# JasonHopeSpace/panda

Measured on AMD Instinct MI355X. Metric: MSM points/s (BN254, 2^24), higher is better.
Workload: dtype u32; 1 GPU; BN254 MSM 2^24 points per GPU, Jacobian output, bases and scalars resident in HBM; curve=bn254, log_points_per_gpu=24, exchange=none

## Files before the change

panda_amd/csrc/curve29.h:

```cpp
#pragma once
#include "fe29.h"

namespace panda29 {

template <class F>
struct Xyzz {
    Fe<F> X, Y, ZZ, ZZZ;
};

template <class F>
struct Bounds {
    static constexpr int M = SubMargin<F>::value;
    static constexpr int XB = 8 + M;
    static constexpr int YB = SubGrowth<F, 2>::value;
    static constexpr int PB = 2 + SubGrowth<F, XB>::value;
    static constexpr int RB = 2 + SubGrowth<F, YB>::value;
    static constexpr int VB = 2 + SubGrowth<F, XB>::value;
    static constexpr long long LIM = F::HEADROOM * 9 / 10;
    static_assert((long long)PB * PB < LIM, "P^2 exceeds the lazy-reduction headroom");
    static constexpr int NB = SubGrowth<F, 2>::value;
    static_assert((long long)RB * VB + (long long)YB * NB < LIM, "R*(Q-X3) - Y1*PPP exceeds the lazy-reduction headroom");
    static_assert(6LL * VB + 2LL * NB < LIM, "3x^2*(S-X3) - W*Y exceeds the lazy-reduction headroom");
    static_assert((long long)(2 * YB) * (2 * YB) < LIM, "(2Y)^2 exceeds the lazy-reduction headroom");
    static_assert(2 + SubGrowth<F, 6>::value <= XB, "X3 bound");
};

template <class F>
PANDA_HD void xyzz_set_identity(Xyzz<F> &p)
{
    fe_zero(p.X);
    fe_zero(p.Y);
    fe_zero(p.ZZ);
    fe_zero(p.ZZZ);
}

template <class F>
PANDA_HD bool xyzz_is_identity(const Xyzz<F> &p)
{
    return fe_all_zero(p.ZZ);
}

template <class F>
PANDA_HD void xyzz_from_affine(Xyzz<F> &p, const Fe<F> &x, const Fe<F> &y)
{
    p.X = x;
    p.Y = y;
    fe_one(p.ZZ);
    fe_one(p.ZZZ);
}

template <class F>
PANDA_HD void xyzz_finish(Fe<F> &X3, Fe<F> &Y3, const Fe<F> &R, const Fe<F> &Q, const Fe<F> &PPP, const Fe<F> &S1)
{
    typedef Bounds<F> B;
    Fe<F> t, rr, v, nppp;
    fe_add_nr(t, Q, Q);
    fe_add_nr(t, t, PPP);
    fe_sqr(rr, R);
    fe_sub<F, 6>(X3, rr, t);
    fe_sub<F, B::XB>(v, Q, X3);
    if constexpr (RawOperandOk<F>::value)
        fe_neg_raw<F, 2>(nppp, PPP);
    else
        fe_neg<F, 2>(nppp, PPP);
    fe_mul_add(Y3, R, v, S1, nppp);
}

template <class F>
PANDA_HD void xyzz_dbl_affine(Xyzz<F> &r, const Fe<F> &x, const Fe<F> &y)
{
    typedef Bounds<F> B;
    Fe<F> U, V, W, S, A, M3, t, v, t1, t2;
    fe_add(U, y, y);
    fe_sqr(V, U);
    if (fe_is_zero_2p(V)) {
        xyzz_set_identity(r);
        return;
    }
    fe_mul(W, U, V);
    fe_mul(S, x, V);
    fe_sqr(A, x);
    fe_add_nr(t, A, A);
    fe_add_nr(t, t, A);
    fe_norm(M3, t);
    fe_sqr(t1, M3);
    fe_add_nr(t, S, S);
    fe_sub<F, 4>(r.X, t1, t);
    fe_sub<F, B::XB>(v, S, r.X);
    fe_neg<F, 2>(t2, W);
    fe_mul_add(r.Y, M3, v, t2, y);
    r.ZZ = V;
    r.ZZZ = W;
}

template <class F>
PANDA_HD void xyzz_dbl(Xyzz<F> &r, const Xyzz<F> &p)
{
    typedef Bounds<F> B;
    if (xyzz_is_identity(p)) {
        xyzz_set_identity(r);
        return;
    }
    Fe<F> U, V, W, S, A, M3, t, v, t1, t2, X3, Y3;
    fe_add(U, p.Y, p.Y);
    fe_sqr(V, U);
    if (fe_is_zero_2p(V)) {
        xyzz_set_identity(r);
        return;
    }
    fe_mul(W, U, V);
    fe_mul(S, p.X, V);
    fe_sqr(A, p.X);
    fe_add_nr(t, A, A);
    fe_add_nr(t, t, A);
    fe_norm(M3, t);
    fe_sqr(t1, M3);
    fe_add_nr(t, S, S);
    fe_sub<F, 4>(X3, t1, t);
    fe_sub<F, B::XB>(v, S, X3);
    fe_neg<F, 2>(t2, W);
    fe_mul_add(Y3, M3, v, t2, p.Y);
    fe_mul(t, V, p.ZZ);
    fe_mul(t2, W, p.ZZZ);
    r.X = X3;
    r.Y = Y3;
    r.ZZ = t;
    r.ZZZ = t2;
}

template <class F>
PANDA_HD int xyzz_madd_core(Xyzz<F> &acc, const Fe<F> &bx, const Fe<F> &by)
{
    typedef Bounds<F> B;
    Fe<F> U2, S2, P, R, PP, PPP, Q, X3, Y3;
    fe_mul(U2, bx, acc.ZZ);
    fe_sub<F, B::XB>(P, U2, acc.X);
    fe_mul(S2, by, acc.ZZZ);
    fe_sub<F, B::YB>(R, S2, acc.Y);
    fe_sqr(PP, P);
    if (fe_is_zero_2p(PP))
        return fe_is_zero_mod_p(R) ? 1 : 2;
    fe_mul(PPP, P, PP);
    fe_mul(Q, acc.X, PP);
    fe_mul(acc.ZZ, acc.ZZ, PP);
    fe_mul(acc.ZZZ, acc.ZZZ, PPP);
    xyzz_finish(X3, Y3, R, Q, PPP, acc.Y);
    acc.X = X3;
    acc.Y = Y3;
    return 0;
}

template <class F>
PANDA_HD void xyzz_madd(Xyzz<F> &acc, const Fe<F> &bx, const Fe<F> &by, bool base_identity)
{
    if (base_identity) return;
    if (xyzz_is_identity(acc)) {
        xyzz_from_affine(acc, bx, by);
        return;
    }
    const int rare = xyzz_madd_core(acc, bx, by);
    if (rare == 1)
        xyzz_dbl_affine(acc, bx, by);
    else if (rare == 2)
        xyzz_set_identity(acc);
}

template <class F>
struct OutlineRareDoubling {
    static constexpr bool value = IsExt2<F>::value && F::N > 18;
};
template <class F>
#if defined(__HIPCC__)
__host__ __device__
#endif
__attribute__((noinline)) void xyzz_dbl_noinline(Xyzz<F> &r, const Xyzz<F> &p)
{
    xyzz_dbl(r, p);
}

template <class F>
PANDA_HD void xyzz_add(Xyzz<F> &acc, const Xyzz<F> &q)
{
    if (xyzz_is_identity(q)) return;
    if (xyzz_is_identity(acc)) {
        acc = q;
        return;
    }
    Fe<F> U1, U2, S1, S2, P, R, PP, PPP, Q, X3, Y3, t;
    fe_mul(U1, acc.X, q.ZZ);
    fe_mul(U2, q.X, acc.ZZ);
    fe_mul(S1, acc.Y, q.ZZZ);
    fe_mul(S2, q.Y, acc.ZZZ);
    fe_sub<F, 2>(P, U2, U1);
    fe_sub<F, 2>(R, S2, S1);
    fe_sqr(PP, P);
    if (fe_is_zero_2p(PP)) {
        if (fe_is_zero_mod_p(R)) {
            Xyzz<F> d;
            if constexpr (OutlineRareDoubling<F>::value)
                xyzz_dbl_noinline(d, acc);
            else
                xyzz_dbl(d, acc);
            acc = d;
        } else
            xyzz_set_identity(acc);
        return;
    }
    fe_mul(PPP, P, PP);
    fe_mul(Q, U1, PP);
    xyzz_finish(X3, Y3, R, Q, PPP, S1);
    fe_mul(t, acc.ZZ, q.ZZ);
    fe_mul(acc.ZZ, t, PP);
    fe_mul(t, acc.ZZZ, q.ZZZ);
    fe_mul(acc.ZZZ, t, PPP);
    acc.X = X3;
    acc.Y = Y3;
}

template <class F>
PANDA_HD void fe_neg_tight2p(Fe<F> &r, const Fe<F> &a)
{
    fe_neg<F, 2>(r, a);
}

template <class F>
PANDA_HD void xyzz_to_jacobian_wire(u32 *out, const Xyzz<F> &p)
{
    constexpr int L = F::L;
    if (xyzz_is_identity(p)) {
#pragma unroll
        for (int i = 0; i < 3 * L; i++) out[i] = 0;
        return;
    }
    Fe<F> x, y;
    fe_mul(x, p.X, p.ZZ);
    fe_mul(y, p.Y, p.ZZZ);
    fe_to_wire(out, x);
    fe_to_wire(out + L, y);
    fe_to_wire(out + 2 * L, p.ZZ);
}

template <class F>
PANDA_HD void xyzz_to_homogeneous_wire(u32 *out, const Xyzz<F> &p)
{
    constexpr int L = F::L;
    if (xyzz_is_identity(p)) {
#pragma unroll
        for (int i = 0; i < 3 * L; i++) out[i] = 0;
        return;
    }
    Fe<F> x, y, z;
    fe_mul(x, p.X, p.ZZZ);
    fe_mul(y, p.Y, p.ZZ);
    fe_mul(z, p.ZZ, p.ZZZ);
    fe_to_wire(out, x);
    fe_to_wire(out + L, y);
    fe_to_wire(out + 2 * L, z);
}

template <class F>
PANDA_HD void xyzz_to_affine_internal(Fe<F> &x, Fe<F> &y, const Xyzz<F> &p)
{
    Fe<F> zi3, t, zi2;
    fe_inv(zi3, p.ZZZ);
    fe_mul(t, p.ZZ, zi3);
    fe_sqr(zi2, t);
    fe_mul(x, p.X, zi2);
    fe_mul(y, p.Y, zi3);
}

template <class F>
PANDA_HD void xyzz_from_jacobian_wire(Xyzz<F> &p, const u32 *in)
{
    constexpr int L = F::L;
    Fe<F> z;
    fe_from_wire(z, in + 2 * L);
    if (fe_is_zero_2p(z)) {
        xyzz_set_identity(p);
        return;
    }
    fe_from_wire(p.X, in);
    fe_from_wire(p.Y, in + L);
    fe_sqr(p.ZZ, z);
    fe_mul(p.ZZZ, p.ZZ, z);
}

template <class F>
PANDA_HD bool affine_from_wire(Fe<F> &x, Fe<F> &y, const u32 *in)
{
    constexpr int L = F::L;
    u32 nz = 0;
#pragma unroll
    for (int i = 0; i < L; i++) nz |= in[i];
    fe_from_wire(x, in);
    fe_from_wire(y, in + L);
    return nz == 0;
}

}
```

panda_amd/csrc/fe29.h:

```cpp
#pragma once
#include <stdint.h>

#include "fe29_params.h"

#if defined(__HIPCC__)
#define PANDA_HD __host__ __device__ inline __attribute__((always_inline))
#else
#define PANDA_HD inline __attribute__((always_inline))
#endif

#if defined(FE29_CHECK)
#include <assert.h>
#define FE29_SHADOW_DECL unsigned __int128 shadow = 0;
#define FE29_SHADOW_MAC(x, y) shadow += (unsigned __int128)(x) * (y);
#define FE29_SHADOW_SHIFT()                                      \
    assert(shadow < ((unsigned __int128)1 << 64) && "fe29 column accumulator overflow"); \
    shadow >>= 29;
#else
#define FE29_SHADOW_DECL
#define FE29_SHADOW_MAC(x, y)
#define FE29_SHADOW_SHIFT()
#endif

#if defined(__HIP_DEVICE_COMPILE__) && !defined(FE29_NO_ASM)
#define FE29_MAC(acc, x, y) asm("v_mad_u64_u32 %0, vcc, %1, %2, %0" : "+v"(acc) : "v"(x), "v"(y) : "vcc")
#define FE29_MAC_CONST(acc, x, c) asm("v_mad_u64_u32 %0, vcc, %1, %2, %0" : "+v"(acc) : "v"(x), "s"(c) : "vcc")
#else
#define FE29_MAC(acc, x, y) acc += (u64)(x) * (y)
#define FE29_MAC_CONST(acc, x, c) acc += (u64)(x) * (c)
#endif

#if defined(__HIP_DEVICE_COMPILE__) && !defined(FE29_NO_ASM)
#define FE29_DEVICE_CHAINS 1
#include <utility>

#include "fe29_chain.h"
#endif

namespace panda29 {

typedef uint32_t u32;
typedef uint64_t u64;
constexpr u32 LIMB_BITS = 29;
constexpr u32 LIMB_MASK = (1u << 29) - 1;

template <class F>
struct Fe {
    u32 l[F::N];
};

template <class B>
struct Ext2;
template <class F>
struct IsExt2 {
    static constexpr bool value = false;
};
template <class B>
struct IsExt2<Ext2<B>> {
    static constexpr bool value = true;
};
template <class B>
PANDA_HD Fe<B> &ext_c0(Fe<Ext2<B>> &a) { return *reinterpret_cast<Fe<B> *>(&a.l[0]); }
template <class B>
PANDA_HD Fe<B> &ext_c1(Fe<Ext2<B>> &a) { return *reinterpret_cast<Fe<B> *>(&a.l[B::N]); }
template <class B>
PANDA_HD const Fe<B> &ext_c0(const Fe<Ext2<B>> &a) { return *reinterpret_cast<const Fe<B> *>(&a.l[0]); }
template <class B>
PANDA_HD const Fe<B> &ext_c1(const Fe<Ext2<B>> &a) { return *reinterpret_cast<const Fe<B> *>(&a.l[B::N]); }

template <class F>
PANDA_HD void fe_zero(Fe<F> &r)
{
#pragma unroll
    for (int i = 0; i < F::N; i++) r.l[i] = 0;
}

template <class F>
PANDA_HD void fe_one(Fe<F> &r)
{
#pragma unroll
    for (int i = 0; i < F::N; i++) r.l[i] = F::ONE[i];
}

template <class F>
PANDA_HD void fe_const(Fe<F> &r, const u32 (&c)[F::N])
{
#pragma unroll
    for (int i = 0; i < F::N; i++) r.l[i] = c[i];
}

template <class F>
PANDA_HD bool fe_all_zero(const Fe<F> &a)
{
    u32 acc = 0;
#pragma unroll
    for (int i = 0; i < F::N; i++) acc |= a.l[i];
    return acc == 0;
}

#if defined(FE29_DEVICE_CHAINS)
template <class F, int K>
__device__ inline __attribute__((always_inline)) void fe29_reduce_col(uint64_t &acc, uint32_t *m, uint32_t *out)
{
    constexpr int N = F::N;
    constexpr bool TOP0 = F::P[N - 1] == 0;
    if constexpr (K < N) {
        if constexpr (TOP0 && K == N - 1)
            MacChain<K - 1>::vs(acc, m + 1, &F::P[K - 1]);
        else
            MacChain<K>::vs(acc, m, &F::P[K]);
        m[K] = ((uint32_t)acc * F::INV) & ((1u << 29) - 1);
        MacChain<1>::vs(acc, m + K, &F::P[0]);
    } else {
        if constexpr (TOP0)
            MacChain<2 * N - 2 - K>::vs(acc, m + (K - N + 2), &F::P[N - 2]);
        else
            MacChain<2 * N - 1 - K>::vs(acc, m + (K - N + 1), &F::P[N - 1]);
        out[K - N] = (uint32_t)acc & ((1u << 29) - 1);
    }
    acc >>= 29;
}
template <class F, int K>
__device__ inline __attribute__((always_inline)) void fe29_mul_col(uint64_t &acc, const uint32_t *a, const uint32_t *b, uint32_t *m, uint32_t *out)
{
    constexpr int N = F::N;
    if constexpr (K == 0)
        MacChain<1>::vv0(acc, a, b);
    else if constexpr (K < N)
        MacChain<K + 1>::vv(acc, a, b + K);
    else
        MacChain<2 * N - 1 - K>::vv(acc, a + (K - N + 1), b + (N - 1));
    fe29_reduce_col<F, K>(acc, m, out);
}
template <class F, int K>
__device__ inline __attribute__((always_inline)) void fe29_sqr_col(uint64_t &acc, const uint32_t *a, const uint32_t *a2, uint32_t *m, uint32_t *out)
{
    constexpr int N = F::N;
    constexpr int I0 = K < N ? 0 : K - N + 1;
    constexpr int CNT = (K + 1) / 2 - I0;
    MacChain<CNT>::vv(acc, a2 + I0, a + (K - I0));
    if constexpr (K == 0)
        MacChain<1>::vv0(acc, a, a);
    else if constexpr ((K & 1) == 0)
        MacChain<1>::vv(acc, a + K / 2, a + K / 2);
    fe29_reduce_col<F, K>(acc, m, out);
}
template <class F, int... K>
__device__ inline __attribute__((always_inline)) void fe29_mul_cols(uint64_t &acc, const uint32_t *a, const uint32_t *b, uint32_t *m, uint32_t *out, std::integer_sequence<int, K...>)
{
    (fe29_mul_col<F, K>(acc, a, b, m, out), ...);
}
template <class F, int K>
__device__ inline __attribute__((always_inline)) void fe29_mul_add_col(uint64_t &acc, const uint32_t *a, const uint32_t *b, const uint32_t *c, const uint32_t *d, uint32_t *m,
                                                                       uint32_t *out)
{
    constexpr int N = F::N;
    if constexpr (K == 0) {
        MacChain<1>::vv0(acc, a, b);
        MacChain<1>::vv(acc, c, d);
    } else if constexpr (K < N) {
        MacChain<K + 1>::vv(acc, a, b + K);
        MacChain<K + 1>::vv(acc, c, d + K);
    } else {
        MacChain<2 * N - 1 - K>::vv(acc, a + (K - N + 1), b + (N - 1));
        MacChain<2 * N - 1 - K>::vv(acc, c + (K - N + 1), d + (N - 1));
    }
    fe29_reduce_col<F, K>(acc, m, out);
}
template <class F, int... K>
__device__ inline __attribute__((always_inline)) void fe29_mul_add_cols(uint64_t &acc, const uint32_t *a, const uint32_t *b, const uint32_t *c, const uint32_t *d,
                                                                        uint32_t *m, uint32_t *out, std::integer_sequence<int, K...>)
{
    (fe29_mul_add_col<F, K>(acc, a, b, c, d, m, out), ...);
}
template <class F, int... K>
__device__ inline __attribute__((always_inline)) void fe29_sqr_cols(uint64_t &acc, const uint32_t *a, const uint32_t *a2, uint32_t *m, uint32_t *out, std::integer_sequence<int, K...>)
{
    (fe29_sqr_col<F, K>(acc, a, a2, m, out), ...);
}
#endif

template <class F>
PANDA_HD void fe_mul(Fe<F> &r, const Fe<F> &a, const Fe<F> &b)
{
    constexpr int N = F::N;
    u32 m[N];
    u32 out[N];
    u64 acc = 0;
#if defined(FE29_DEVICE_CHAINS)
    fe29_mul_cols<F>(acc, a.l, b.l, m, out, std::make_integer_sequence<int, 2 * N - 1>());
    out[N - 1] = (u32)acc;
#pragma unroll
    for (int i = 0; i < N; i++) r.l[i] = out[i];
    return;
#endif
    FE29_SHADOW_DECL
#pragma unroll
    for (int k = 0; k < N; k++) {
#pragma unroll
        for (int i = 0; i <= k; i++) {
            FE29_MAC(acc, a.l[i], b.l[k - i]);
            FE29_SHADOW_MAC(a.l[i], b.l[k - i])
        }
#pragma unroll
        for (int i = 0; i < k; i++) {
            FE29_MAC_CONST(acc, m[i], F::P[k - i]);
            FE29_SHADOW_MAC(m[i], F::P[k - i])
        }
        m[k] = ((u32)acc * F::INV) & LIMB_MASK;
        FE29_MAC_CONST(acc, m[k], F::P[0]);
        FE29_SHADOW_MAC(m[k], F::P[0])
        acc >>= LIMB_BITS;
        FE29_SHADOW_SHIFT()
    }
#pragma unroll
    for (int k = N; k < 2 * N - 1; k++) {
#pragma unroll
        for (int i = k - N + 1; i < N; i++) {
            FE29_MAC(acc, a.l[i], b.l[k - i]);
            FE29_SHADOW_MAC(a.l[i], b.l[k - i])
        }
#pragma unroll
        for (int i = k - N + 1; i < N; i++) {
            FE29_MAC_CONST(acc, m[i], F::P[k - i]);
            FE29_SHADOW_MAC(m[i], F::P[k - i])
        }
        out[k - N] = (u32)acc & LIMB_MASK;
        acc >>= LIMB_BITS;
        FE29_SHADOW_SHIFT()
    }
    out[N - 1] = (u32)acc;
#pragma unroll
    for (int i = 0; i < N; i++) r.l[i] = out[i];
}

template <class F>
PANDA_HD void fe_mul_add(Fe<F> &r, const Fe<F> &a, const Fe<F> &b, const Fe<F> &c, const Fe<F> &d)
{
    constexpr int N = F::N;
    static_assert(3 * N * (1ull << 58) + (3ull * N << 38) < (1ull << 63) * 2 - 1, "column accumulator too narrow");
    u32 m[N];
    u32 out[N];
    u64 acc = 0;
#if defined(FE29_DEVICE_CHAINS)
    fe29_mul_add_cols<F>(acc, a.l, b.l, c.l, d.l, m, out, std::make_integer_sequence<int, 2 * N - 1>());
    out[N - 1] = (u32)acc;
#pragma unroll
    for (int i = 0; i < N; i++) r.l[i] = out[i];
    return;
#endif
    FE29_SHADOW_DECL
#pragma unroll
    for (int k = 0; k < N; k++) {
#pragma unroll
        for (int i = 0; i <= k; i++) {
            FE29_MAC(acc, a.l[i], b.l[k - i]);
            FE29_SHADOW_MAC(a.l[i], b.l[k - i])
            FE29_MAC(acc, c.l[i], d.l[k - i]);
            FE29_SHADOW_MAC(c.l[i], d.l[k - i])
        }
#pragma unroll
        for (int i = 0; i < k; i++) {
            FE29_MAC_CONST(acc, m[i], F::P[k - i]);
            FE29_SHADOW_MAC(m[i], F::P[k - i])
        }
        m[k] = ((u32)acc * F::INV) & LIMB_MASK;
        FE29_MAC_CONST(acc, m[k], F::P[0]);
        FE29_SHADOW_MAC(m[k], F::P[0])
        acc >>= LIMB_BITS;
        FE29_SHADOW_SHIFT()
    }
#pragma unroll
    for (int k = N; k < 2 * N - 1; k++) {
#pragma unroll
        for (int i = k - N + 1; i < N; i++) {
            FE29_MAC(acc, a.l[i], b.l[k - i]);
            FE29_SHADOW_MAC(a.l[i], b.l[k - i])
            FE29_MAC(acc, c.l[i], d.l[k - i]);
            FE29_SHADOW_MAC(c.l[i], d.l[k - i])
        }
#pragma unroll
        for (int i = k - N + 1; i < N; i++) {
            FE29_MAC_CONST(acc, m[i], F::P[k - i]);
            FE29_SHADOW_MAC(m[i], F::P[k - i])
        }
        out[k - N] = (u32)acc & LIMB_MASK;
        acc >>= LIMB_BITS;
        FE29_SHADOW_SHIFT()
    }
    out[N - 1] = (u32)acc;
#pragma unroll
    for (int i = 0; i < N; i++) r.l[i] = out[i];
}

template <class F>
PANDA_HD void fe_sqr(Fe<F> &r, const Fe<F> &a)
{
    constexpr int N = F::N;
    u32 m[N], out[N], a2[N];
#pragma unroll
    for (int i = 0; i < N; i++) a2[i] = a.l[i] << 1;
    u64 acc = 0;
#if defined(FE29_DEVICE_CHAINS)
    fe29_sqr_cols<F>(acc, a.l, a2, m, out, std::make_integer_sequence<int, 2 * N - 1>());
    out[N - 1] = (u32)acc;
#pragma unroll
    for (int i = 0; i < N; i++) r.l[i] = out[i];
    return;
#endif
    FE29_SHADOW_DECL
#pragma unroll
    for (int k = 0; k < N; k++) {
#pragma unroll
        for (int i = 0; 2 * i < k; i++) {
            FE29_MAC(acc, a2[i], a.l[k - i]);
            FE29_SHADOW_MAC(a2[i], a.l[k - i])
        }
        if ((k & 1) == 0) {
            FE29_MAC(acc, a.l[k / 2], a.l[k / 2]);
            FE29_SHADOW_MAC(a.l[k / 2], a.l[k / 2])
        }
#pragma unroll
        for (int i = 0; i < k; i++) {
            FE29_MAC_CONST(acc, m[i], F::P[k - i]);
            FE29_SHADOW_MAC(m[i], F::P[k - i])
        }
        m[k] = ((u32)acc * F::INV) & LIMB_MASK;
        FE29_MAC_CONST(acc, m[k], F::P[0]);
        FE29_SHADOW_MAC(m[k], F::P[0])
        acc >>= LIMB_BITS;
        FE29_SHADOW_SHIFT()
    }
// ... 21 lines not shown
#pragma unroll
    for (int i = 0; i < N; i++) r.l[i] = out[i];
}

template <class F>
PANDA_HD void fe_norm(Fe<F> &r, const Fe<F> &t)
{
    constexpr int N = F::N;
    u32 c[N];
#pragma unroll
    for (int i = 0; i < N - 1; i++) c[i] = t.l[i] >> LIMB_BITS;
    u32 o[N];
    o[0] = t.l[0] & LIMB_MASK;
#pragma unroll
    for (int i = 1; i < N - 1; i++) o[i] = (t.l[i] & LIMB_MASK) + c[i - 1];
    o[N - 1] = t.l[N - 1] + c[N - 2];
#pragma unroll
    for (int i = 0; i < N; i++) r.l[i] = o[i];
}

template <class F>
PANDA_HD void fe_add_nr(Fe<F> &r, const Fe<F> &a, const Fe<F> &b)
{
#pragma unroll
    for (int i = 0; i < F::N; i++) r.l[i] = a.l[i] + b.l[i];
}

template <class F>
PANDA_HD void fe_add(Fe<F> &r, const Fe<F> &a, const Fe<F> &b)
{
    Fe<F> t;
    fe_add_nr(t, a, b);
    fe_norm(r, t);
}

template <class F>
struct SubMargin {
    static constexpr int value = (F::P[F::N - 1] >= 16) ? 1 : 6;
};

template <class F, int KB>
PANDA_HD void fe_sub(Fe<F> &r, const Fe<F> &a, const Fe<F> &b)
{
    if constexpr (IsExt2<F>::value) {
        fe_sub<typename F::Base, KB>(ext_c0(r), ext_c0(a), ext_c0(b));
        fe_sub<typename F::Base, KB>(ext_c1(r), ext_c1(a), ext_c1(b));
        return;
    } else {
    constexpr int K = KB + SubMargin<F>::value;
    static_assert(K <= 200, "subtraction constant table too small");
    Fe<F> t;
#pragma unroll
    for (int i = 0; i < F::N; i++) {
#if defined(FE29_CHECK)
        assert((u64)a.l[i] + F::KP[K][i] >= b.l[i] && (u64)a.l[i] + F::KP[K][i] - b.l[i] < (1ull << 32) && "fe_sub limb range");
#endif
        t.l[i] = a.l[i] + F::KP[K][i] - b.l[i];
    }
    fe_norm(r, t);
    }
}

template <class F, int K>
PANDA_HD constexpr u32 fe_kp30(int i)
{
    return i == 0 ? F::KP[K][0] - (2u << LIMB_BITS) : (i < F::N - 1 ? F::KP[K][i] - (2u << LIMB_BITS) + 2u : F::KP[K][i] + 2u);
}

template <class F>
struct RawOperandOk {
    static constexpr bool value = F::N <= 9;
};

template <class F, int KB>
PANDA_HD void fe_sub_raw(Fe<F> &r, const Fe<F> &a, const Fe<F> &b)
{
    static_assert(RawOperandOk<F>::value, "no column headroom for a raw operand in this field");
    constexpr int K = KB + SubMargin<F>::value;
    static_assert(K <= 200, "subtraction constant table too small");
#pragma unroll
    for (int i = 0; i < F::N; i++) {
        const u32 kp = fe_kp30<F, K>(i);
#if defined(FE29_CHECK)
        assert((u64)a.l[i] + kp >= b.l[i] && (u64)a.l[i] + kp - b.l[i] < (1ull << 31) + (1ull << 24) && "fe_sub_raw limb range");
#endif
        r.l[i] = a.l[i] + kp - b.l[i];
    }
}

template <class F, int K, int U>
PANDA_HD constexpr u32 fe_kp_bias(int i)
{
    static_assert(U >= 2 && U <= 4, "bias in units of 2^29");
    return i == 0 ? F::KP[K][0] - ((u32)(4 - U) << LIMB_BITS) : (i < F::N - 1 ? F::KP[K][i] - ((u32)(4 - U) << LIMB_BITS) + (u32)(4 - U) : F::KP[K][i] + (u32)(4 - U));
}
template <class F, int KB, int U>
PANDA_HD void fe_sub_raw_bias(Fe<F> &r, const Fe<F> &a, const Fe<F> &b)
{
    static_assert(RawOperandOk<F>::value, "no column headroom for a raw operand in this field");
    constexpr int K = KB + SubMargin<F>::value;
    static_assert(K <= 200, "subtraction constant table too small");
#pragma unroll
    for (int i = 0; i < F::N; i++) {
        const u32 kp = fe_kp_bias<F, K, U>(i);
#if defined(FE29_CHECK)
        assert((u64)a.l[i] + kp >= b.l[i] && (u64)a.l[i] + kp - b.l[i] < 3 * (1ull << 30) + 64 && "fe_sub_raw_bias limb range");
#endif
        r.l[i] = a.l[i] + kp - b.l[i];
    }
}

template <class F, int KB>
PANDA_HD void fe_neg_raw(Fe<F> &r, const Fe<F> &a)
{
    static_assert(RawOperandOk<F>::value, "no column headroom for a raw operand in this field");
    constexpr int K = KB + SubMargin<F>::value;
#pragma unroll
    for (int i = 0; i < F::N; i++) {
        const u32 kp = fe_kp30<F, K>(i);
#if defined(FE29_CHECK)
        assert(kp >= a.l[i] && "fe_neg_raw limb range");
#endif
        r.l[i] = kp - a.l[i];
    }
}

template <class F, int KB>
struct SubGrowth {
    static constexpr int value = F::KEFF[KB + SubMargin<F>::value];
};

template <class F, int KB>
PANDA_HD void fe_neg(Fe<F> &r, const Fe<F> &a)
{
    if constexpr (IsExt2<F>::value) {
        fe_neg<typename F::Base, KB>(ext_c0(r), ext_c0(a));
        fe_neg<typename F::Base, KB>(ext_c1(r), ext_c1(a));
        return;
    } else {
    constexpr int K = KB + SubMargin<F>::value;
    Fe<F> t;
#pragma unroll
    for (int i = 0; i < F::N; i++) {
#if defined(FE29_CHECK)
        assert(F::KP[K][i] >= a.l[i] && "fe_neg limb range");
#endif
        t.l[i] = F::KP[K][i] - a.l[i];
    }
    fe_norm(r, t);
    }
}

template <class F>
PANDA_HD void fe_unpack(Fe<F> &r, const u32 *w)
{
    constexpr int N = F::N, L = F::L;
#pragma unroll
    for (int k = 0; k < N; k++) {
        const int bit = 29 * k, wi = bit >> 5, sh = bit & 31;
        u32 v = 0;
        if (wi < L) {
            v = w[wi] >> sh;
            if (sh > 3 && wi + 1 < L) v |= w[wi + 1] << (32 - sh);
        }
        r.l[k] = (k < N - 1) ? (v & LIMB_MASK) : v;
    }
}

template <class F>
PANDA_HD void fe_pack(u32 *w, const Fe<F> &a)
{
    constexpr int N = F::N, L = F::L;
#pragma unroll
    for (int i = 0; i < L; i++) {
        const int bit = 32 * i, j = bit / 29, s = bit - 29 * j;
        u32 v = a.l[j] >> s;
        if (j + 1 < N) v |= a.l[j + 1] << (29 - s);
        if (29 - s + 29 < 32 && j + 2 < N) v |= a.l[j + 2] << (58 - s);
        w[i] = v;
    }
}

template <class F>
PANDA_HD void fe_words_neg(u32 *r, const u32 *w)
{
    static_assert(!IsExt2<F>::value, "prime fields only");
#if defined(__clang__)
    unsigned borrow = 0;
#pragma unroll
    for (int i = 0; i < F::L; i++) r[i] = __builtin_subc(F::PW[i], w[i], borrow, &borrow);
#else
    u32 borrow = 0;
#pragma unroll
    for (int i = 0; i < F::L; i++) {
        const u32 d = F::PW[i] - w[i];
        const u32 out = (u32)(F::PW[i] < w[i]) | (u32)(d < borrow);
        r[i] = d - borrow;
        borrow = out;
    }
#endif
}

template <class F>
PANDA_HD void fe_carry(Fe<F> &a)
{
#pragma unroll
    for (int i = 0; i < F::N - 1; i++) {
#if defined(FE29_CHECK)
        assert((u64)a.l[i + 1] + (a.l[i] >> LIMB_BITS) < (1ull << 32) && "fe_carry limb range");
#endif
        a.l[i + 1] += a.l[i] >> LIMB_BITS;
        a.l[i] &= LIMB_MASK;
    }
}

template <class F>
PANDA_HD void fe_reduce_once(Fe<F> &a)
{
    constexpr int N = F::N;
    u32 d[N];
    u32 borrow = 0;
#pragma unroll
    for (int i = 0; i < N; i++) {
        u32 t = a.l[i] - F::P[i] - borrow;
        borrow = t >> 31;
        d[i] = (i < N - 1) ? (t & LIMB_MASK) : t;
    }
#pragma unroll
    for (int i = 0; i < N; i++) a.l[i] = borrow ? a.l[i] : d[i];
}

template <class F>
PANDA_HD void fe_reduce_small_2p(Fe<F> &a)
{
    constexpr int N = F::N;
    fe_carry(a);
    u32 m;
    if constexpr (F::P[N - 1] >= (1u << 16)) {
        constexpr u64 C = (1ull << 52) / ((u64)F::P[N - 1] + 1);
        m = (u32)(((u64)a.l[N - 1] * C) >> 52);
    } else {
        constexpr u64 D = ((u64)F::P[N - 1] << LIMB_BITS) + F::P[N - 2] + 1;
        static_assert(F::P[N - 1] < (1u << 12) && D >= (1u << 16), "fe_reduce_small: two-limb quotient estimate needs 2^16 <= D, top limb of p < 2^12");
        constexpr u64 C = (1ull << 52) / D;
        const u64 T = ((u64)a.l[N - 1] << LIMB_BITS) | a.l[N - 2];
        m = (u32)((T * C) >> 52);
    }
    int64_t carry = 0;
#pragma unroll
    for (int i = 0; i < N; i++) {
        int64_t t = (int64_t)a.l[i] - (int64_t)((u64)m * F::P[i]) + carry;
        a.l[i] = (i < N - 1) ? ((u32)t & LIMB_MASK) : (u32)t;
        carry = t >> LIMB_BITS;
    }
}

template <class F>
PANDA_HD void fe_reduce_small(Fe<F> &a)
{
    fe_reduce_small_2p(a);
    fe_reduce_once(a);
}

template <class F>
struct FeTw {
    u32 w[F::N];
    u32 q[F::N];
};

#if defined(FE29_DEVICE_CHAINS)
template <class F, bool UNIFORM, int C>
__device__ inline __attribute__((always_inline)) void fe29_shoup_hi_col(uint64_t &acc, const uint32_t *x, const uint32_t *wq, uint32_t *q)
{
    constexpr int N = F::N;
    constexpr int I0 = C < N ? 0 : C - N + 1;
    constexpr int CNT = (C < N ? C : N - 1) - I0 + 1;
    if constexpr (C == N - 2) {
        if constexpr (UNIFORM)
            MacChain<CNT>::vs0(acc, x + I0, wq + (C - I0));
        else
            MacChain<CNT>::vv0(acc, x + I0, wq + (C - I0));
    } else if constexpr (UNIFORM)
        MacChain<CNT>::vs(acc, x + I0, wq + (C - I0));
    else
        MacChain<CNT>::vv(acc, x + I0, wq + (C - I0));
    if constexpr (C >= N) q[C - N] = (uint32_t)acc & ((1u << 29) - 1);
    acc >>= 29;
}
template <class F, bool UNIFORM, int... C>
__device__ inline __attribute__((always_inline)) void fe29_shoup_hi_cols(uint64_t &acc, const uint32_t *x, const uint32_t *wq, uint32_t *q, std::integer_sequence<int, C...>)
{
    (fe29_shoup_hi_col<F, UNIFORM, F::N - 2 + C>(acc, x, wq, q), ...);
}
template <class F, bool UNIFORM, int C>
__device__ inline __attribute__((always_inline)) void fe29_shoup_lo_col(uint64_t &acc, const uint32_t *x, const uint32_t *w, const uint32_t *q, uint32_t *out)
{
    if constexpr (C == 0) {
        if constexpr (UNIFORM)
            MacChain<1>::vs0(acc, x, w);
        else
            MacChain<1>::vv0(acc, x, w);
    } else if constexpr (UNIFORM)
        MacChain<C + 1>::vs(acc, x, w + C);
    else
        MacChain<C + 1>::vv(acc, x, w + C);
    MacChain<C + 1>::vs(acc, q, &F::PNEG[C]);
    out[C] = (uint32_t)acc & ((1u << 29) - 1);
    if constexpr (C + 1 < F::N) acc >>= 29;
}
template <class F, bool UNIFORM, int... C>
__device__ inline __attribute__((always_inline)) void fe29_shoup_lo_cols(uint64_t &acc, const uint32_t *x, const uint32_t *w, const uint32_t *q, uint32_t *out,
                                                                         std::integer_sequence<int, C...>)
{
    (fe29_shoup_lo_col<F, UNIFORM, C>(acc, x, w, q, out), ...);
}
template <class F, bool UNIFORM, int... C>
__device__ inline __attribute__((always_inline)) void fe29_shoup_hi_cols_x2(uint64_t &a0, uint64_t &a1, const uint32_t *x0, const uint32_t *x1, const uint32_t *wq0,
                                                                            const uint32_t *wq1, uint32_t *q0, uint32_t *q1, std::integer_sequence<int, C...>)
{
    ((fe29_shoup_hi_col<F, UNIFORM, F::N - 2 + C>(a0, x0, wq0, q0), fe29_shoup_hi_col<F, UNIFORM, F::N - 2 + C>(a1, x1, wq1, q1)), ...);
}
template <class F, bool UNIFORM, int... C>
__device__ inline __attribute__((always_inline)) void fe29_shoup_lo_cols_x2(uint64_t &a0, uint64_t &a1, const uint32_t *x0, const uint32_t *x1, const uint32_t *w0,
                                                                            const uint32_t *w1, const uint32_t *q0, const uint32_t *q1, uint32_t *o0, uint32_t *o1,
                                                                            std::integer_sequence<int, C...>)
{
    ((fe29_shoup_lo_col<F, UNIFORM, C>(a0, x0, w0, q0, o0), fe29_shoup_lo_col<F, UNIFORM, C>(a1, x1, w1, q1, o1)), ...);
}
#endif

template <class F, bool UNIFORM = false>
PANDA_HD void fe_mul_shoup(Fe<F> &r, const Fe<F> &x, const u32 *w, const u32 *wq)
{
    constexpr int N = F::N;
    static_assert(RawOperandOk<F>::value, "no column headroom for a raw operand in this field");
    u32 q[N], out[N];
    u64 acc = 0;
#if defined(FE29_DEVICE_CHAINS)
    fe29_shoup_hi_cols<F, UNIFORM>(acc, x.l, wq, q, std::make_integer_sequence<int, N + 1>());
    q[N - 1] = (u32)acc & LIMB_MASK;
    acc = 0;
    fe29_shoup_lo_cols<F, UNIFORM>(acc, x.l, w, q, out, std::make_integer_sequence<int, N>());
#pragma unroll
// ... 231 lines not shown
```

panda_amd/csrc/fe29_chain.h:

```cpp
#pragma once
#include <stdint.h>

namespace panda29 {

template <int CNT>
struct MacChain;

template <>
struct MacChain<1> {
    static __device__ inline __attribute__((always_inline)) void vv(uint64_t &acc, const uint32_t *x, const uint32_t *y)
    {
        asm("v_mad_u64_u32 %0, vcc, %1, %2, %0" : "+v"(acc) : "v"(x[0]), "v"(y[0]) : "vcc");
    }
    static __device__ inline __attribute__((always_inline)) void vs(uint64_t &acc, const uint32_t *x, const uint32_t *y)
    {
        asm("v_mad_u64_u32 %0, vcc, %1, %2, %0" : "+v"(acc) : "v"(x[0]), "s"(y[0]) : "vcc");
    }
    static __device__ inline __attribute__((always_inline)) void vv0(uint64_t &acc, const uint32_t *x, const uint32_t *y)
    {
        asm("v_mad_u64_u32 %0, vcc, %1, %2, 0" : "=&v"(acc) : "v"(x[0]), "v"(y[0]) : "vcc");
    }
    static __device__ inline __attribute__((always_inline)) void vs0(uint64_t &acc, const uint32_t *x, const uint32_t *y)
    {
        asm("v_mad_u64_u32 %0, vcc, %1, %2, 0" : "=&v"(acc) : "v"(x[0]), "s"(y[0]) : "vcc");
    }
};
template <>
struct MacChain<2> {
    static __device__ inline __attribute__((always_inline)) void vv(uint64_t &acc, const uint32_t *x, const uint32_t *y)
    {
        asm("v_mad_u64_u32 %0, vcc, %1, %2, %0\n\tv_mad_u64_u32 %0, vcc, %3, %4, %0" : "+v"(acc) : "v"(x[0]), "v"(y[0]), "v"(x[1]), "v"(y[-1]) : "vcc");
    }
    static __device__ inline __attribute__((always_inline)) void vs(uint64_t &acc, const uint32_t *x, const uint32_t *y)
    {
        asm("v_mad_u64_u32 %0, vcc, %1, %2, %0\n\tv_mad_u64_u32 %0, vcc, %3, %4, %0" : "+v"(acc) : "v"(x[0]), "s"(y[0]), "v"(x[1]), "s"(y[-1]) : "vcc");
    }
    static __device__ inline __attribute__((always_inline)) void vv0(uint64_t &acc, const uint32_t *x, const uint32_t *y)
    {
        asm("v_mad_u64_u32 %0, vcc, %1, %2, 0\n\tv_mad_u64_u32 %0, vcc, %3, %4, %0" : "=&v"(acc) : "v"(x[0]), "v"(y[0]), "v"(x[1]), "v"(y[-1]) : "vcc");
    }
    static __device__ inline __attribute__((always_inline)) void vs0(uint64_t &acc, const uint32_t *x, const uint32_t *y)
    {
        asm("v_mad_u64_u32 %0, vcc, %1, %2, 0\n\tv_mad_u64_u32 %0, vcc, %3, %4, %0" : "=&v"(acc) : "v"(x[0]), "s"(y[0]), "v"(x[1]), "s"(y[-1]) : "vcc");
    }
};
template <>
struct MacChain<3> {
    static __device__ inline __attribute__((always_inline)) void vv(uint64_t &acc, const uint32_t *x, const uint32_t *y)
    {
        asm("v_mad_u64_u32 %0, vcc, %1, %2, %0\n\tv_mad_u64_u32 %0, vcc, %3, %4, %0\n\tv_mad_u64_u32 %0, vcc, %5, %6, %0" : "+v"(acc) : "v"(x[0]), "v"(y[0]), "v"(x[1]), "v"(y[-1]), "v"(x[2]), "v"(y[-2]) : "vcc");
    }
    static __device__ inline __attribute__((always_inline)) void vs(uint64_t &acc, const uint32_t *x, const uint32_t *y)
    {
        asm("v_mad_u64_u32 %0, vcc, %1, %2, %0\n\tv_mad_u64_u32 %0, vcc, %3, %4, %0\n\tv_mad_u64_u32 %0, vcc, %5, %6, %0" : "+v"(acc) : "v"(x[0]), "s"(y[0]), "v"(x[1]), "s"(y[-1]), "v"(x[2]), "s"(y[-2]) : "vcc");
    }
    static __device__ inline __attribute__((always_inline)) void vv0(uint64_t &acc, const uint32_t *x, const uint32_t *y)
    {
        asm("v_mad_u64_u32 %0, vcc, %1, %2, 0\n\tv_mad_u64_u32 %0, vcc, %3, %4, %0\n\tv_mad_u64_u32 %0, vcc, %5, %6, %0" : "=&v"(acc) : "v"(x[0]), "v"(y[0]), "v"(x[1]), "v"(y[-1]), "v"(x[2]), "v"(y[-2]) : "vcc");
    }
    static __device__ inline __attribute__((always_inline)) void vs0(uint64_t &acc, const uint32_t *x, const uint32_t *y)
    {
        asm("v_mad_u64_u32 %0, vcc, %1, %2, 0\n\tv_mad_u64_u32 %0, vcc, %3, %4, %0\n\tv_mad_u64_u32 %0, vcc, %5, %6, %0" : "=&v"(acc) : "v"(x[0]), "s"(y[0]), "v"(x[1]), "s"(y[-1]), "v"(x[2]), "s"(y[-2]) : "vcc");
    }
};
template <>
struct MacChain<4> {
    static __device__ inline __attribute__((always_inline)) void vv(uint64_t &acc, const uint32_t *x, const uint32_t *y)
    {
        asm("v_mad_u64_u32 %0, vcc, %1, %2, %0\n\tv_mad_u64_u32 %0, vcc, %3, %4, %0\n\tv_mad_u64_u32 %0, vcc, %5, %6, %0\n\tv_mad_u64_u32 %0, vcc, %7, %8, %0" : "+v"(acc) : "v"(x[0]), "v"(y[0]), "v"(x[1]), "v"(y[-1]), "v"(x[2]), "v"(y[-2]), "v"(x[3]), "v"(y[-3]) : "vcc");
    }
    static __device__ inline __attribute__((always_inline)) void vs(uint64_t &acc, const uint32_t *x, const uint32_t *y)
    {
        asm("v_mad_u64_u32 %0, vcc, %1, %2, %0\n\tv_mad_u64_u32 %0, vcc, %3, %4, %0\n\tv_mad_u64_u32 %0, vcc, %5, %6, %0\n\tv_mad_u64_u32 %0, vcc, %7, %8, %0" : "+v"(acc) : "v"(x[0]), "s"(y[0]), "v"(x[1]), "s"(y[-1]), "v"(x[2]), "s"(y[-2]), "v"(x[3]), "s"(y[-3]) : "vcc");
    }
    static __device__ inline __attribute__((always_inline)) void vv0(uint64_t &acc, const uint32_t *x, const uint32_t *y)
    {
        asm("v_mad_u64_u32 %0, vcc, %1, %2, 0\n\tv_mad_u64_u32 %0, vcc, %3, %4, %0\n\tv_mad_u64_u32 %0, vcc, %5, %6, %0\n\tv_mad_u64_u32 %0, vcc, %7, %8, %0" : "=&v"(acc) : "v"(x[0]), "v"(y[0]), "v"(x[1]), "v"(y[-1]), "v"(x[2]), "v"(y[-2]), "v"(x[3]), "v"(y[-3]) : "vcc");
    }
    static __device__ inline __attribute__((always_inline)) void vs0(uint64_t &acc, const uint32_t *x, const uint32_t *y)
    {
        asm("v_mad_u64_u32 %0, vcc, %1, %2, 0\n\tv_mad_u64_u32 %0, vcc, %3, %4, %0\n\tv_mad_u64_u32 %0, vcc, %5, %6, %0\n\tv_mad_u64_u32 %0, vcc, %7, %8, %0" : "=&v"(acc) : "v"(x[0]), "s"(y[0]), "v"(x[1]), "s"(y[-1]), "v"(x[2]), "s"(y[-2]), "v"(x[3]), "s"(y[-3]) : "vcc");
    }
};
template <>
struct MacChain<5> {
    static __device__ inline __attribute__((always_inline)) void vv(uint64_t &acc, const uint32_t *x, const uint32_t *y)
    {
        asm("v_mad_u64_u32 %0, vcc, %1, %2, %0\n\tv_mad_u64_u32 %0, vcc, %3, %4, %0\n\tv_mad_u64_u32 %0, vcc, %5, %6, %0\n\tv_mad_u64_u32 %0, vcc, %7, %8, %0\n\tv_mad_u64_u32 %0, vcc, %9, %10, %0" : "+v"(acc) : "v"(x[0]), "v"(y[0]), "v"(x[1]), "v"(y[-1]), "v"(x[2]), "v"(y[-2]), "v"(x[3]), "v"(y[-3]), "v"(x[4]), "v"(y[-4]) : "vcc");
    }
    static __device__ inline __attribute__((always_inline)) void vs(uint64_t &acc, const uint32_t *x, const uint32_t *y)
    {
        asm("v_mad_u64_u32 %0, vcc, %1, %2, %0\n\tv_mad_u64_u32 %0, vcc, %3, %4, %0\n\tv_mad_u64_u32 %0, vcc, %5, %6, %0\n\tv_mad_u64_u32 %0, vcc, %7, %8, %0\n\tv_mad_u64_u32 %0, vcc, %9, %10, %0" : "+v"(acc) : "v"(x[0]), "s"(y[0]), "v"(x[1]), "s"(y[-1]), "v"(x[2]), "s"(y[-2]), "v"(x[3]), "s"(y[-3]), "v"(x[4]), "s"(y[-4]) : "vcc");
    }
    static __device__ inline __attribute__((always_inline)) void vv0(uint64_t &acc, const uint32_t *x, const uint32_t *y)
    {
        asm("v_mad_u64_u32 %0, vcc, %1, %2, 0\n\tv_mad_u64_u32 %0, vcc, %3, %4, %0\n\tv_mad_u64_u32 %0, vcc, %5, %6, %0\n\tv_mad_u64_u32 %0, vcc, %7, %8, %0\n\tv_mad_u64_u32 %0, vcc, %9, %10, %0" : "=&v"(acc) : "v"(x[0]), "v"(y[0]), "v"(x[1]), "v"(y[-1]), "v"(x[2]), "v"(y[-2]), "v"(x[3]), "v"(y[-3]), "v"(x[4]), "v"(y[-4]) : "vcc");
    }
    static __device__ inline __attribute__((always_inline)) void vs0(uint64_t &acc, const uint32_t *x, const uint32_t *y)
    {
        asm("v_mad_u64_u32 %0, vcc, %1, %2, 0\n\tv_mad_u64_u32 %0, vcc, %3, %4, %0\n\tv_mad_u64_u32 %0, vcc, %5, %6, %0\n\tv_mad_u64_u32 %0, vcc, %7, %8, %0\n\tv_mad_u64_u32 %0, vcc, %9, %10, %0" : "=&v"(acc) : "v"(x[0]), "s"(y[0]), "v"(x[1]), "s"(y[-1]), "v"(x[2]), "s"(y[-2]), "v"(x[3]), "s"(y[-3]), "v"(x[4]), "s"(y[-4]) : "vcc");
    }
};
template <>
struct MacChain<6> {
    static __device__ inline __attribute__((always_inline)) void vv(uint64_t &acc, const uint32_t *x, const uint32_t *y)
    {
        asm("v_mad_u64_u32 %0, vcc, %1, %2, %0\n\tv_mad_u64_u32 %0, vcc, %3, %4, %0\n\tv_mad_u64_u32 %0, vcc, %5, %6, %0\n\tv_mad_u64_u32 %0, vcc, %7, %8, %0\n\tv_mad_u64_u32 %0, vcc, %9, %10, %0\n\tv_mad_u64_u32 %0, vcc, %11, %12, %0" : "+v"(acc) : "v"(x[0]), "v"(y[0]), "v"(x[1]), "v"(y[-1]), "v"(x[2]), "v"(y[-2]), "v"(x[3]), "v"(y[-3]), "v"(x[4]), "v"(y[-4]), "v"(x[5]), "v"(y[-5]) : "vcc");
    }
    static __device__ inline __attribute__((always_inline)) void vs(uint64_t &acc, const uint32_t *x, const uint32_t *y)
    {
        asm("v_mad_u64_u32 %0, vcc, %1, %2, %0\n\tv_mad_u64_u32 %0, vcc, %3, %4, %0\n\tv_mad_u64_u32 %0, vcc, %5, %6, %0\n\tv_mad_u64_u32 %0, vcc, %7, %8, %0\n\tv_mad_u64_u32 %0, vcc, %9, %10, %0\n\tv_mad_u64_u32 %0, vcc, %11, %12, %0" : "+v"(acc) : "v"(x[0]), "s"(y[0]), "v"(x[1]), "s"(y[-1]), "v"(x[2]), "s"(y[-2]), "v"(x[3]), "s"(y[-3]), "v"(x[4]), "s"(y[-4]), "v"(x[5]), "s"(y[-5]) : "vcc");
    }
    static __device__ inline __attribute__((always_inline)) void vv0(uint64_t &acc, const uint32_t *x, const uint32_t *y)
    {
        asm("v_mad_u64_u32 %0, vcc, %1, %2, 0\n\tv_mad_u64_u32 %0, vcc, %3, %4, %0\n\tv_mad_u64_u32 %0, vcc, %5, %6, %0\n\tv_mad_u64_u32 %0, vcc, %7, %8, %0\n\tv_mad_u64_u32 %0, vcc, %9, %10, %0\n\tv_mad_u64_u32 %0, vcc, %11, %12, %0" : "=&v"(acc) : "v"(x[0]), "v"(y[0]), "v"(x[1]), "v"(y[-1]), "v"(x[2]), "v"(y[-2]), "v"(x[3]), "v"(y[-3]), "v"(x[4]), "v"(y[-4]), "v"(x[5]), "v"(y[-5]) : "vcc");
    }
    static __device__ inline __attribute__((always_inline)) void vs0(uint64_t &acc, const uint32_t *x, const uint32_t *y)
    {
        asm("v_mad_u64_u32 %0, vcc, %1, %2, 0\n\tv_mad_u64_u32 %0, vcc, %3, %4, %0\n\tv_mad_u64_u32 %0, vcc, %5, %6, %0\n\tv_mad_u64_u32 %0, vcc, %7, %8, %0\n\tv_mad_u64_u32 %0, vcc, %9, %10, %0\n\tv_mad_u64_u32 %0, vcc, %11, %12, %0" : "=&v"(acc) : "v"(x[0]), "s"(y[0]), "v"(x[1]), "s"(y[-1]), "v"(x[2]), "s"(y[-2]), "v"(x[3]), "s"(y[-3]), "v"(x[4]), "s"(y[-4]), "v"(x[5]), "s"(y[-5]) : "vcc");
    }
};
template <>
struct MacChain<7> {
    static __device__ inline __attribute__((always_inline)) void vv(uint64_t &acc, const uint32_t *x, const uint32_t *y)
    {
        asm("v_mad_u64_u32 %0, vcc, %1, %2, %0\n\tv_mad_u64_u32 %0, vcc, %3, %4, %0\n\tv_mad_u64_u32 %0, vcc, %5, %6, %0\n\tv_mad_u64_u32 %0, vcc, %7, %8, %0\n\tv_mad_u64_u32 %0, vcc, %9, %10, %0\n\tv_mad_u64_u32 %0, vcc, %11, %12, %0\n\tv_mad_u64_u32 %0, vcc, %13, %14, %0" : "+v"(acc) : "v"(x[0]), "v"(y[0]), "v"(x[1]), "v"(y[-1]), "v"(x[2]), "v"(y[-2]), "v"(x[3]), "v"(y[-3]), "v"(x[4]), "v"(y[-4]), "v"(x[5]), "v"(y[-5]), "v"(x[6]), "v"(y[-6]) : "vcc");
    }
    static __device__ inline __attribute__((always_inline)) void vs(uint64_t &acc, const uint32_t *x, const uint32_t *y)
    {
        asm("v_mad_u64_u32 %0, vcc, %1, %2, %0\n\tv_mad_u64_u32 %0, vcc, %3, %4, %0\n\tv_mad_u64_u32 %0, vcc, %5, %6, %0\n\tv_mad_u64_u32 %0, vcc, %7, %8, %0\n\tv_mad_u64_u32 %0, vcc, %9, %10, %0\n\tv_mad_u64_u32 %0, vcc, %11, %12, %0\n\tv_mad_u64_u32 %0, vcc, %13, %14, %0" : "+v"(acc) : "v"(x[0]), "s"(y[0]), "v"(x[1]), "s"(y[-1]), "v"(x[2]), "s"(y[-2]), "v"(x[3]), "s"(y[-3]), "v"(x[4]), "s"(y[-4]), "v"(x[5]), "s"(y[-5]), "v"(x[6]), "s"(y[-6]) : "vcc");
    }
    static __device__ inline __attribute__((always_inline)) void vv0(uint64_t &acc, const uint32_t *x, const uint32_t *y)
    {
        asm("v_mad_u64_u32 %0, vcc, %1, %2, 0\n\tv_mad_u64_u32 %0, vcc, %3, %4, %0\n\tv_mad_u64_u32 %0, vcc, %5, %6, %0\n\tv_mad_u64_u32 %0, vcc, %7, %8, %0\n\tv_mad_u64_u32 %0, vcc, %9, %10, %0\n\tv_mad_u64_u32 %0, vcc, %11, %12, %0\n\tv_mad_u64_u32 %0, vcc, %13, %14, %0" : "=&v"(acc) : "v"(x[0]), "v"(y[0]), "v"(x[1]), "v"(y[-1]), "v"(x[2]), "v"(y[-2]), "v"(x[3]), "v"(y[-3]), "v"(x[4]), "v"(y[-4]), "v"(x[5]), "v"(y[-5]), "v"(x[6]), "v"(y[-6]) : "vcc");
    }
    static __device__ inline __attribute__((always_inline)) void vs0(uint64_t &acc, const uint32_t *x, const uint32_t *y)
    {
        asm("v_mad_u64_u32 %0, vcc, %1, %2, 0\n\tv_mad_u64_u32 %0, vcc, %3, %4, %0\n\tv_mad_u64_u32 %0, vcc, %5, %6, %0\n\tv_mad_u64_u32 %0, vcc, %7, %8, %0\n\tv_mad_u64_u32 %0, vcc, %9, %10, %0\n\tv_mad_u64_u32 %0, vcc, %11, %12, %0\n\tv_mad_u64_u32 %0, vcc, %13, %14, %0" : "=&v"(acc) : "v"(x[0]), "s"(y[0]), "v"(x[1]), "s"(y[-1]), "v"(x[2]), "s"(y[-2]), "v"(x[3]), "s"(y[-3]), "v"(x[4]), "s"(y[-4]), "v"(x[5]), "s"(y[-5]), "v"(x[6]), "s"(y[-6]) : "vcc");
    }
};
template <>
struct MacChain<8> {
    static __device__ inline __attribute__((always_inline)) void vv(uint64_t &acc, const uint32_t *x, const uint32_t *y)
    {
        asm("v_mad_u64_u32 %0, vcc, %1, %2, %0\n\tv_mad_u64_u32 %0, vcc, %3, %4, %0\n\tv_mad_u64_u32 %0, vcc, %5, %6, %0\n\tv_mad_u64_u32 %0, vcc, %7, %8, %0\n\tv_mad_u64_u32 %0, vcc, %9, %10, %0\n\tv_mad_u64_u32 %0, vcc, %11, %12, %0\n\tv_mad_u64_u32 %0, vcc, %13, %14, %0\n\tv_mad_u64_u32 %0, vcc, %15, %16, %0" : "+v"(acc) : "v"(x[0]), "v"(y[0]), "v"(x[1]), "v"(y[-1]), "v"(x[2]), "v"(y[-2]), "v"(x[3]), "v"(y[-3]), "v"(x[4]), "v"(y[-4]), "v"(x[5]), "v"(y[-5]), "v"(x[6]), "v"(y[-6]), "v"(x[7]), "v"(y[-7]) : "vcc");
    }
    static __device__ inline __attribute__((always_inline)) void vs(uint64_t &acc, const uint32_t *x, const uint32_t *y)
    {
        asm("v_mad_u64_u32 %0, vcc, %1, %2, %0\n\tv_mad_u64_u32 %0, vcc, %3, %4, %0\n\tv_mad_u64_u32 %0, vcc, %5, %6, %0\n\tv_mad_u64_u32 %0, vcc, %7, %8, %0\n\tv_mad_u64_u32 %0, vcc, %9, %10, %0\n\tv_mad_u64_u32 %0, vcc, %11, %12, %0\n\tv_mad_u64_u32 %0, vcc, %13, %14, %0\n\tv_mad_u64_u32 %0, vcc, %15, %16, %0" : "+v"(acc) : "v"(x[0]), "s"(y[0]), "v"(x[1]), "s"(y[-1]), "v"(x[2]), "s"(y[-2]), "v"(x[3]), "s"(y[-3]), "v"(x[4]), "s"(y[-4]), "v"(x[5]), "s"(y[-5]), "v"(x[6]), "s"(y[-6]), "v"(x[7]), "s"(y[-7]) : "vcc");
    }
    static __device__ inline __attribute__((always_inline)) void vv0(uint64_t &acc, const uint32_t *x, const uint32_t *y)
    {
        asm("v_mad_u64_u32 %0, vcc, %1, %2, 0\n\tv_mad_u64_u32 %0, vcc, %3, %4, %0\n\tv_mad_u64_u32 %0, vcc, %5, %6, %0\n\tv_mad_u64_u32 %0, vcc, %7, %8, %0\n\tv_mad_u64_u32 %0, vcc, %9, %10, %0\n\tv_mad_u64_u32 %0, vcc, %11, %12, %0\n\tv_mad_u64_u32 %0, vcc, %13, %14, %0\n\tv_mad_u64_u32 %0, vcc, %15, %16, %0" : "=&v"(acc) : "v"(x[0]), "v"(y[0]), "v"(x[1]), "v"(y[-1]), "v"(x[2]), "v"(y[-2]), "v"(x[3]), "v"(y[-3]), "v"(x[4]), "v"(y[-4]), "v"(x[5]), "v"(y[-5]), "v"(x[6]), "v"(y[-6]), "v"(x[7]), "v"(y[-7]) : "vcc");
    }
    static __device__ inline __attribute__((always_inline)) void vs0(uint64_t &acc, const uint32_t *x, const uint32_t *y)
    {
        asm("v_mad_u64_u32 %0, vcc, %1, %2, 0\n\tv_mad_u64_u32 %0, vcc, %3, %4, %0\n\tv_mad_u64_u32 %0, vcc, %5, %6, %0\n\tv_mad_u64_u32 %0, vcc, %7, %8, %0\n\tv_mad_u64_u32 %0, vcc, %9, %10, %0\n\tv_mad_u64_u32 %0, vcc, %11, %12, %0\n\tv_mad_u64_u32 %0, vcc, %13, %14, %0\n\tv_mad_u64_u32 %0, vcc, %15, %16, %0" : "=&v"(acc) : "v"(x[0]), "s"(y[0]), "v"(x[1]), "s"(y[-1]), "v"(x[2]), "s"(y[-2]), "v"(x[3]), "s"(y[-3]), "v"(x[4]), "s"(y[-4]), "v"(x[5]), "s"(y[-5]), "v"(x[6]), "s"(y[-6]), "v"(x[7]), "s"(y[-7]) : "vcc");
    }
};
template <>
struct MacChain<9> {
    static __device__ inline __attribute__((always_inline)) void vv(uint64_t &acc, const uint32_t *x, const uint32_t *y)
    {
        asm("v_mad_u64_u32 %0, vcc, %1, %2, %0\n\tv_mad_u64_u32 %0, vcc, %3, %4, %0\n\tv_mad_u64_u32 %0, vcc, %5, %6, %0\n\tv_mad_u64_u32 %0, vcc, %7, %8, %0\n\tv_mad_u64_u32 %0, vcc, %9, %10, %0\n\tv_mad_u64_u32 %0, vcc, %11, %12, %0\n\tv_mad_u64_u32 %0, vcc, %13, %14, %0\n\tv_mad_u64_u32 %0, vcc, %15, %16, %0\n\tv_mad_u64_u32 %0, vcc, %17, %18, %0" : "+v"(acc) : "v"(x[0]), "v"(y[0]), "v"(x[1]), "v"(y[-1]), "v"(x[2]), "v"(y[-2]), "v"(x[3]), "v"(y[-3]), "v"(x[4]), "v"(y[-4]), "v"(x[5]), "v"(y[-5]), "v"(x[6]), "v"(y[-6]), "v"(x[7]), "v"(y[-7]), "v"(x[8]), "v"(y[-8]) : "vcc");
    }
    static __device__ inline __attribute__((always_inline)) void vs(uint64_t &acc, const uint32_t *x, const uint32_t *y)
    {
        asm("v_mad_u64_u32 %0, vcc, %1, %2, %0\n\tv_mad_u64_u32 %0, vcc, %3, %4, %0\n\tv_mad_u64_u32 %0, vcc, %5, %6, %0\n\tv_mad_u64_u32 %0, vcc, %7, %8, %0\n\tv_mad_u64_u32 %0, vcc, %9, %10, %0\n\tv_mad_u64_u32 %0, vcc, %11, %12, %0\n\tv_mad_u64_u32 %0, vcc, %13, %14, %0\n\tv_mad_u64_u32 %0, vcc, %15, %16, %0\n\tv_mad_u64_u32 %0, vcc, %17, %18, %0" : "+v"(acc) : "v"(x[0]), "s"(y[0]), "v"(x[1]), "s"(y[-1]), "v"(x[2]), "s"(y[-2]), "v"(x[3]), "s"(y[-3]), "v"(x[4]), "s"(y[-4]), "v"(x[5]), "s"(y[-5]), "v"(x[6]), "s"(y[-6]), "v"(x[7]), "s"(y[-7]), "v"(x[8]), "s"(y[-8]) : "vcc");
    }
    static __device__ inline __attribute__((always_inline)) void vv0(uint64_t &acc, const uint32_t *x, const uint32_t *y)
    {
        asm("v_mad_u64_u32 %0, vcc, %1, %2, 0\n\tv_mad_u64_u32 %0, vcc, %3, %4, %0\n\tv_mad_u64_u32 %0, vcc, %5, %6, %0\n\tv_mad_u64_u32 %0, vcc, %7, %8, %0\n\tv_mad_u64_u32 %0, vcc, %9, %10, %0\n\tv_mad_u64_u32 %0, vcc, %11, %12, %0\n\tv_mad_u64_u32 %0, vcc, %13, %14, %0\n\tv_mad_u64_u32 %0, vcc, %15, %16, %0\n\tv_mad_u64_u32 %0, vcc, %17, %18, %0" : "=&v"(acc) : "v"(x[0]), "v"(y[0]), "v"(x[1]), "v"(y[-1]), "v"(x[2]), "v"(y[-2]), "v"(x[3]), "v"(y[-3]), "v"(x[4]), "v"(y[-4]), "v"(x[5]), "v"(y[-5]), "v"(x[6]), "v"(y[-6]), "v"(x[7]), "v"(y[-7]), "v"(x[8]), "v"(y[-8]) : "vcc");
    }
    static __device__ inline __attribute__((always_inline)) void vs0(uint64_t &acc, const uint32_t *x, const uint32_t *y)
    {
        asm("v_mad_u64_u32 %0, vcc, %1, %2, 0\n\tv_mad_u64_u32 %0, vcc, %3, %4, %0\n\tv_mad_u64_u32 %0, vcc, %5, %6, %0\n\tv_mad_u64_u32 %0, vcc, %7, %8, %0\n\tv_mad_u64_u32 %0, vcc, %9, %10, %0\n\tv_mad_u64_u32 %0, vcc, %11, %12, %0\n\tv_mad_u64_u32 %0, vcc, %13, %14, %0\n\tv_mad_u64_u32 %0, vcc, %15, %16, %0\n\tv_mad_u64_u32 %0, vcc, %17, %18, %0" : "=&v"(acc) : "v"(x[0]), "s"(y[0]), "v"(x[1]), "s"(y[-1]), "v"(x[2]), "s"(y[-2]), "v"(x[3]), "s"(y[-3]), "v"(x[4]), "s"(y[-4]), "v"(x[5]), "s"(y[-5]), "v"(x[6]), "s"(y[-6]), "v"(x[7]), "s"(y[-7]), "v"(x[8]), "s"(y[-8]) : "vcc");
    }
};
template <>
struct MacChain<10> {
    static __device__ inline __attribute__((always_inline)) void vv(uint64_t &acc, const uint32_t *x, const uint32_t *y)
    {
        asm("v_mad_u64_u32 %0, vcc, %1, %2, %0\n\tv_mad_u64_u32 %0, vcc, %3, %4, %0\n\tv_mad_u64_u32 %0, vcc, %5, %6, %0\n\tv_mad_u64_u32 %0, vcc, %7, %8, %0\n\tv_mad_u64_u32 %0, vcc, %9, %10, %0\n\tv_mad_u64_u32 %0, vcc, %11, %12, %0\n\tv_mad_u64_u32 %0, vcc, %13, %14, %0\n\tv_mad_u64_u32 %0, vcc, %15, %16, %0\n\tv_mad_u64_u32 %0, vcc, %17, %18, %0\n\tv_mad_u64_u32 %0, vcc, %19, %20, %0" : "+v"(acc) : "v"(x[0]), "v"(y[0]), "v"(x[1]), "v"(y[-1]), "v"(x[2]), "v"(y[-2]), "v"(x[3]), "v"(y[-3]), "v"(x[4]), "v"(y[-4]), "v"(x[5]), "v"(y[-5]), "v"(x[6]), "v"(y[-6]), "v"(x[7]), "v"(y[-7]), "v"(x[8]), "v"(y[-8]), "v"(x[9]), "v"(y[-9]) : "vcc");
    }
    static __device__ inline __attribute__((always_inline)) void vs(uint64_t &acc, const uint32_t *x, const uint32_t *y)
    {
        asm("v_mad_u64_u32 %0, vcc, %1, %2, %0\n\tv_mad_u64_u32 %0, vcc, %3, %4, %0\n\tv_mad_u64_u32 %0, vcc, %5, %6, %0\n\tv_mad_u64_u32 %0, vcc, %7, %8, %0\n\tv_mad_u64_u32 %0, vcc, %9, %10, %0\n\tv_mad_u64_u32 %0, vcc, %11, %12, %0\n\tv_mad_u64_u32 %0, vcc, %13, %14, %0\n\tv_mad_u64_u32 %0, vcc, %15, %16, %0\n\tv_mad_u64_u32 %0, vcc, %17, %18, %0\n\tv_mad_u64_u32 %0, vcc, %19, %20, %0" : "+v"(acc) : "v"(x[0]), "s"(y[0]), "v"(x[1]), "s"(y[-1]), "v"(x[2]), "s"(y[-2]), "v"(x[3]), "s"(y[-3]), "v"(x[4]), "s"(y[-4]), "v"(x[5]), "s"(y[-5]), "v"(x[6]), "s"(y[-6]), "v"(x[7]), "s"(y[-7]), "v"(x[8]), "s"(y[-8]), "v"(x[9]), "s"(y[-9]) : "vcc");
    }
    static __device__ inline __attribute__((always_inline)) void vv0(uint64_t &acc, const uint32_t *x, const uint32_t *y)
    {
        asm("v_mad_u64_u32 %0, vcc, %1, %2, 0\n\tv_mad_u64_u32 %0, vcc, %3, %4, %0\n\tv_mad_u64_u32 %0, vcc, %5, %6, %0\n\tv_mad_u64_u32 %0, vcc, %7, %8, %0\n\tv_mad_u64_u32 %0, vcc, %9, %10, %0\n\tv_mad_u64_u32 %0, vcc, %11, %12, %0\n\tv_mad_u64_u32 %0, vcc, %13, %14, %0\n\tv_mad_u64_u32 %0, vcc, %15, %16, %0\n\tv_mad_u64_u32 %0, vcc, %17, %18, %0\n\tv_mad_u64_u32 %0, vcc, %19, %20, %0" : "=&v"(acc) : "v"(x[0]), "v"(y[0]), "v"(x[1]), "v"(y[-1]), "v"(x[2]), "v"(y[-2]), "v"(x[3]), "v"(y[-3]), "v"(x[4]), "v"(y[-4]), "v"(x[5]), "v"(y[-5]), "v"(x[6]), "v"(y[-6]), "v"(x[7]), "v"(y[-7]), "v"(x[8]), "v"(y[-8]), "v"(x[9]), "v"(y[-9]) : "vcc");
    }
    static __device__ inline __attribute__((always_inline)) void vs0(uint64_t &acc, const uint32_t *x, const uint32_t *y)
    {
        asm("v_mad_u64_u32 %0, vcc, %1, %2, 0\n\tv_mad_u64_u32 %0, vcc, %3, %4, %0\n\tv_mad_u64_u32 %0, vcc, %5, %6, %0\n\tv_mad_u64_u32 %0, vcc, %7, %8, %0\n\tv_mad_u64_u32 %0, vcc, %9, %10, %0\n\tv_mad_u64_u32 %0, vcc, %11, %12, %0\n\tv_mad_u64_u32 %0, vcc, %13, %14, %0\n\tv_mad_u64_u32 %0, vcc, %15, %16, %0\n\tv_mad_u64_u32 %0, vcc, %17, %18, %0\n\tv_mad_u64_u32 %0, vcc, %19, %20, %0" : "=&v"(acc) : "v"(x[0]), "s"(y[0]), "v"(x[1]), "s"(y[-1]), "v"(x[2]), "s"(y[-2]), "v"(x[3]), "s"(y[-3]), "v"(x[4]), "s"(y[-4]), "v"(x[5]), "s"(y[-5]), "v"(x[6]), "s"(y[-6]), "v"(x[7]), "s"(y[-7]), "v"(x[8]), "s"(y[-8]), "v"(x[9]), "s"(y[-9]) : "vcc");
    }
};
template <>
struct MacChain<11> {
    static __device__ inline __attribute__((always_inline)) void vv(uint64_t &acc, const uint32_t *x, const uint32_t *y)
    {
        asm("v_mad_u64_u32 %0, vcc, %1, %2, %0\n\tv_mad_u64_u32 %0, vcc, %3, %4, %0\n\tv_mad_u64_u32 %0, vcc, %5, %6, %0\n\tv_mad_u64_u32 %0, vcc, %7, %8, %0\n\tv_mad_u64_u32 %0, vcc, %9, %10, %0\n\tv_mad_u64_u32 %0, vcc, %11, %12, %0\n\tv_mad_u64_u32 %0, vcc, %13, %14, %0\n\tv_mad_u64_u32 %0, vcc, %15, %16, %0\n\tv_mad_u64_u32 %0, vcc, %17, %18, %0\n\tv_mad_u64_u32 %0, vcc, %19, %20, %0\n\tv_mad_u64_u32 %0, vcc, %21, %22, %0" : "+v"(acc) : "v"(x[0]), "v"(y[0]), "v"(x[1]), "v"(y[-1]), "v"(x[2]), "v"(y[-2]), "v"(x[3]), "v"(y[-3]), "v"(x[4]), "v"(y[-4]), "v"(x[5]), "v"(y[-5]), "v"(x[6]), "v"(y[-6]), "v"(x[7]), "v"(y[-7]), "v"(x[8]), "v"(y[-8]), "v"(x[9]), "v"(y[-9]), "v"(x[10]), "v"(y[-10]) : "vcc");
    }
    static __device__ inline __attribute__((always_inline)) void vs(uint64_t &acc, const uint32_t *x, const uint32_t *y)
    {
        asm("v_mad_u64_u32 %0, vcc, %1, %2, %0\n\tv_mad_u64_u32 %0, vcc, %3, %4, %0\n\tv_mad_u64_u32 %0, vcc, %5, %6, %0\n\tv_mad_u64_u32 %0, vcc, %7, %8, %0\n\tv_mad_u64_u32 %0, vcc, %9, %10, %0\n\tv_mad_u64_u32 %0, vcc, %11, %12, %0\n\tv_mad_u64_u32 %0, vcc, %13, %14, %0\n\tv_mad_u64_u32 %0, vcc, %15, %16, %0\n\tv_mad_u64_u32 %0, vcc, %17, %18, %0\n\tv_mad_u64_u32 %0, vcc, %19, %20, %0\n\tv_mad_u64_u32 %0, vcc, %21, %22, %0" : "+v"(acc) : "v"(x[0]), "s"(y[0]), "v"(x[1]), "s"(y[-1]), "v"(x[2]), "s"(y[-2]), "v"(x[3]), "s"(y[-3]), "v"(x[4]), "s"(y[-4]), "v"(x[5]), "s"(y[-5]), "v"(x[6]), "s"(y[-6]), "v"(x[7]), "s"(y[-7]), "v"(x[8]), "s"(y[-8]), "v"(x[9]), "s"(y[-9]), "v"(x[10]), "s"(y[-10]) : "vcc");
    }
    static __device__ inline __attribute__((always_inline)) void vv0(uint64_t &acc, const uint32_t *x, const uint32_t *y)
    {
        asm("v_mad_u64_u32 %0, vcc, %1, %2, 0\n\tv_mad_u64_u32 %0, vcc, %3, %4, %0\n\tv_mad_u64_u32 %0, vcc, %5, %6, %0\n\tv_mad_u64_u32 %0, vcc, %7, %8, %0\n\tv_mad_u64_u32 %0, vcc, %9, %10, %0\n\tv_mad_u64_u32 %0, vcc, %11, %12, %0\n\tv_mad_u64_u32 %0, vcc, %13, %14, %0\n\tv_mad_u64_u32 %0, vcc, %15, %16, %0\n\tv_mad_u64_u32 %0, vcc, %17, %18, %0\n\tv_mad_u64_u32 %0, vcc, %19, %20, %0\n\tv_mad_u64_u32 %0, vcc, %21, %22, %0" : "=&v"(acc) : "v"(x[0]), "v"(y[0]), "v"(x[1]), "v"(y[-1]), "v"(x[2]), "v"(y[-2]), "v"(x[3]), "v"(y[-3]), "v"(x[4]), "v"(y[-4]), "v"(x[5]), "v"(y[-5]), "v"(x[6]), "v"(y[-6]), "v"(x[7]), "v"(y[-7]), "v"(x[8]), "v"(y[-8]), "v"(x[9]), "v"(y[-9]), "v"(x[10]), "v"(y[-10]) : "vcc");
    }
    static __device__ inline __attribute__((always_inline)) void vs0(uint64_t &acc, const uint32_t *x, const uint32_t *y)
    {
        asm("v_mad_u64_u32 %0, vcc, %1, %2, 0\n\tv_mad_u64_u32 %0, vcc, %3, %4, %0\n\tv_mad_u64_u32 %0, vcc, %5, %6, %0\n\tv_mad_u64_u32 %0, vcc, %7, %8, %0\n\tv_mad_u64_u32 %0, vcc, %9, %10, %0\n\tv_mad_u64_u32 %0, vcc, %11, %12, %0\n\tv_mad_u64_u32 %0, vcc, %13, %14, %0\n\tv_mad_u64_u32 %0, vcc, %15, %16, %0\n\tv_mad_u64_u32 %0, vcc, %17, %18, %0\n\tv_mad_u64_u32 %0, vcc, %19, %20, %0\n\tv_mad_u64_u32 %0, vcc, %21, %22, %0" : "=&v"(acc) : "v"(x[0]), "s"(y[0]), "v"(x[1]), "s"(y[-1]), "v"(x[2]), "s"(y[-2]), "v"(x[3]), "s"(y[-3]), "v"(x[4]), "s"(y[-4]), "v"(x[5]), "s"(y[-5]), "v"(x[6]), "s"(y[-6]), "v"(x[7]), "s"(y[-7]), "v"(x[8]), "s"(y[-8]), "v"(x[9]), "s"(y[-9]), "v"(x[10]), "s"(y[-10]) : "vcc");
    }
};
template <>
struct MacChain<12> {
    static __device__ inline __attribute__((always_inline)) void vv(uint64_t &acc, const uint32_t *x, const uint32_t *y)
    {
        asm("v_mad_u64_u32 %0, vcc, %1, %2, %0\n\tv_mad_u64_u32 %0, vcc, %3, %4, %0\n\tv_mad_u64_u32 %0, vcc, %5, %6, %0\n\tv_mad_u64_u32 %0, vcc, %7, %8, %0\n\tv_mad_u64_u32 %0, vcc, %9, %10, %0\n\tv_mad_u64_u32 %0, vcc, %11, %12, %0\n\tv_mad_u64_u32 %0, vcc, %13, %14, %0\n\tv_mad_u64_u32 %0, vcc, %15, %16, %0\n\tv_mad_u64_u32 %0, vcc, %17, %18, %0\n\tv_mad_u64_u32 %0, vcc, %19, %20, %0\n\tv_mad_u64_u32 %0, vcc, %21, %22, %0\n\tv_mad_u64_u32 %0, vcc, %23, %24, %0" : "+v"(acc) : "v"(x[0]), "v"(y[0]), "v"(x[1]), "v"(y[-1]), "v"(x[2]), "v"(y[-2]), "v"(x[3]), "v"(y[-3]), "v"(x[4]), "v"(y[-4]), "v"(x[5]), "v"(y[-5]), "v"(x[6]), "v"(y[-6]), "v"(x[7]), "v"(y[-7]), "v"(x[8]), "v"(y[-8]), "v"(x[9]), "v"(y[-9]), "v"(x[10]), "v"(y[-10]), "v"(x[11]), "v"(y[-11]) : "vcc");
    }
    static __device__ inline __attribute__((always_inline)) void vs(uint64_t &acc, const uint32_t *x, const uint32_t *y)
    {
        asm("v_mad_u64_u32 %0, vcc, %1, %2, %0\n\tv_mad_u64_u32 %0, vcc, %3, %4, %0\n\tv_mad_u64_u32 %0, vcc, %5, %6, %0\n\tv_mad_u64_u32 %0, vcc, %7, %8, %0\n\tv_mad_u64_u32 %0, vcc, %9, %10, %0\n\tv_mad_u64_u32 %0, vcc, %11, %12, %0\n\tv_mad_u64_u32 %0, vcc, %13, %14, %0\n\tv_mad_u64_u32 %0, vcc, %15, %16, %0\n\tv_mad_u64_u32 %0, vcc, %17, %18, %0\n\tv_mad_u64_u32 %0, vcc, %19, %20, %0\n\tv_mad_u64_u32 %0, vcc, %21, %22, %0\n\tv_mad_u64_u32 %0, vcc, %23, %24, %0" : "+v"(acc) : "v"(x[0]), "s"(y[0]), "v"(x[1]), "s"(y[-1]), "v"(x[2]), "s"(y[-2]), "v"(x[3]), "s"(y[-3]), "v"(x[4]), "s"(y[-4]), "v"(x[5]), "s"(y[-5]), "v"(x[6]), "s"(y[-6]), "v"(x[7]), "s"(y[-7]), "v"(x[8]), "s"(y[-8]), "v"(x[9]), "s"(y[-9]), "v"(x[10]), "s"(y[-10]), "v"(x[11]), "s"(y[-11]) : "vcc");
    }
    static __device__ inline __attribute__((always_inline)) void vv0(uint64_t &acc, const uint32_t *x, const uint32_t *y)
    {
        asm("v_mad_u64_u32 %0, vcc, %1, %2, 0\n\tv_mad_u64_u32 %0, vcc, %3, %4, %0\n\tv_mad_u64_u32 %0, vcc, %5, %6, %0\n\tv_mad_u64_u32 %0, vcc, %7, %8, %0\n\tv_mad_u64_u32 %0, vcc, %9, %10, %0\n\tv_mad_u64_u32 %0, vcc, %11, %12, %0\n\tv_mad_u64_u32 %0, vcc, %13, %14, %0\n\tv_mad_u64_u32 %0, vcc, %15, %16, %0\n\tv_mad_u64_u32 %0, vcc, %17, %18, %0\n\tv_mad_u64_u32 %0, vcc, %19, %20, %0\n\tv_mad_u64_u32 %0, vcc, %21, %22, %0\n\tv_mad_u64_u32 %0, vcc, %23, %24, %0" : "=&v"(acc) : "v"(x[0]), "v"(y[0]), "v"(x[1]), "v"(y[-1]), "v"(x[2]), "v"(y[-2]), "v"(x[3]), "v"(y[-3]), "v"(x[4]), "v"(y[-4]), "v"(x[5]), "v"(y[-5]), "v"(x[6]), "v"(y[-6]), "v"(x[7]), "v"(y[-7]), "v"(x[8]), "v"(y[-8]), "v"(x[9]), "v"(y[-9]), "v"(x[10]), "v"(y[-10]), "v"(x[11]), "v"(y[-11]) : "vcc");
    }
    static __device__ inline __attribute__((always_inline)) void vs0(uint64_t &acc, const uint32_t *x, const uint32_t *y)
    {
        asm("v_mad_u64_u32 %0, vcc, %1, %2, 0\n\tv_mad_u64_u32 %0, vcc, %3, %4, %0\n\tv_mad_u64_u32 %0, vcc, %5, %6, %0\n\tv_mad_u64_u32 %0, vcc, %7, %8, %0\n\tv_mad_u64_u32 %0, vcc, %9, %10, %0\n\tv_mad_u64_u32 %0, vcc, %11, %12, %0\n\tv_mad_u64_u32 %0, vcc, %13, %14, %0\n\tv_mad_u64_u32 %0, vcc, %15, %16, %0\n\tv_mad_u64_u32 %0, vcc, %17, %18, %0\n\tv_mad_u64_u32 %0, vcc, %19, %20, %0\n\tv_mad_u64_u32 %0, vcc, %21, %22, %0\n\tv_mad_u64_u32 %0, vcc, %23, %24, %0" : "=&v"(acc) : "v"(x[0]), "s"(y[0]), "v"(x[1]), "s"(y[-1]), "v"(x[2]), "s"(y[-2]), "v"(x[3]), "s"(y[-3]), "v"(x[4]), "s"(y[-4]), "v"(x[5]), "s"(y[-5]), "v"(x[6]), "s"(y[-6]), "v"(x[7]), "s"(y[-7]), "v"(x[8]), "s"(y[-8]), "v"(x[9]), "s"(y[-9]), "v"(x[10]), "s"(y[-10]), "v"(x[11]), "s"(y[-11]) : "vcc");
    }
};
template <>
struct MacChain<13> {
    static __device__ inline __attribute__((always_inline)) void vv(uint64_t &acc, const uint32_t *x, const uint32_t *y)
    {
        asm("v_mad_u64_u32 %0, vcc, %1, %2, %0\n\tv_mad_u64_u32 %0, vcc, %3, %4, %0\n\tv_mad_u64_u32 %0, vcc, %5, %6, %0\n\tv_mad_u64_u32 %0, vcc, %7, %8, %0\n\tv_mad_u64_u32 %0, vcc, %9, %10, %0\n\tv_mad_u64_u32 %0, vcc, %11, %12, %0\n\tv_mad_u64_u32 %0, vcc, %13, %14, %0\n\tv_mad_u64_u32 %0, vcc, %15, %16, %0\n\tv_mad_u64_u32 %0, vcc, %17, %18, %0\n\tv_mad_u64_u32 %0, vcc, %19, %20, %0\n\tv_mad_u64_u32 %0, vcc, %21, %22, %0\n\tv_mad_u64_u32 %0, vcc, %23, %24, %0\n\tv_mad_u64_u32 %0, vcc, %25, %26, %0" : "+v"(acc) : "v"(x[0]), "v"(y[0]), "v"(x[1]), "v"(y[-1]), "v"(x[2]), "v"(y[-2]), "v"(x[3]), "v"(y[-3]), "v"(x[4]), "v"(y[-4]), "v"(x[5]), "v"(y[-5]), "v"(x[6]), "v"(y[-6]), "v"(x[7]), "v"(y[-7]), "v"(x[8]), "v"(y[-8]), "v"(x[9]), "v"(y[-9]), "v"(x[10]), "v"(y[-10]), "v"(x[11]), "v"(y[-11]), "v"(x[12]), "v"(y[-12]) : "vcc");
    }
    static __device__ inline __attribute__((always_inline)) void vs(uint64_t &acc, const uint32_t *x, const uint32_t *y)
    {
        asm("v_mad_u64_u32 %0, vcc, %1, %2, %0\n\tv_mad_u64_u32 %0, vcc, %3, %4, %0\n\tv_mad_u64_u32 %0, vcc, %5, %6, %0\n\tv_mad_u64_u32 %0, vcc, %7, %8, %0\n\tv_mad_u64_u32 %0, vcc, %9, %10, %0\n\tv_mad_u64_u32 %0, vcc, %11, %12, %0\n\tv_mad_u64_u32 %0, vcc, %13, %14, %0\n\tv_mad_u64_u32 %0, vcc, %15, %16, %0\n\tv_mad_u64_u32 %0, vcc, %17, %18, %0\n\tv_mad_u64_u32 %0, vcc, %19, %20, %0\n\tv_mad_u64_u32 %0, vcc, %21, %22, %0\n\tv_mad_u64_u32 %0, vcc, %23, %24, %0\n\tv_mad_u64_u32 %0, vcc, %25, %26, %0" : "+v"(acc) : "v"(x[0]), "s"(y[0]), "v"(x[1]), "s"(y[-1]), "v"(x[2]), "s"(y[-2]), "v"(x[3]), "s"(y[-3]), "v"(x[4]), "s"(y[-4]), "v"(x[5]), "s"(y[-5]), "v"(x[6]), "s"(y[-6]), "v"(x[7]), "s"(y[-7]), "v"(x[8]), "s"(y[-8]), "v"(x[9]), "s"(y[-9]), "v"(x[10]), "s"(y[-10]), "v"(x[11]), "s"(y[-11]), "v"(x[12]), "s"(y[-12]) : "vcc");
    }
    static __device__ inline __attribute__((always_inline)) void vv0(uint64_t &acc, const uint32_t *x, const uint32_t *y)
    {
        asm("v_mad_u64_u32 %0, vcc, %1, %2, 0\n\tv_mad_u64_u32 %0, vcc, %3, %4, %0\n\tv_mad_u64_u32 %0, vcc, %5, %6, %0\n\tv_mad_u64_u32 %0, vcc, %7, %8, %0\n\tv_mad_u64_u32 %0, vcc, %9, %10, %0\n\tv_mad_u64_u32 %0, vcc, %11, %12, %0\n\tv_mad_u64_u32 %0, vcc, %13, %14, %0\n\tv_mad_u64_u32 %0, vcc, %15, %16, %0\n\tv_mad_u64_u32 %0, vcc, %17, %18, %0\n\tv_mad_u64_u32 %0, vcc, %19, %20, %0\n\tv_mad_u64_u32 %0, vcc, %21, %22, %0\n\tv_mad_u64_u32 %0, vcc, %23, %24, %0\n\tv_mad_u64_u32 %0, vcc, %25, %26, %0" : "=&v"(acc) : "v"(x[0]), "v"(y[0]), "v"(x[1]), "v"(y[-1]), "v"(x[2]), "v"(y[-2]), "v"(x[3]), "v"(y[-3]), "v"(x[4]), "v"(y[-4]), "v"(x[5]), "v"(y[-5]), "v"(x[6]), "v"(y[-6]), "v"(x[7]), "v"(y[-7]), "v"(x[8]), "v"(y[-8]), "v"(x[9]), "v"(y[-9]), "v"(x[10]), "v"(y[-10]), "v"(x[11]), "v"(y[-11]), "v"(x[12]), "v"(y[-12]) : "vcc");
    }
    static __device__ inline __attribute__((always_inline)) void vs0(uint64_t &acc, const uint32_t *x, const uint32_t *y)
    {
        asm("v_mad_u64_u32 %0, vcc, %1, %2, 0\n\tv_mad_u64_u32 %0, vcc, %3, %4, %0\n\tv_mad_u64_u32 %0, vcc, %5, %6, %0\n\tv_mad_u64_u32 %0, vcc, %7, %8, %0\n\tv_mad_u64_u32 %0, vcc, %9, %10, %0\n\tv_mad_u64_u32 %0, vcc, %11, %12, %0\n\tv_mad_u64_u32 %0, vcc, %13, %14, %0\n\tv_mad_u64_u32 %0, vcc, %15, %16, %0\n\tv_mad_u64_u32 %0, vcc, %17, %18, %0\n\tv_mad_u64_u32 %0, vcc, %19, %20, %0\n\tv_mad_u64_u32 %0, vcc, %21, %22, %0\n\tv_mad_u64_u32 %0, vcc, %23, %24, %0\n\tv_mad_u64_u32 %0, vcc, %25, %26, %0" : "=&v"(acc) : "v"(x[0]), "s"(y[0]), "v"(x[1]), "s"(y[-1]), "v"(x[2]), "s"(y[-2]), "v"(x[3]), "s"(y[-3]), "v"(x[4]), "s"(y[-4]), "v"(x[5]), "s"(y[-5]), "v"(x[6]), "s"(y[-6]), "v"(x[7]), "s"(y[-7]), "v"(x[8]), "s"(y[-8]), "v"(x[9]), "s"(y[-9]), "v"(x[10]), "s"(y[-10]), "v"(x[11]), "s"(y[-11]), "v"(x[12]), "s"(y[-12]) : "vcc");
    }
};
template <>
struct MacChain<14> {
    static __device__ inline __attribute__((always_inline)) void vv(uint64_t &acc, const uint32_t *x, const uint32_t *y)
    {
        asm("v_mad_u64_u32 %0, vcc, %1, %2, %0\n\tv_mad_u64_u32 %0, vcc, %3, %4, %0\n\tv_mad_u64_u32 %0, vcc, %5, %6, %0\n\tv_mad_u64_u32 %0, vcc, %7, %8, %0\n\tv_mad_u64_u32 %0, vcc, %9, %10, %0\n\tv_mad_u64_u32 %0, vcc, %11, %12, %0\n\tv_mad_u64_u32 %0, vcc, %13, %14, %0\n\tv_mad_u64_u32 %0, vcc, %15, %16, %0\n\tv_mad_u64_u32 %0, vcc, %17, %18, %0\n\tv_mad_u64_u32 %0, vcc, %19, %20, %0\n\tv_mad_u64_u32 %0, vcc, %21, %22, %0\n\tv_mad_u64_u32 %0, vcc, %23, %24, %0\n\tv_mad_u64_u32 %0, vcc, %25, %26, %0\n\tv_mad_u64_u32 %0, vcc, %27, %28, %0" : "+v"(acc) : "v"(x[0]), "v"(y[0]), "v"(x[1]), "v"(y[-1]), "v"(x[2]), "v"(y[-2]), "v"(x[3]), "v"(y[-3]), "v"(x[4]), "v"(y[-4]), "v"(x[5]), "v"(y[-5]), "v"(x[6]), "v"(y[-6]), "v"(x[7]), "v"(y[-7]), "v"(x[8]), "v"(y[-8]), "v"(x[9]), "v"(y[-9]), "v"(x[10]), "v"(y[-10]), "v"(x[11]), "v"(y[-11]), "v"(x[12]), "v"(y[-12]), "v"(x[13]), "v"(y[-13]) : "vcc");
    }
    static __device__ inline __attribute__((always_inline)) void vs(uint64_t &acc, const uint32_t *x, const uint32_t *y)
    {
        asm("v_mad_u64_u32 %0, vcc, %1, %2, %0\n\tv_mad_u64_u32 %0, vcc, %3, %4, %0\n\tv_mad_u64_u32 %0, vcc, %5, %6, %0\n\tv_mad_u64_u32 %0, vcc, %7, %8, %0\n\tv_mad_u64_u32 %0, vcc, %9, %10, %0\n\tv_mad_u64_u32 %0, vcc, %11, %12, %0\n\tv_mad_u64_u32 %0, vcc, %13, %14, %0\n\tv_mad_u64_u32 %0, vcc, %15, %16, %0\n\tv_mad_u64_u32 %0, vcc, %17, %18, %0\n\tv_mad_u64_u32 %0, vcc, %19, %20, %0\n\tv_mad_u64_u32 %0, vcc, %21, %22, %0\n\tv_mad_u64_u32 %0, vcc, %23, %24, %0\n\tv_mad_u64_u32 %0, vcc, %25, %26, %0\n\tv_mad_u64_u32 %0, vcc, %27, %28, %0" : "+v"(acc) : "v"(x[0]), "s"(y[0]), "v"(x[1]), "s"(y[-1]), "v"(x[2]), "s"(y[-2]), "v"(x[3]), "s"(y[-3]), "v"(x[4]), "s"(y[-4]), "v"(x[5]), "s"(y[-5]), "v"(x[6]), "s"(y[-6]), "v"(x[7]), "s"(y[-7]), "v"(x[8]), "s"(y[-8]), "v"(x[9]), "s"(y[-9]), "v"(x[10]), "s"(y[-10]), "v"(x[11]), "s"(y[-11]), "v"(x[12]), "s"(y[-12]), "v"(x[13]), "s"(y[-13]) : "vcc");
    }
    static __device__ inline __attribute__((always_inline)) void vv0(uint64_t &acc, const uint32_t *x, const uint32_t *y)
    {
        asm("v_mad_u64_u32 %0, vcc, %1, %2, 0\n\tv_mad_u64_u32 %0, vcc, %3, %4, %0\n\tv_mad_u64_u32 %0, vcc, %5, %6, %0\n\tv_mad_u64_u32 %0, vcc, %7, %8, %0\n\tv_mad_u64_u32 %0, vcc, %9, %10, %0\n\tv_mad_u64_u32 %0, vcc, %11, %12, %0\n\tv_mad_u64_u32 %0, vcc, %13, %14, %0\n\tv_mad_u64_u32 %0, vcc, %15, %16, %0\n\tv_mad_u64_u32 %0, vcc, %17, %18, %0\n\tv_mad_u64_u32 %0, vcc, %19, %20, %0\n\tv_mad_u64_u32 %0, vcc, %21, %22, %0\n\tv_mad_u64_u32 %0, vcc, %23, %24, %0\n\tv_mad_u64_u32 %0, vcc, %25, %26, %0\n\tv_mad_u64_u32 %0, vcc, %27, %28, %0" : "=&v"(acc) : "v"(x[0]), "v"(y[0]), "v"(x[1]), "v"(y[-1]), "v"(x[2]), "v"(y[-2]), "v"(x[3]), "v"(y[-3]), "v"(x[4]), "v"(y[-4]), "v"(x[5]), "v"(y[-5]), "v"(x[6]), "v"(y[-6]), "v"(x[7]), "v"(y[-7]), "v"(x[8]), "v"(y[-8]), "v"(x[9]), "v"(y[-9]), "v"(x[10]), "v"(y[-10]), "v"(x[11]), "v"(y[-11]), "v"(x[12]), "v"(y[-12]), "v"(x[13]), "v"(y[-13]) : "vcc");
    }
    static __device__ inline __attribute__((always_inline)) void vs0(uint64_t &acc, const uint32_t *x, const uint32_t *y)
    {
        asm("v_mad_u64_u32 %0, vcc, %1, %2, 0\n\tv_mad_u64_u32 %0, vcc, %3, %4, %0\n\tv_mad_u64_u32 %0, vcc, %5, %6, %0\n\tv_mad_u64_u32 %0, vcc, %7, %8, %0\n\tv_mad_u64_u32 %0, vcc, %9, %10, %0\n\tv_mad_u64_u32 %0, vcc, %11, %12, %0\n\tv_mad_u64_u32 %0, vcc, %13, %14, %0\n\tv_mad_u64_u32 %0, vcc, %15, %16, %0\n\tv_mad_u64_u32 %0, vcc, %17, %18, %0\n\tv_mad_u64_u32 %0, vcc, %19, %20, %0\n\tv_mad_u64_u32 %0, vcc, %21, %22, %0\n\tv_mad_u64_u32 %0, vcc, %23, %24, %0\n\tv_mad_u64_u32 %0, vcc, %25, %26, %0\n\tv_mad_u64_u32 %0, vcc, %27, %28, %0" : "=&v"(acc) : "v"(x[0]), "s"(y[0]), "v"(x[1]), "s"(y[-1]), "v"(x[2]), "s"(y[-2]), "v"(x[3]), "s"(y[-3]), "v"(x[4]), "s"(y[-4]), "v"(x[5]), "s"(y[-5]), "v"(x[6]), "s"(y[-6]), "v"(x[7]), "s"(y[-7]), "v"(x[8]), "s"(y[-8]), "v"(x[9]), "s"(y[-9]), "v"(x[10]), "s"(y[-10]), "v"(x[11]), "s"(y[-11]), "v"(x[12]), "s"(y[-12]), "v"(x[13]), "s"(y[-13]) : "vcc");
    }
};
template <>
struct MacChain<0> {
    static __device__ inline __attribute__((always_inline)) void vv(uint64_t &, const uint32_t *, const uint32_t *) {}
    static __device__ inline __attribute__((always_inline)) void vs(uint64_t &, const uint32_t *, const uint32_t *) {}
    static __device__ inline __attribute__((always_inline)) void vv0(uint64_t &acc, const uint32_t *, const uint32_t *) { acc = 0; }
    static __device__ inline __attribute__((always_inline)) void vs0(uint64_t &acc, const uint32_t *, const uint32_t *) { acc = 0; }
};

}
```

panda_amd/csrc/msm_impl.h:

```cpp
#pragma once
#include <algorithm>
#include <vector>

#include "curve29_quad.h"
#include "msm_sort.h"
#include "panda_internal.h"

namespace panda {

struct MsmRegistration {
    const void *wire;
    void *converted;
    unsigned log_n, curve;
    int device;
    bool tabled;
    WindowPlan plan;
    size_t bytes;
    const uint32_t *samples;
    uint64_t hash;
};
hipError_t msm_hash_wire(const void *d_buf, size_t bytes, hipStream_t s, uint64_t *hash);

struct MsmTuning {
    unsigned window_bits;
// ... 153 lines not shown
        dst[4 * i] = v.x;
        dst[4 * i + 1] = v.y;
        dst[4 * i + 2] = v.z;
        dst[4 * i + 3] = v.w;
    }
}

template <int WORDS>
__device__ __forceinline__ void load_words_stream(u32 *dst, const u32 *src)
{
    static_assert(WORDS % 4 == 0, "vector loads");
    typedef u32 v4u __attribute__((ext_vector_type(4)));
    const v4u *s4 = reinterpret_cast<const v4u *>(src);
#pragma unroll
    for (int i = 0; i < WORDS / 4; i++) {
        const v4u v = __builtin_nontemporal_load(&s4[i]);
        dst[4 * i] = v.x;
        dst[4 * i + 1] = v.y;
        dst[4 * i + 2] = v.z;
        dst[4 * i + 3] = v.w;
    }
}

template <int WORDS>
__device__ __forceinline__ void store_words(u32 *dst, const u32 *src)
{
    uint4 *d4 = reinterpret_cast<uint4 *>(dst);
#pragma unroll
    for (int i = 0; i < WORDS / 4; i++) d4[i] = make_uint4(src[4 * i], src[4 * i + 1], src[4 * i + 2], src[4 * i + 3]);
}


template <class F>
__global__ void __launch_bounds__(256) k_convert_bases(const u32 *__restrict__ wire, u32 *__restrict__ out, u64 n)
{
    constexpr int L = F::L;
    u64 i = (u64)blockIdx.x * blockDim.x + threadIdx.x;
    if (i >= n) return;
    u32 w[2 * L], o[2 * L];
    load_words<2 * L>(w, wire + i * 2 * L);
    Fe<F> x, y;
    bool inf = affine_from_wire(x, y, w);
    fe_reduce_once(x);
    fe_reduce_once(y);
    fe_pack(o, x);
    fe_pack(o + L, y);
    if (inf) {
#pragma unroll
        for (int k = 0; k < 2 * L; k++) o[k] = 0;
    }
    store_words<2 * L>(out + i * 2 * L, o);
}

template <class F>
__device__ __noinline__ void xyzz_add_outlined(Xyzz<F> &acc, const Xyzz<F> &q)
{
    xyzz_add(acc, q);
}
template <class F>
__device__ __noinline__ void xyzz_dbl_outlined(Xyzz<F> &r, const Xyzz<F> &p)
{
    xyzz_dbl(r, p);
}
template <class F>
__device__ __forceinline__ void xyzz_add_k(Xyzz<F> &acc, const Xyzz<F> &q)
{
    if constexpr (IsExt2<F>::value)
        xyzz_add_outlined(acc, q);
    else
        xyzz_add(acc, q);
}
template <class F>
__device__ __forceinline__ void xyzz_dbl_k(Xyzz<F> &r, const Xyzz<F> &p)
{
    if constexpr (IsExt2<F>::value)
        xyzz_dbl_outlined(r, p);
    else
        xyzz_dbl(r, p);
}

template <class F>
__device__ __noinline__ void xyzz_add_quad_outlined(Xyzz<F> &acc, const Xyzz<F> &q, unsigned role)
{
    xyzz_add_quad(acc, q, role);
}
template <class F>
__device__ __noinline__ void xyzz_dbl_quad_outlined(Xyzz<F> &r, const Xyzz<F> &p, unsigned role)
{
    xyzz_dbl_quad(r, p, role);
}
template <class F>
__device__ __forceinline__ void xyzz_add_q(Xyzz<F> &acc, const Xyzz<F> &q, unsigned role)
{
    if constexpr (IsExt2<F>::value)
        xyzz_add_quad_outlined(acc, q, role);
    else
        xyzz_add_quad(acc, q, role);
}
template <class F>
__device__ __forceinline__ void xyzz_dbl_q(Xyzz<F> &r, const Xyzz<F> &p, unsigned role)
{
    if constexpr (IsExt2<F>::value)
        xyzz_dbl_quad_outlined(r, p, role);
    else
        xyzz_dbl_quad(r, p, role);
}

__global__ void __launch_bounds__(panda::REG_SAMPLES * 16) k_take_samples(const u32 *__restrict__ wire, u32 *__restrict__ samples, u64 n, unsigned row_words)
{
    const unsigned t = threadIdx.x >> 4, l = threadIdx.x & 15;
    const u64 row = panda::sample_row(t, n);
    for (unsigned k = l; k < row_words; k += 16) samples[t * row_words + k] = wire[row * row_words + k];
}

__device__ __forceinline__ u32 owner_bucket(const u32 *off, u32 NB, u32 pos)
{
    u32 lo = 0, hi = NB;
    while (hi - lo > 1) {
        u32 mid = (lo + hi) >> 1;
        if (off[mid] <= pos) lo = mid;
        else hi = mid;
    }
    return lo;
}

__global__ void __launch_bounds__(256) k_chunk_first(const u32 *__restrict__ off, u32 *__restrict__ first, unsigned NB, unsigned K, unsigned chunks)
{
    const unsigned w = blockIdx.y;
    const u32 *ow = off + (u64)w * (NB + 1);
    u32 *fw = first + (u64)w * chunks;
    const unsigned b = blockIdx.x * blockDim.x + threadIdx.x;
    u32 t0 = 0, t1 = 0;
    if (b < NB) {
        const u32 lo = ow[b], hi = ow[b + 1];
        t0 = (lo + K - 1) / K;
        t1 = min((u32)((hi + K - 1) / K), (u32)chunks);
    }
    const unsigned lane = threadIdx.x & 63u;
    u64 wide = __ballot(t1 > t0 + 4);
    while (wide) {
        const int src = __ffsll((long long)wide) - 1;
        wide &= wide - 1;
        const u32 a = (u32)__shfl((int)t0, src), e = (u32)__shfl((int)t1, src), owner = (u32)__shfl((int)b, src);
        for (u32 t = a + lane; t < e; t += 64) fw[t] = owner;
    }
    if (t1 <= t0 + 4)
        for (u32 t = t0; t < t1; t++) fw[t] = b;
}

#ifndef PANDA_ROW_MASK
#define PANDA_ROW_MASK 0x7fffffffu
#endif
#ifndef PANDA_ACC_ITEMS
#define PANDA_ACC_ITEMS 0x3fu
#endif
constexpr unsigned ACC_ITEM_ROW_TUPLES = 32u;
constexpr unsigned ACC_ITEM_WORDS_NEG = 1u;
constexpr unsigned ACC_ITEM_Y_IDENTITY = 2u;
constexpr unsigned ACC_ITEM_QUAD_SHIFT = 4u;
constexpr unsigned ACC_ITEM_ID_FLAG = 8u;
constexpr unsigned ACC_ITEM_BOUNDARY = 16u;
template <class F>
struct AccSlim {
    static constexpr bool value = !IsExt2<F>::value && F::N <= 9;
};
template <class F>
__host__ __device__ constexpr bool acc_item(unsigned item)
{
    return AccSlim<F>::value && (PANDA_ACC_ITEMS & item) != 0;
}
template <class F>
struct PackedBase {
    u32 w[2 * F::L];
};

template <class F>
__device__ __forceinline__ void fetch_base(PackedBase<F> &b, const u32 *bases, u32 entry)
{
#if defined(PANDA_ROWS_NT)
    load_words_stream<2 * F::L>(b.w, bases + (u64)(entry & PANDA_ROW_MASK) * 2 * F::L);
#else
    load_words<2 * F::L>(b.w, bases + (u64)(entry & PANDA_ROW_MASK) * 2 * F::L);
#endif
}

template <class F>
struct PackedRow {
    typedef u32 v4u __attribute__((ext_vector_type(4)));
    v4u q[2 * F::L / 4];
};
template <class F>
__device__ __forceinline__ void fetch_row(PackedRow<F> &r, const u32 *bases, u32 entry)
{
    typedef typename PackedRow<F>::v4u v4u;
    const v4u *s4 = reinterpret_cast<const v4u *>(bases + (u64)(entry & PANDA_ROW_MASK) * 2 * F::L);
#pragma unroll
    for (int j = 0; j < 2 * F::L / 4; j++) {
#if defined(PANDA_ROWS_NT)
        r.q[j] = __builtin_nontemporal_load(&s4[j]);
#else
        r.q[j] = s4[j];
#endif
    }
}
template <class F>
__device__ __forceinline__ void row_words(PackedBase<F> &b, const PackedRow<F> &r)
{
#pragma unroll
    for (int j = 0; j < 2 * F::L / 4; j++) {
        b.w[4 * j] = r.q[j].x;
        b.w[4 * j + 1] = r.q[j].y;
        b.w[4 * j + 2] = r.q[j].z;
        b.w[4 * j + 3] = r.q[j].w;
    }
}

template <class F, bool RAW = false, bool SLIM = false>
__device__ __forceinline__ void unpack_base(Fe<F> &x, Fe<F> &y, bool &inf, const PackedBase<F> &b, u32 entry)
{
    constexpr int L = F::L;
    constexpr bool WORDS_NEG = SLIM && acc_item<F>(ACC_ITEM_WORDS_NEG);
    constexpr int NZ_FROM = SLIM && acc_item<F>(ACC_ITEM_Y_IDENTITY) ? L : 0;
    u32 nz = 0;
#pragma unroll
    for (int k = NZ_FROM; k < 2 * L; k++) nz |= b.w[k];
    if constexpr (WORDS_NEG) asm volatile("" : "+v"(nz));
    inf = (nz == 0);
    fe_unpack(x, b.w);
    if constexpr (WORDS_NEG) {
        u32 yw[L];
#pragma unroll
        for (int k = 0; k < L; k++) yw[k] = b.w[L + k];
        if (entry >> 31) fe_words_neg<F>(yw, b.w + L);
        fe_unpack(y, yw);
    } else {
        fe_unpack(y, b.w + L);
        if (entry >> 31) {
            Fe<F> ny;
            if constexpr (RAW)
                fe_neg_raw<F, 1>(ny, y);
            else
                fe_neg<F, 1>(ny, y);
            y = ny;
        }
    }
}

#ifndef ACC_RAW_Y
#define ACC_RAW_Y false
#endif
struct AccPart {
    const u32 *pos;
    unsigned lo, hi, last, hi_bucket;
    u32 *queue;
};

template <class F>
__device__ __forceinline__ void fetch_base_lds(uint4 *lds_wave, const u32 *bases, u32 entry)
{
    const u32 *src = bases + (u64)(entry & PANDA_ROW_MASK) * 2 * F::L;
#pragma unroll
    for (int j = 0; j < 2 * F::L / 4; j++)
        __builtin_amdgcn_global_load_lds((const __attribute__((address_space(1))) void *)(src + 4 * j), (__attribute__((address_space(3))) void *)(lds_wave + j * 64), 16, 0, 0);
}
template <class F>
__device__ __forceinline__ void read_base_lds(PackedBase<F> &b, const uint4 *lds_wave, unsigned lane)
{
    asm volatile("s_waitcnt vmcnt(0)" ::: "memory");
#pragma unroll
    for (int j = 0; j < 2 * F::L / 4; j++) {
        const uint4 v = lds_wave[j * 64 + lane];
        b.w[4 * j] = v.x;
        b.w[4 * j + 1] = v.y;
        b.w[4 * j + 2] = v.z;
        b.w[4 * j + 3] = v.w;
    }
}

template <class F, bool LDSROW, bool SWLDS = false>
__device__ __forceinline__ void accumulate_chunk(const u32 *__restrict__ bases, const u32 *__restrict__ sw, const u32 *__restrict__ ow, u32 *__restrict__ bw, u32 *__restrict__ pw,
                                                 u32 b, u32 start, u32 end, uint4 *lds_wave, unsigned lane, uint4 *lds_words = nullptr)
{
    constexpr int PW = 4 * F::N;
    u32 next = ow[b + 1];
    bool run_starts_inside = ow[b] >= start;
    Xyzz<F> acc;
    xyzz_set_identity(acc);

    PackedBase<F> next_base;
    const bool quads = ((reinterpret_cast<uintptr_t>(sw + start) & 15) == 0);
    const bool sectors = SWLDS && ((reinterpret_cast<uintptr_t>(sw + start) & 63) == 0);
    auto sector_to_lds = [&](u32 sector, const u32 *src) {
        const u32 buffer = (u32)__builtin_amdgcn_readfirstlane((int)(sector & 1u));
#pragma unroll
        for (int q = 0; q < 4; q++)
            __builtin_amdgcn_global_load_lds((const __attribute__((address_space(1))) void *)(src + 4 * q),
                                             (__attribute__((address_space(3))) void *)(lds_words + buffer * 256 + q * 64), 16, 0, 0);
    };
    uint4 quad = make_uint4(0, 0, 0, 0);
    if constexpr (SWLDS) {
        if (sectors) {
            sector_to_lds(0, sw + start);
            if (start + 16 < end) sector_to_lds(1, sw + start + 16);
            asm volatile("s_waitcnt vmcnt(0)" ::: "memory");
            quad = lds_words[lane];
        } else if (quads)
            quad = *reinterpret_cast<const uint4 *>(sw + start);
    } else if (quads)
        quad = *reinterpret_cast<const uint4 *>(sw + start);
    u32 cur_entry = quads ? quad.x : sw[start];
    u32 ahead_entry = quads ? quad.y : (start + 1 < end ? sw[start + 1] : 0u);
    constexpr bool ROW_TUPLES = !LDSROW && acc_item<F>(ACC_ITEM_ROW_TUPLES);
    constexpr int ROW_LOADS = 2 * F::L / 4;
    PackedRow<F> next_row;
    if constexpr (LDSROW)
        fetch_base_lds<F>(lds_wave, bases, cur_entry);
    else if constexpr (ROW_TUPLES)
        fetch_row<F>(next_row, bases, cur_entry);
    else
        fetch_base<F>(next_base, bases, cur_entry);
    constexpr bool QUAD_SHIFT = acc_item<F>(ACC_ITEM_QUAD_SHIFT);
    constexpr bool ID_FLAG = acc_item<F>(ACC_ITEM_ID_FLAG);
    constexpr bool SLIM_BOUNDARY = ID_FLAG && acc_item<F>(ACC_ITEM_BOUNDARY);
    constexpr bool Y_STORABLE = acc_item<F>(ACC_ITEM_WORDS_NEG) || !(ACC_RAW_Y && RawOperandOk<F>::value);
    bool acc_id = true;
    u32 *brun = bw + (u64)b * PW;
    if constexpr (QUAD_SHIFT) {
        quad.x = quad.y;
        quad.y = quad.z;
        quad.z = quad.w;
    }
    u32 trip = 0;
    for (u32 pos = start; pos < end; pos++, trip++) {
        Fe<F> cx, cy;
        bool cinf;
        const u32 entry = cur_entry;
        if constexpr (LDSROW) read_base_lds<F>(next_base, lds_wave, lane);
        if constexpr (ROW_TUPLES) row_words<F>(next_base, next_row);
        unpack_base<F, ACC_RAW_Y && RawOperandOk<F>::value, true>(cx, cy, cinf, next_base, entry);
        if constexpr (ROW_TUPLES) {
#pragma unroll
            for (int i = 0; i < F::N; i++) asm volatile("" : "+v"(cx.l[i]), "+v"(cy.l[i]));
        }
        const bool boundary = pos >= next;
        if (boundary) {
            if constexpr (SLIM_BOUNDARY) {
                store_xyzz<F>(run_starts_inside ? brun : pw, acc);
                run_starts_inside = true;
                do {
                    b++;
                    brun += PW;
                    next = ow[b + 1];
                } while (next <= pos);
                if (cinf) xyzz_set_identity(acc);
                acc_id = true;
            } else {
                store_xyzz<F>(run_starts_inside ? bw + (u64)b * PW : pw, acc);
                run_starts_inside = true;
                do {
                    b++;
                    next = ow[b + 1];
                } while (next <= pos);
                acc_id = cinf;
                if (cinf)
                    xyzz_set_identity(acc);
                else {
                    Fe<F> ty;
                    fe_norm(ty, cy);
                    xyzz_from_affine(acc, cx, ty);
                }
            }
        }
        if (pos + 1 < end) {
            cur_entry = ahead_entry;
            if constexpr (LDSROW)
                fetch_base_lds<F>(lds_wave, bases, cur_entry);
            else if constexpr (ROW_TUPLES)
                fetch_row<F>(next_row, bases, cur_entry);
            else
                fetch_base<F>(next_base, bases, cur_entry);
            if (pos + 2 < end) {
                if (quads) {
                    const u32 idx = QUAD_SHIFT ? trip + 2 : pos + 2 - start;
                    if ((idx & 3u) == 0) {
                        if (SWLDS && sectors) {
                            if ((idx & 15u) == 0) {
                                if (pos + 18 < end) {
                                    sector_to_lds((idx >> 4) + 1, sw + pos + 18);
                                    asm volatile("s_waitcnt vmcnt(%0)" ::"n"(ROW_LOADS + 4) : "memory");
                                } else
                                    asm volatile("s_waitcnt vmcnt(%0)" ::"n"(ROW_LOADS) : "memory");
                            }
                            quad = lds_words[((idx >> 4) & 1u) * 256 + ((idx >> 2) & 3u) * 64 + lane];
                        } else {
                            quad = *reinterpret_cast<const uint4 *>(sw + pos + 2);
                            if constexpr (ROW_TUPLES) asm volatile("" : "+v"(quad.x), "+v"(quad.y), "+v"(quad.z), "+v"(quad.w));
                        }
                    } else if constexpr (QUAD_SHIFT) {
                        quad.x = quad.y;
                        quad.y = quad.z;
                        quad.z = quad.w;
                    }
                    if constexpr (QUAD_SHIFT)
                        ahead_entry = quad.x;
                    else
                        ahead_entry = (idx & 2u) ? ((idx & 1u) ? quad.w : quad.z) : ((idx & 1u) ? quad.y : quad.x);
                } else {
                    ahead_entry = sw[pos + 2];
                    if constexpr (ROW_TUPLES) asm volatile("" : "+v"(ahead_entry));
                }
            }
        }
        if constexpr (!SLIM_BOUNDARY)
            if (boundary) continue;
        if (cinf) continue;
        if (ID_FLAG ? acc_id : xyzz_is_identity(acc)) {
            if constexpr (SLIM_BOUNDARY && Y_STORABLE) {
#pragma unroll
                for (int i = 0; i < F::N; i++) {
                    asm("v_mov_b32 %0, %1" : "=v"(acc.X.l[i]) : "v"(cx.l[i]));
                    asm("v_mov_b32 %0, %1" : "=v"(acc.Y.l[i]) : "v"(cy.l[i]));
                }
                fe_one(acc.ZZ);
                fe_one(acc.ZZZ);
            } else {
                Fe<F> ty;
                fe_norm(ty, cy);
                xyzz_from_affine(acc, cx, ty);
            }
            acc_id = false;
            continue;
        }
        const int rare = xyzz_madd_core(acc, cx, cy);
        if (rare) {
            if (rare == 1) {
                PackedBase<F> again;
                const u32 same = acc_item<F>(ACC_ITEM_WORDS_NEG) ? sw[pos] : entry;
                fetch_base<F>(again, bases, same);
                unpack_base<F, false, true>(cx, cy, cinf, again, same);
                xyzz_dbl_affine(acc, cx, cy);
                acc_id = xyzz_is_identity(acc);
            } else {
                xyzz_set_identity(acc);
                acc_id = true;
            }
        }
    }
    const bool starts_inside = run_starts_inside;
    const bool ends_inside = next <= end;
    u32 *dst = (starts_inside && ends_inside) ? (SLIM_BOUNDARY ? brun : bw + (u64)b * PW) : (starts_inside ? pw + PW : pw);
    store_xyzz<F>(dst, acc);
}

template <class F, bool PERSIST, int WAVES = AccWaves<F>::value, bool LDSROW = false, bool SWLDS = false>
__global__ void __launch_bounds__(128, WAVES) k_accumulate(const u32 *__restrict__ bases, const u32 *__restrict__ sorted, const u32 *__restrict__ off,
                                                    u32 *__restrict__ bucket_acc, u32 *__restrict__ parts, u64 stride, unsigned NB, unsigned K,
                                                    unsigned chunks, u32 *__restrict__ long_count, const u32 *__restrict__ stale, AccPart part,
                                                    const u32 *__restrict__ chunk_first)
{
    constexpr int PW = 4 * F::N;
    const unsigned w = blockIdx.y;
    const unsigned t0 = blockIdx.x * blockDim.x + threadIdx.x;
    const u32 *fw = chunk_first ? chunk_first + (u64)w * chunks : nullptr;
    if (t0 == 0) long_count[w] = 0;
    if (stale && *stale) return;
    const u32 *ow = off + (u64)w * (NB + 1);
    const u32 lo_pos = part.pos ? part.pos[part.lo] : 0u;
    const u32 limit = part.pos ? part.pos[part.hi] : ow[NB];
    const unsigned search_hi = part.pos ? part.hi_bucket : NB;
    const bool takes_short_chunk = part.pos ? part.last != 0 : true;
    const u32 *sw = sorted + (u64)w * stride;
    u32 *bw = bucket_acc + (u64)w * NB * PW;
    __shared__ uint4 s_rows[LDSROW ? 2 * (2 * F::L / 4) * 64 : 1];
    uint4 *lds_wave = s_rows + (threadIdx.x >> 6) * (LDSROW ? (2 * F::L / 4) * 64 : 0);
    __shared__ uint4 s_words[SWLDS ? 2 * 512 : 1];
    uint4 *lds_words = s_words + (threadIdx.x >> 6) * (SWLDS ? 512 : 0);
    const unsigned lane = threadIdx.x & 63u;
    if constexpr (PERSIST) {
        const unsigned first = lo_pos / K;
#pragma unroll 1
        for (;;) {
            unsigned base = 0;
            if (lane == 0) base = atomicAdd(part.queue, 64u);
            base = __builtin_amdgcn_readfirstlane(base) + first;
            if (base >= chunks || (u64)base * K >= limit) return;
            const unsigned t = base + lane;
            const u32 start = t * K;
            u32 end = start + K;
            bool mine = t < chunks && start < limit;
            bool clamped = false;
            if (end > limit) {
                mine = mine && takes_short_chunk;
                end = limit;
                clamped = true;
            }
            if (mine && (end > lo_pos || clamped))
                accumulate_chunk<F, LDSROW, SWLDS>(bases, sw, ow, bw, parts + ((u64)w * chunks + t) * 2 * PW, fw ? fw[t] : owner_bucket(ow, search_hi, start), start, end, lds_wave, lane, lds_words);
        }
    } else {
        const unsigned t = t0;
        if (t >= chunks) return;
        const u32 start = t * K;
        if (start >= limit) return;
        u32 end = start + K;
        bool clamped = false;
        if (end > limit) {
            if (!takes_short_chunk) return;
            end = limit;
            clamped = true;
        }
        if (end > lo_pos || clamped)
            accumulate_chunk<F, LDSROW, SWLDS>(bases, sw, ow, bw, parts + ((u64)w * chunks + t) * 2 * PW, fw ? fw[t] : owner_bucket(ow, search_hi, start), start, end, lds_wave, lane, lds_words);
    }
}

template <class F>
__device__ __forceinline__ void fetch_rows_shared(uint4 *lds_wave, const u32 *bases, u32 entry, unsigned lane)
{
    constexpr unsigned P = 2 * F::L / 4;
#pragma unroll
    for (unsigned m = 0; m < P; m++) {
        const unsigned f = m * 64 + lane;
        const u32 e = (u32)__shfl((int)entry, (int)(f / P));
        const u32 *src = bases + (u64)(e & PANDA_ROW_MASK) * 2 * F::L + 4 * (f % P);
        __builtin_amdgcn_global_load_lds((const __attribute__((address_space(1))) void *)src, (__attribute__((address_space(3))) void *)(lds_wave + m * 64), 16, 0, 0);
    }
}
template <class F>
__device__ __forceinline__ void read_row_shared(PackedBase<F> &b, const uint4 *lds_wave, unsigned lane)
{
    constexpr unsigned P = 2 * F::L / 4;
    asm volatile("s_waitcnt vmcnt(0)" ::: "memory");
#pragma unroll
    for (unsigned j = 0; j < P; j++) {
        const uint4 v = lds_wave[lane * P + j];
        b.w[4 * j] = v.x;
        b.w[4 * j + 1] = v.y;
        b.w[4 * j + 2] = v.z;
        b.w[4 * j + 3] = v.w;
    }
}

template <class F, int WAVES = AccWaves<F>::value>
__global__ void __launch_bounds__(128, WAVES) k_accumulate_shared(const u32 *__restrict__ bases, const u32 *__restrict__ sorted, const u32 *__restrict__ off,
                                                           u32 *__restrict__ bucket_acc, u32 *__restrict__ parts, u64 stride, unsigned NB, unsigned K,
                                                           unsigned chunks, u32 *__restrict__ long_count, const u32 *__restrict__ stale)
{
    constexpr int PW = 4 * F::N;
    constexpr unsigned P = 2 * F::L / 4;
    const unsigned w = blockIdx.y;
    const unsigned t = blockIdx.x * blockDim.x + threadIdx.x;
    if (t == 0) long_count[w] = 0;
    if (stale && *stale) return;
    const u32 *ow = off + (u64)w * (NB + 1);
    const u32 *sw = sorted + (u64)w * stride;
    u32 *bw = bucket_acc + (u64)w * NB * PW;
    u32 *pw = parts + ((u64)w * chunks + t) * 2 * PW;
    const u32 limit = ow[NB];
    const bool has = t < chunks && (u64)t * K < limit;
    if (__ballot(has) == 0) return;
    const u32 start = has ? t * K : 0u;
    const u32 end = has ? (u32)min((u64)start + K, (u64)limit) : 0u;
    __shared__ uint4 s_rows[2 * P * 64];
    uint4 *lds_wave = s_rows + (threadIdx.x >> 6) * (P * 64);
    const unsigned lane = threadIdx.x & 63u;

    u32 b = 0, next = 0;
    bool run_starts_inside = false;
    if (has) {
        b = owner_bucket(ow, NB, start);
        next = ow[b + 1];
        run_starts_inside = ow[b] >= start;
    }
    Xyzz<F> acc;
    xyzz_set_identity(acc);
    const bool quads = has && ((reinterpret_cast<uintptr_t>(sw + start) & 15) == 0);
    uint4 quad = make_uint4(0, 0, 0, 0);
    if (quads) quad = *reinterpret_cast<const uint4 *>(sw + start);
    u32 cur_entry = has ? (quads ? quad.x : sw[start]) : 0u;
    u32 ahead_entry = quads ? quad.y : (start + 1 < end ? sw[start + 1] : 0u);
    fetch_rows_shared<F>(lds_wave, bases, cur_entry, lane);
#pragma unroll 1
    for (u32 i = 0; i < K; i++) {
        const u32 pos = start + i;
        const bool live = pos < end;
        const u32 entry = cur_entry;
        PackedBase<F> row;
        read_row_shared<F>(row, lds_wave, lane);
        Fe<F> cx, cy;
        bool cinf;
        unpack_base<F, ACC_RAW_Y && RawOperandOk<F>::value>(cx, cy, cinf, row, entry);
        const bool boundary = live && pos >= next;
        if (boundary) {
            store_xyzz<F>(run_starts_inside ? bw + (u64)b * PW : pw, acc);
            run_starts_inside = true;
            do {
                b++;
                next = ow[b + 1];
            } while (next <= pos);
            if (cinf)
                xyzz_set_identity(acc);
            else {
                Fe<F> ty;
                fe_norm(ty, cy);
                xyzz_from_affine(acc, cx, ty);
            }
        }
        cur_entry = (pos + 1 < end) ? ahead_entry : 0u;
        if (i + 1 < K) fetch_rows_shared<F>(lds_wave, bases, cur_entry, lane);
        if (pos + 2 < end) {
            if (quads) {
                const u32 idx = i + 2;
                if ((idx & 3u) == 0) quad = *reinterpret_cast<const uint4 *>(sw + pos + 2);
                ahead_entry = (idx & 2u) ? ((idx & 1u) ? quad.w : quad.z) : ((idx & 1u) ? quad.y : quad.x);
            } else
                ahead_entry = sw[pos + 2];
        }
        if (!live || boundary || cinf) continue;
        if (xyzz_is_identity(acc)) {
            Fe<F> ty;
            fe_norm(ty, cy);
            xyzz_from_affine(acc, cx, ty);
            continue;
        }
        const int rare = xyzz_madd_core(acc, cx, cy);
        if (rare) {
            if (rare == 1) {
                PackedBase<F> again;
                fetch_base<F>(again, bases, entry);
                unpack_base<F>(cx, cy, cinf, again, entry);
                xyzz_dbl_affine(acc, cx, cy);
            } else
                xyzz_set_identity(acc);
        }
    }
    if (!has) return;
    const bool ends_inside = next <= end;
    u32 *dst = (run_starts_inside && ends_inside) ? bw + (u64)b * PW : (run_starts_inside ? pw + PW : pw);
    store_xyzz<F>(dst, acc);
}

constexpr unsigned LONG_SPAN = 128;
constexpr unsigned LONG_BLOCKS = 256;

template <class F, bool MERGE>
__global__ void __launch_bounds__(256) k_fixup(const u32 *__restrict__ off, const u32 *__restrict__ parts, u32 *__restrict__ bucket_acc, u32 *__restrict__ total,
                                               unsigned NB, unsigned K, unsigned chunks, u32 *__restrict__ long_count, u32 *__restrict__ long_list, unsigned long_cap)
{
    constexpr int PW = 4 * F::N;
    const unsigned w = blockIdx.y;
    const unsigned b = blockIdx.x * blockDim.x + threadIdx.x;
    if (b >= NB) return;
    const u32 *ow = off + (u64)w * (NB + 1);
    const u32 s = ow[b], e = ow[b + 1];
    Xyzz<F> acc, q;
    if (s == e) {
        if (!MERGE) {
            xyzz_set_identity(acc);
            store_xyzz<F>(bucket_acc + ((u64)w * NB + b) * PW, acc);
        }
        return;
    }
    const u32 t0 = s / K, t1 = (e - 1) / K;
    if (t0 == t1) {
        if (!MERGE) return;
        load_xyzz<F>(acc, bucket_acc + ((u64)w * NB + b) * PW);
    } else if (t1 - t0 > LONG_SPAN) {
        u32 slot = atomicAdd(&long_count[w], 1u);
        if (slot < long_cap) {
            u32 *e3 = long_list + ((u64)w * long_cap + slot) * 3;
            e3[0] = b;
            e3[1] = t0;
            e3[2] = t1;
        }
        return;
    } else {
        const u32 *pw = parts + (u64)w * chunks * 2 * PW;
        load_xyzz<F>(acc, pw + ((u64)t0 * 2 + 1) * PW);
        for (u32 t = t0 + 1; t <= t1; t++) {
            load_xyzz<F>(q, pw + (u64)t * 2 * PW);
            xyzz_add_k(acc, q);
        }
    }
    if (MERGE) {
        load_xyzz<F>(q, total + ((u64)w * NB + b) * PW);
        xyzz_add_k(acc, q);
        store_xyzz<F>(total + ((u64)w * NB + b) * PW, acc);
    } else
        store_xyzz<F>(bucket_acc + ((u64)w * NB + b) * PW, acc);
}

template <class F>
__global__ void __launch_bounds__(256) k_fixup_long(const u32 *__restrict__ parts, u32 *__restrict__ dst, unsigned add, unsigned NB, unsigned chunks,
                                                    const u32 *__restrict__ long_count, const u32 *__restrict__ long_list, unsigned long_cap)
{
    constexpr int PW = 4 * F::N;
    __shared__ __attribute__((aligned(16))) u32 lds[256 * PW];
    const unsigned w = blockIdx.y, t = threadIdx.x;
    const u32 count = min(long_count[w], long_cap);
    const u32 *pw = parts + (u64)w * chunks * 2 * PW;
    for (u32 item = blockIdx.x; item < count; item += gridDim.x) {
        const u32 *e3 = long_list + ((u64)w * long_cap + item) * 3;
        const u32 b = e3[0], t0 = e3[1], t1 = e3[2];
        Xyzz<F> acc, q;
        xyzz_set_identity(acc);
        for (u32 c = t0 + t; c <= t1; c += 256) {
            load_xyzz<F>(q, pw + ((u64)c * 2 + (c == t0 ? 1 : 0)) * PW);
            xyzz_add_k(acc, q);
        }
        store_xyzz<F>(lds + t * PW, acc);
        __syncthreads();
        for (unsigned s = 128; s > 0; s >>= 1) {
            if (t < s) {
                load_xyzz<F>(q, lds + (t + s) * PW);
                xyzz_add_k(acc, q);
                store_xyzz<F>(lds + t * PW, acc);
            }
            __syncthreads();
        }
        if (t == 0) {
            if (add) {
                load_xyzz<F>(q, dst + ((u64)w * NB + b) * PW);
                xyzz_add_k(acc, q);
            }
            store_xyzz<F>(dst + ((u64)w * NB + b) * PW, acc);
        }
        __syncthreads();
    }
}

template <class F>
__device__ __forceinline__ void wave_reduce(Xyzz<F> &acc, u32 *lds, unsigned lane)
{
    constexpr int PW = 4 * F::N;
    const unsigned quad = lane >> 2, role = lane & 3u;
    Xyzz<F> q;
    store_xyzz<F>(lds + lane * PW, acc);
    __syncthreads();
    load_xyzz<F>(acc, lds + (4 * quad) * PW);
#pragma unroll 1
    for (unsigned k = 1; k < 4; k++) {
        load_xyzz<F>(q, lds + (4 * quad + k) * PW);
        xyzz_add_q(acc, q, role);
    }
#pragma unroll 1
    for (unsigned s = 8; s > 0; s >>= 1) {
        __syncthreads();
        if (quad >= s && quad < 2 * s && role == 0) store_xyzz<F>(lds + quad * PW, acc);
        __syncthreads();
        if (quad < s) {
            load_xyzz<F>(q, lds + (quad + s) * PW);
            xyzz_add_q(acc, q, role);
        }
    }
}

template <class F>
__global__ void __launch_bounds__(64) k_sum_lines(const u32 *__restrict__ bucket_acc, u32 *__restrict__ outR, u32 *__restrict__ outC, unsigned rows, unsigned cols,
                                                  unsigned csplit)
{
    constexpr int PW = 4 * F::N;
    __shared__ __attribute__((aligned(16))) u32 lds[64 * PW];
    const unsigned x = blockIdx.x, list = blockIdx.y, lane = threadIdx.x;
    const u64 NB = (u64)rows * cols;
    const u32 *src;
    u32 *dst;
    unsigned count, stride;
    if (x < rows) {
        src = bucket_acc + (list * NB + (u64)x * cols) * PW;
        count = cols;
        stride = 1;
        dst = outR + ((u64)list * rows + x) * PW;
    } else {
        const unsigned seg = (x - rows) / cols, lo = (x - rows) % cols;
        count = rows / csplit;
        src = bucket_acc + (list * NB + (u64)seg * count * cols + lo) * PW;
        stride = cols;
        dst = outC + ((u64)list * cols * csplit + (x - rows)) * PW;
    }
    Xyzz<F> acc, q;
    xyzz_set_identity(acc);
#pragma unroll 1
    for (unsigned i = lane; i < count; i += 64) {
        load_xyzz<F>(q, src + (u64)i * stride * PW);
        xyzz_add_k(acc, q);
    }
    wave_reduce<F>(acc, lds, lane);
    if (lane == 0) store_xyzz<F>(dst, acc);
}

template <class F>
__global__ void __launch_bounds__(64) k_weighted_slots(const u32 *__restrict__ inR, const u32 *__restrict__ inC, u32 *__restrict__ slot_out, unsigned a, unsigned b,
                                                       unsigned csplit)
{
    constexpr int PW = 4 * F::N;
    __shared__ __attribute__((aligned(16))) u32 lds[64 * PW];
    const unsigned slot = blockIdx.x, list = blockIdx.y, part = blockIdx.z, parts = gridDim.z, lane = threadIdx.x, role = lane & 3u;
    const unsigned rows = 1u << a, cols = 1u << b, slots = 1 + a + b, partials = slots * parts;
    Xyzz<F> acc, q;
    xyzz_set_identity(acc);
    unsigned doublings = 0;
    if (slot == 0) {
        const u32 *src = inR + (u64)list * rows * PW;
        const unsigned per = (rows + parts - 1) / parts, end = min(rows, (part + 1) * per);
#pragma unroll 1
        for (unsigned i = part * per + lane; i < end; i += 64) {
            load_xyzz<F>(q, src + (u64)i * PW);
            xyzz_add_k(acc, q);
        }
    } else {
        const bool row_slot = slot <= a;
        const unsigned j = row_slot ? slot - 1 : slot - 1 - a;
        const unsigned half = (row_slot ? rows : cols * csplit) >> 1;
        const u32 *src = row_slot ? inR + (u64)list * rows * PW : inC + (u64)list * cols * csplit * PW;
        const u32 low = (1u << j) - 1;
        const unsigned per = (half + parts - 1) / parts, end = min(half, (part + 1) * per);
        doublings = j + (row_slot ? b : 0u);
#pragma unroll 1
        for (unsigned i = part * per + lane; i < end; i += 64) {
            const unsigned idx = ((i & ~low) << 1) | (1u << j) | (i & low);
            load_xyzz<F>(q, src + (u64)idx * PW);
            xyzz_add_k(acc, q);
        }
    }
    wave_reduce<F>(acc, lds, lane);
    if (lane < 4) {
#pragma unroll 1
        for (unsigned d = 0; d < doublings; d++) {
            xyzz_dbl_q(q, acc, role);
            acc = q;
        }
        if (lane == 0) store_xyzz<F>(slot_out + ((u64)list * partials + slot * parts + part) * PW, acc);
    }
}

template <class F>
__global__ void __launch_bounds__(64) k_slot_total(const u32 *__restrict__ slot_out, u32 *__restrict__ win, unsigned partials, unsigned emit)
{
    constexpr int PW = 4 * F::N;
    __shared__ __attribute__((aligned(16))) u32 lds[64 * PW];
    const unsigned list = blockIdx.x, lane = threadIdx.x;
    Xyzz<F> acc, q;
    xyzz_set_identity(acc);
#pragma unroll 1
    for (unsigned i = lane; i < partials; i += 64) {
        load_xyzz<F>(q, slot_out + ((u64)list * partials + i) * PW);
        xyzz_add_k(acc, q);
    }
    wave_reduce<F>(acc, lds, lane);
    if (lane == 0) {
        if (emit == 0)
            store_xyzz<F>(win + (u64)list * PW, acc);
        else {
            u32 out[3 * F::L];
            if (emit == 2)
                xyzz_to_homogeneous_wire(out, acc);
            else
                xyzz_to_jacobian_wire(out, acc);
#pragma unroll
            for (int k = 0; k < 3 * F::L; k++) win[(u64)list * (3 * F::L) + k] = out[k];
        }
    }
}

template <class F>
__global__ void __launch_bounds__(128) k_table_step(const u32 *__restrict__ prev, u32 *__restrict__ next, u64 n, unsigned steps)
{
    constexpr int L = F::L;
    const u64 i = (u64)blockIdx.x * blockDim.x + threadIdx.x;
    if (i >= n) return;
    PackedBase<F> b;
    load_words<2 * L>(b.w, prev + i * 2 * L);
    Fe<F> x, y;
    bool inf;
    unpack_base<F>(x, y, inf, b, 0u);
    u32 o[2 * L];
    if (inf) {
#pragma unroll
        for (int k = 0; k < 2 * L; k++) o[k] = 0;
    } else {
        Xyzz<F> p, d;
        xyzz_dbl_affine(p, x, y);
#pragma unroll 1
        for (unsigned s = 1; s < steps; s++) {
            xyzz_dbl_k(d, p);
            p = d;
        }
        xyzz_to_affine_internal(x, y, p);
        fe_reduce_once(x);
        fe_reduce_once(y);
        fe_pack(o, x);
        fe_pack(o + L, y);
    }
    store_words<2 * L>(next + i * 2 * L, o);
}

template <class F>
void host_horner(Xyzz<F> &result, const std::vector<Xyzz<F>> &windows, const panda::WindowPlan &plan)
{
    Xyzz<F> acc, d;
    xyzz_set_identity(acc);
    for (int w = (int)windows.size() - 1; w >= 0; w--) {
        for (unsigned k = 0; k < plan.width[w]; k++) {
            xyzz_dbl(d, acc);
            acc = d;
        }
        xyzz_add(acc, windows[w]);
    }
    result = acc;
}

unsigned floor_log2(u64 v)
{
    unsigned l = 0;
    while (v >> (l + 1)) l++;
    return l;
}

template <class Fq>
unsigned acc_chunk_entries(u64 entries, unsigned forced)
{
    const u64 per_k = entries >> 20;
    unsigned K = per_k >= 128 ? 128 : (per_k >= 64 ? 64 : (per_k >= 32 ? 32 : 16));
    if (Fq::N <= 9 && per_k < 32) K = per_k >= 12 ? 32 : (per_k >= 6 ? 24 : 16);
    if (forced) K = std::min(std::max((forced + 3u) & ~3u, 4u), 1024u);
    return K;
}

template <class C>
hipError_t msm_execute(const panda_msm_configuration &cfg, const panda::MsmRegistration *registration, panda::MsmTuning tuning, float *phase_ms, bool *stale,
                       const panda::MsmPipeline *pipe)
{
    typedef typename C::Fq Fq;
    constexpr int PW = 4 * Fq::N;
    constexpr int LQ = Fq::L;
    constexpr unsigned curve = panda::msm_scalar_field_of(C::ID);
    hipStream_t stream = static_cast<hipStream_t>(cfg.stream.handle);
// ... 520 lines not shown
```

Measured before the change: 1.012 billion points/s.

## Use signed-limb Montgomery arithmetic in bucket accumulation mixed addition

Adds signed 29-bit limb field operations (signed subtraction, v_mad_i64_i32-based multiply/square/mul-add with arithmetic-shift carries) and a signed mixed-add core for the bucket accumulation loop. Subtractions no longer add multiples of p, and the chained normalisation work is reduced. Accumulators stored in signed form are tagged with a high bit in ZZ and converted back to unsigned form on load in the later reduction kernels. It also enables the new accumulation item bit by default and uses a local-P variant of the y-negation. The cost is extra conversion work on every stored-bucket load and tighter bound reasoning that must hold for correctness.

Result: faster. 1.024 billion points/s (median of 6 runs) (+1.3%).

```diff
diff --git a/panda_amd/csrc/curve29.h b/panda_amd/csrc/curve29.h
--- a/panda_amd/csrc/curve29.h
+++ b/panda_amd/csrc/curve29.h
@@ -151,6 +151,64 @@
 }
 
 template <class F>
+struct SignedBounds {
+    static constexpr double H = (double)F::HEADROOM;
+    static constexpr double XS = 4.4, XN = 3.2, YS = 2.0, ZS = 2.0;
+    static constexpr double XM = XS > XN ? XS : XN;
+    static constexpr double PS = XM + ZS / H + 1, RS = YS + ZS / H + 1;
+    static constexpr double PPS = PS * PS / H + 1, P3S = PS * PPS / H + 1, QS = XM * PPS / H + 1;
+    static constexpr double RRS = RS * RS / H + 1, VS = QS + XM;
+    static_assert(PPS < 2, "PP must stay below 2p for fe_is_zero_2p");
+    static_assert(2 * QS + P3S < XN && RRS + 2 * QS + P3S < XS, "X3 leaves the accumulator's bound");
+    static_assert((RS * VS + YS * P3S) / H + 1 < YS, "Y3 leaves the accumulator's bound");
+    static_assert(ZS * PPS / H + 1 < ZS && ZS * P3S / H + 1 < ZS, "ZZ, ZZZ leave the accumulator's bound");
+    static constexpr int KX = 4, KY = 1, KZZZ = 1;
+    static_assert(XN < KX - 0.5 && XS + KX <= Bounds<F>::XB, "stored X after the conversion");
+    static_assert((RS * VS + YS * P3S) / H < KY - 0.5 && YS + KY <= Bounds<F>::YB, "stored Y after the conversion");
+    static_assert(ZS * P3S / H < KZZZ - 0.5 && ZS + KZZZ <= 3, "stored ZZZ after the conversion");
+};
+
+template <class F>
+PANDA_HD void signed_after_doubling(Xyzz<F> &acc)
+{
+    fe_reduce_small_2p(acc.X);
+}
+
+template <class F>
+PANDA_HD int xyzz_madd_core_s(Xyzz<F> &acc, const Fe<F> &bx, const Fe<F> &by)
+{
+    typedef SignedBounds<F> B;
+    (void)sizeof(B);
+    Fe<F> U2, S2, P, R, PP, PPP, Q, X3, Y3, t, rr, v, nppp;
+    fe_mul(U2, bx, acc.ZZ);
+    fe_sub_s(P, U2, acc.X);
+    fe_mul_s(S2, by, acc.ZZZ);
+    fe_sub_s(R, S2, acc.Y);
+    fe_sqr_s(PP, P);
+    if (fe_is_zero_2p(PP))
+        return fe_is_zero_mod_p_s(R) ? 1 : 2;
+    fe_mul_s(PPP, P, PP);
+    fe_mul_s(Q, acc.X, PP);
+    fe_mul(acc.ZZ, acc.ZZ, PP);
+    fe_mul_s(acc.ZZZ, acc.ZZZ, PPP);
+    fe_sqr_s(rr, R);
+#if defined(__HIP_DEVICE_COMPILE__)
+#pragma unroll
+    for (int i = 0; i < F::N; i++) asm volatile("" : "+v"(Q.l[i]), "+v"(PPP.l[i]) : "v"(rr.l[F::N - 1]));
+#endif
+    fe_add_nr(t, Q, Q);
+    fe_add_nr(t, t, PPP);
+    fe_sub_s_wide(X3, rr, t);
+    fe_norm_s(X3, X3);
+    fe_sub_s(v, Q, X3);
+    fe_neg_s(nppp, PPP);
+    fe_mul_add_s(Y3, R, v, acc.Y, nppp);
+    acc.X = X3;
+    acc.Y = Y3;
+    return 0;
+}
+
+template <class F>
 PANDA_HD void xyzz_madd(Xyzz<F> &acc, const Fe<F> &bx, const Fe<F> &by, bool base_identity)
 {
     if (base_identity) return;
diff --git a/panda_amd/csrc/fe29.h b/panda_amd/csrc/fe29.h
--- a/panda_amd/csrc/fe29.h
+++ b/panda_amd/csrc/fe29.h
@@ -31,6 +31,26 @@
 #endif
 
 #if defined(__HIP_DEVICE_COMPILE__) && !defined(FE29_NO_ASM)
+#define FE29_MAC_S(acc, x, y) asm("v_mad_i64_i32 %0, vcc, %1, %2, %0" : "+v"(acc) : "v"(x), "v"(y) : "vcc")
+#else
+#define FE29_MAC_S(acc, x, y) acc += (u64)((int64_t)(int32_t)(x) * (int32_t)(y))
+#endif
+#if defined(FE29_CHECK)
+#define FE29_SHADOW_DECL_S __int128 shadow = 0;
+#define FE29_SHADOW_MAC_S(x, y) shadow += (__int128)(int32_t)(x) * (int32_t)(y);
+#define FE29_SHADOW_SHIFT_S()                                                                                                      \
+    assert(shadow >= -((__int128)1 << 63) && shadow < ((__int128)1 << 63) && "fe29 signed column accumulator overflow");          \
+    assert((int64_t)acc == (int64_t)shadow && "fe29 signed column differs from its shadow");                                       \
+    shadow >>= 29;
+#define FE29_CHECK_SLIMB(x) assert((int32_t)(x) >= -(int32_t)SLIMB_MAX && (int32_t)(x) <= (int32_t)SLIMB_MAX && "fe29 signed operand limb range")
+#else
+#define FE29_SHADOW_DECL_S
+#define FE29_SHADOW_MAC_S(x, y)
+#define FE29_SHADOW_SHIFT_S()
+#define FE29_CHECK_SLIMB(x)
+#endif
+
+#if defined(__HIP_DEVICE_COMPILE__) && !defined(FE29_NO_ASM)
 #define FE29_DEVICE_CHAINS 1
 #include <utility>
 
@@ -43,6 +63,7 @@
 typedef uint64_t u64;
 constexpr u32 LIMB_BITS = 29;
 constexpr u32 LIMB_MASK = (1u << 29) - 1;
+constexpr u32 SLIMB_MAX = (1u << 29) + 16;
 
 template <class F>
 struct Fe {
@@ -99,7 +120,7 @@
 }
 
 #if defined(FE29_DEVICE_CHAINS)
-template <class F, int K>
+template <class F, int K, bool SGN = false>
 __device__ inline __attribute__((always_inline)) void fe29_reduce_col(uint64_t &acc, uint32_t *m, uint32_t *out)
 {
     constexpr int N = F::N;
@@ -118,7 +139,10 @@
             MacChain<2 * N - 1 - K>::vs(acc, m + (K - N + 1), &F::P[N - 1]);
         out[K - N] = (uint32_t)acc & ((1u << 29) - 1);
     }
-    acc >>= 29;
+    if constexpr (SGN)
+        acc = (uint64_t)((int64_t)acc >> 29);
+    else
+        acc >>= 29;
 }
 template <class F, int K>
 __device__ inline __attribute__((always_inline)) void fe29_mul_col(uint64_t &acc, const uint32_t *a, const uint32_t *b, uint32_t *m, uint32_t *out)
@@ -178,6 +202,64 @@
 {
     (fe29_sqr_col<F, K>(acc, a, a2, m, out), ...);
 }
+template <class F, int K>
+__device__ inline __attribute__((always_inline)) void fe29_mul_col_s(uint64_t &acc, const uint32_t *a, const uint32_t *b, uint32_t *m, uint32_t *out)
+{
+    constexpr int N = F::N;
+    if constexpr (K == 0)
+        MacChain<1>::vvi0(acc, a, b);
+    else if constexpr (K < N)
+        MacChain<K + 1>::vvi(acc, a, b + K);
+    else
+        MacChain<2 * N - 1 - K>::vvi(acc, a + (K - N + 1), b + (N - 1));
+    fe29_reduce_col<F, K, true>(acc, m, out);
+}
+template <class F, int K>
+__device__ inline __attribute__((always_inline)) void fe29_sqr_col_s(uint64_t &acc, const uint32_t *a, const uint32_t *a2, uint32_t *m, uint32_t *out)
+{
+    constexpr int N = F::N;
+    constexpr int I0 = K < N ? 0 : K - N + 1;
+    constexpr int CNT = (K + 1) / 2 - I0;
+    MacChain<CNT>::vvi(acc, a2 + I0, a + (K - I0));
+    if constexpr (K == 0)
+        MacChain<1>::vvi0(acc, a, a);
+    else if constexpr ((K & 1) == 0)
+        MacChain<1>::vvi(acc, a + K / 2, a + K / 2);
+    fe29_reduce_col<F, K, true>(acc, m, out);
+}
+template <class F, int K>
+__device__ inline __attribute__((always_inline)) void fe29_mul_add_col_s(uint64_t &acc, const uint32_t *a, const uint32_t *b, const uint32_t *c, const uint32_t *d, uint32_t *m,
+                                                                         uint32_t *out)
+{
+    constexpr int N = F::N;
+    if constexpr (K == 0) {
+        MacChain<1>::vvi0(acc, a, b);
+        MacChain<1>::vvi(acc, c, d);
+    } else if constexpr (K < N) {
+        MacChain<K + 1>::vvi(acc, a, b + K);
+        MacChain<K + 1>::vvi(acc, c, d + K);
+    } else {
+        MacChain<2 * N - 1 - K>::vvi(acc, a + (K - N + 1), b + (N - 1));
+        MacChain<2 * N - 1 - K>::vvi(acc, c + (K - N + 1), d + (N - 1));
+    }
+    fe29_reduce_col<F, K, true>(acc, m, out);
+}
+template <class F, int... K>
+__device__ inline __attribute__((always_inline)) void fe29_mul_cols_s(uint64_t &acc, const uint32_t *a, const uint32_t *b, uint32_t *m, uint32_t *out, std::integer_sequence<int, K...>)
+{
+    (fe29_mul_col_s<F, K>(acc, a, b, m, out), ...);
+}
+template <class F, int... K>
+__device__ inline __attribute__((always_inline)) void fe29_sqr_cols_s(uint64_t &acc, const uint32_t *a, const uint32_t *a2, uint32_t *m, uint32_t *out, std::integer_sequence<int, K...>)
+{
+    (fe29_sqr_col_s<F, K>(acc, a, a2, m, out), ...);
+}
+template <class F, int... K>
+__device__ inline __attribute__((always_inline)) void fe29_mul_add_cols_s(uint64_t &acc, const uint32_t *a, const uint32_t *b, const uint32_t *c, const uint32_t *d,
+                                                                          uint32_t *m, uint32_t *out, std::integer_sequence<int, K...>)
+{
+    (fe29_mul_add_col_s<F, K>(acc, a, b, c, d, m, out), ...);
+}
 #endif
 
 template <class F>
@@ -505,6 +587,282 @@
 }
 
 template <class F>
+struct SignedLimbsOk {
+    static constexpr bool value = !IsExt2<F>::value && F::N <= 9;
+};
+template <class F>
+PANDA_HD constexpr bool fe_signed_columns_fit()
+{
+    return 2ull * F::N * ((u64)SLIMB_MAX * SLIMB_MAX) + (u64)F::N * (1ull << 58) + (1ull << 35) < (1ull << 63);
+}
+
+template <class F>
+PANDA_HD void fe_mul_s(Fe<F> &r, const Fe<F> &a, const Fe<F> &b)
+{
+    constexpr int N = F::N;
+    static_assert(SignedLimbsOk<F>::value && fe_signed_columns_fit<F>(), "signed column accumulator too narrow");
+    u32 m[N];
+    u32 out[N];
+    u64 acc = 0;
+#if defined(FE29_DEVICE_CHAINS)
+    fe29_mul_cols_s<F>(acc, a.l, b.l, m, out, std::make_integer_sequence<int, 2 * N - 1>());
+    out[N - 1] = (u32)acc;
+#pragma unroll
+    for (int i = 0; i < N; i++) r.l[i] = out[i];
+    return;
+#endif
+    FE29_SHADOW_DECL_S
+#pragma unroll
+    for (int i = 0; i < N; i++) {
+        FE29_CHECK_SLIMB(a.l[i]);
+        FE29_CHECK_SLIMB(b.l[i]);
+    }
+#pragma unroll
+    for (int k = 0; k < N; k++) {
+#pragma unroll
+        for (int i = 0; i <= k; i++) {
+            FE29_MAC_S(acc, a.l[i], b.l[k - i]);
+            FE29_SHADOW_MAC_S(a.l[i], b.l[k - i])
+        }
+#pragma unroll
+        for (int i = 0; i < k; i++) {
+            FE29_MAC_CONST(acc, m[i], F::P[k - i]);
+            FE29_SHADOW_MAC_S(m[i], F::P[k - i])
+        }
+        m[k] = ((u32)acc * F::INV) & LIMB_MASK;
+        FE29_MAC_CONST(acc, m[k], F::P[0]);
+        FE29_SHADOW_MAC_S(m[k], F::P[0])
+        FE29_SHADOW_SHIFT_S()
+        acc = (u64)((int64_t)acc >> LIMB_BITS);
+    }
+#pragma unroll
+    for (int k = N; k < 2 * N - 1; k++) {
+#pragma unroll
+        for (int i = k - N + 1; i < N; i++) {
+            FE29_MAC_S(acc, a.l[i], b.l[k - i]);
+            FE29_SHADOW_MAC_S(a.l[i], b.l[k - i])
+        }
+#pragma unroll
+        for (int i = k - N + 1; i < N; i++) {
+            FE29_MAC_CONST(acc, m[i], F::P[k - i]);
+            FE29_SHADOW_MAC_S(m[i], F::P[k - i])
+        }
+        out[k - N] = (u32)acc & LIMB_MASK;
+        FE29_SHADOW_SHIFT_S()
+        acc = (u64)((int64_t)acc >> LIMB_BITS);
+    }
+    out[N - 1] = (u32)acc;
+#pragma unroll
+    for (int i = 0; i < N; i++) r.l[i] = out[i];
+}
+
+template <class F>
+PANDA_HD void fe_mul_add_s(Fe<F> &r, const Fe<F> &a, const Fe<F> &b, const Fe<F> &c, const Fe<F> &d)
+{
+    constexpr int N = F::N;
+    static_assert(SignedLimbsOk<F>::value && fe_signed_columns_fit<F>(), "signed column accumulator too narrow");
+    u32 m[N];
+    u32 out[N];
+    u64 acc = 0;
+#if defined(FE29_DEVICE_CHAINS)
+    fe29_mul_add_cols_s<F>(acc, a.l, b.l, c.l, d.l, m, out, std::make_integer_sequence<int, 2 * N - 1>());
+    out[N - 1] = (u32)acc;
+#pragma unroll
+    for (int i = 0; i < N; i++) r.l[i] = out[i];
+    return;
+#endif
+    FE29_SHADOW_DECL_S
+#pragma unroll
+    for (int i = 0; i < N; i++) {
+        FE29_CHECK_SLIMB(a.l[i]);
+        FE29_CHECK_SLIMB(b.l[i]);
+        FE29_CHECK_SLIMB(c.l[i]);
+        FE29_CHECK_SLIMB(d.l[i]);
+    }
+#pragma unroll
+    for (int k = 0; k < N; k++) {
+#pragma unroll
+        for (int i = 0; i <= k; i++) {
+            FE29_MAC_S(acc, a.l[i], b.l[k - i]);
+            FE29_SHADOW_MAC_S(a.l[i], b.l[k - i])
+            FE29_MAC_S(acc, c.l[i], d.l[k - i]);
+            FE29_SHADOW_MAC_S(c.l[i], d.l[k - i])
+        }
+#pragma unroll
+        for (int i = 0; i < k; i++) {
+            FE29_MAC_CONST(acc, m[i], F::P[k - i]);
+            FE29_SHADOW_MAC_S(m[i], F::P[k - i])
+        }
+        m[k] = ((u32)acc * F::INV) & LIMB_MASK;
+        FE29_MAC_CONST(acc, m[k], F::P[0]);
+        FE29_SHADOW_MAC_S(m[k], F::P[0])
+        FE29_SHADOW_SHIFT_S()
+        acc = (u64)((int64_t)acc >> LIMB_BITS);
+    }
+#pragma unroll
+    for (int k = N; k < 2 * N - 1; k++) {
+#pragma unroll
+        for (int i = k - N + 1; i < N; i++) {
+            FE29_MAC_S(acc, a.l[i], b.l[k - i]);
+            FE29_SHADOW_MAC_S(a.l[i], b.l[k - i])
+            FE29_MAC_S(acc, c.l[i], d.l[k - i]);
+            FE29_SHADOW_MAC_S(c.l[i], d.l[k - i])
+        }
+#pragma unroll
+        for (int i = k - N + 1; i < N; i++) {
+            FE29_MAC_CONST(acc, m[i], F::P[k - i]);
+            FE29_SHADOW_MAC_S(m[i], F::P[k - i])
+        }
+        out[k - N] = (u32)acc & LIMB_MASK;
+        FE29_SHADOW_SHIFT_S()
+        acc = (u64)((int64_t)acc >> LIMB_BITS);
+    }
+    out[N - 1] = (u32)acc;
+#pragma unroll
+    for (int i = 0; i < N; i++) r.l[i] = out[i];
+}
+
+template <class F>
+PANDA_HD void fe_sqr_s(Fe<F> &r, const Fe<F> &a)
+{
+    constexpr int N = F::N;
+    static_assert(SignedLimbsOk<F>::value && fe_signed_columns_fit<F>(), "signed column accumulator too narrow");
+    u32 m[N], out[N], a2[N];
+#pragma unroll
+    for (int i = 0; i < N; i++) a2[i] = a.l[i] << 1;
+    u64 acc = 0;
+#if defined(FE29_DEVICE_CHAINS)
+    fe29_sqr_cols_s<F>(acc, a.l, a2, m, out, std::make_integer_sequence<int, 2 * N - 1>());
+    out[N - 1] = (u32)acc;
+#pragma unroll
+    for (int i = 0; i < N; i++) r.l[i] = out[i];
+    return;
+#endif
+    FE29_SHADOW_DECL_S
+#pragma unroll
+    for (int i = 0; i < N; i++) FE29_CHECK_SLIMB(a.l[i]);
+#pragma unroll
+    for (int k = 0; k < N; k++) {
+#pragma unroll
+        for (int i = 0; 2 * i < k; i++) {
+            FE29_MAC_S(acc, a2[i], a.l[k - i]);
+            FE29_SHADOW_MAC_S(a2[i], a.l[k - i])
+        }
+        if ((k & 1) == 0) {
+            FE29_MAC_S(acc, a.l[k / 2], a.l[k / 2]);
+            FE29_SHADOW_MAC_S(a.l[k / 2], a.l[k / 2])
+        }
+#pragma unroll
+        for (int i = 0; i < k; i++) {
+            FE29_MAC_CONST(acc, m[i], F::P[k - i]);
+            FE29_SHADOW_MAC_S(m[i], F::P[k - i])
+        }
+        m[k] = ((u32)acc * F::INV) & LIMB_MASK;
+        FE29_MAC_CONST(acc, m[k], F::P[0]);
+        FE29_SHADOW_MAC_S(m[k], F::P[0])
+        FE29_SHADOW_SHIFT_S()
+        acc = (u64)((int64_t)acc >> LIMB_BITS);
+    }
+#pragma unroll
+    for (int k = N; k < 2 * N - 1; k++) {
+#pragma unroll
+        for (int i = k - N + 1; 2 * i < k; i++) {
+            FE29_MAC_S(acc, a2[i], a.l[k - i]);
+            FE29_SHADOW_MAC_S(a2[i], a.l[k - i])
+        }
+        if ((k & 1) == 0) {
+            FE29_MAC_S(acc, a.l[k / 2], a.l[k / 2]);
+            FE29_SHADOW_MAC_S(a.l[k / 2], a.l[k / 2])
+        }
+#pragma unroll
+        for (int i = k - N + 1; i < N; i++) {
+            FE29_MAC_CONST(acc, m[i], F::P[k - i]);
+            FE29_SHADOW_MAC_S(m[i], F::P[k - i])
+        }
+        out[k - N] = (u32)acc & LIMB_MASK;
+        FE29_SHADOW_SHIFT_S()
+        acc = (u64)((int64_t)acc >> LIMB_BITS);
+    }
+    out[N - 1] = (u32)acc;
+#pragma unroll
+    for (int i = 0; i < N; i++) r.l[i] = out[i];
+}
+
+template <class F>
+PANDA_HD void fe_sub_s(Fe<F> &r, const Fe<F> &a, const Fe<F> &b)
+{
+    static_assert(SignedLimbsOk<F>::value, "signed limbs: 9-limb prime fields only");
+#pragma unroll
+    for (int i = 0; i < F::N; i++) {
+        r.l[i] = a.l[i] - b.l[i];
+        FE29_CHECK_SLIMB(r.l[i]);
+    }
+}
+
+template <class F>
+PANDA_HD void fe_sub_s_wide(Fe<F> &r, const Fe<F> &a, const Fe<F> &b)
+{
+    static_assert(SignedLimbsOk<F>::value, "signed limbs: 9-limb prime fields only");
+#pragma unroll
+    for (int i = 0; i < F::N; i++) r.l[i] = a.l[i] - b.l[i];
+}
+
+template <class F>
+PANDA_HD void fe_neg_s(Fe<F> &r, const Fe<F> &a)
+{
+    static_assert(SignedLimbsOk<F>::value, "signed limbs: 9-limb prime fields only");
+#pragma unroll
+    for (int i = 0; i < F::N; i++) r.l[i] = 0u - a.l[i];
+}
+
+template <class F>
+PANDA_HD void fe_norm_s(Fe<F> &r, const Fe<F> &t)
+{
+    constexpr int N = F::N;
+    static_assert(SignedLimbsOk<F>::value, "signed limbs: 9-limb prime fields only");
+    u32 c[N];
+#pragma unroll
+    for (int i = 0; i < N - 1; i++) {
+        c[i] = (u32)((int32_t)t.l[i] >> LIMB_BITS);
+#if defined(FE29_CHECK)
+        assert((int32_t)c[i] >= -3 && (int32_t)c[i] <= 1 && "fe_norm_s carry range");
+#endif
+    }
+    u32 o[N];
+    o[0] = t.l[0] & LIMB_MASK;
+#pragma unroll
+    for (int i = 1; i < N - 1; i++) o[i] = (t.l[i] & LIMB_MASK) + c[i - 1];
+    o[N - 1] = t.l[N - 1] + c[N - 2];
+#pragma unroll
+    for (int i = 0; i < N; i++) r.l[i] = o[i];
+}
+
+template <class F>
+PANDA_HD bool fe_is_zero_mod_p_s(const Fe<F> &a)
+{
+    static_assert(F::HEADROOM >= 160, "the bound above is BN254-like: R / p >= 160");
+    Fe<F> one, t;
+    fe_one(one);
+    fe_mul_s(t, a, one);
+    return fe_is_zero_2p(t);
+}
+
+template <class F, int K>
+PANDA_HD void fe_from_signed(Fe<F> &r, const Fe<F> &a)
+{
+    static_assert(SignedLimbsOk<F>::value && K >= 1 && K <= 200, "signed limbs: 9-limb prime fields only");
+    Fe<F> t;
+#pragma unroll
+    for (int i = 0; i < F::N; i++) {
+#if defined(FE29_CHECK)
+        assert((int64_t)(int32_t)a.l[i] + (int64_t)F::KP[K][i] >= 0 && (int64_t)(int32_t)a.l[i] + (int64_t)F::KP[K][i] < (1ll << 32) && "fe_from_signed limb range");
+#endif
+        t.l[i] = a.l[i] + F::KP[K][i];
+    }
+    fe_norm(r, t);
+}
+
+template <class F>
 PANDA_HD void fe_unpack(Fe<F> &r, const u32 *w)
 {
     constexpr int N = F::N, L = F::L;
@@ -534,14 +892,21 @@
     }
 }
 
-template <class F>
+template <class F, bool LOCAL_P = false>
 PANDA_HD void fe_words_neg(u32 *r, const u32 *w)
 {
     static_assert(!IsExt2<F>::value, "prime fields only");
 #if defined(__clang__)
     unsigned borrow = 0;
 #pragma unroll
-    for (int i = 0; i < F::L; i++) r[i] = __builtin_subc(F::PW[i], w[i], borrow, &borrow);
+    for (int i = 0; i < F::L; i++) {
+        u32 pw = F::PW[i];
+#if defined(__HIP_DEVICE_COMPILE__)
+        if constexpr (LOCAL_P)
+            if (i > 0) asm volatile("v_mov_b32 %0, %1" : "=v"(pw) : "n"(F::PW[i]));
+#endif
+        r[i] = __builtin_subc(pw, w[i], borrow, &borrow);
+    }
 #else
     u32 borrow = 0;
 #pragma unroll
diff --git a/panda_amd/csrc/fe29_chain.h b/panda_amd/csrc/fe29_chain.h
--- a/panda_amd/csrc/fe29_chain.h
+++ b/panda_amd/csrc/fe29_chain.h
@@ -24,6 +24,14 @@
     {
         asm("v_mad_u64_u32 %0, vcc, %1, %2, 0" : "=&v"(acc) : "v"(x[0]), "s"(y[0]) : "vcc");
     }
+    static __device__ inline __attribute__((always_inline)) void vvi(uint64_t &acc, const uint32_t *x, const uint32_t *y)
+    {
+        asm("v_mad_i64_i32 %0, vcc, %1, %2, %0" : "+v"(acc) : "v"(x[0]), "v"(y[0]) : "vcc");
+    }
+    static __device__ inline __attribute__((always_inline)) void vvi0(uint64_t &acc, const uint32_t *x, const uint32_t *y)
+    {
+        asm("v_mad_i64_i32 %0, vcc, %1, %2, 0" : "=&v"(acc) : "v"(x[0]), "v"(y[0]) : "vcc");
+    }
 };
 template <>
 struct MacChain<2> {
@@ -43,6 +51,14 @@
     {
         asm("v_mad_u64_u32 %0, vcc, %1, %2, 0\n\tv_mad_u64_u32 %0, vcc, %3, %4, %0" : "=&v"(acc) : "v"(x[0]), "s"(y[0]), "v"(x[1]), "s"(y[-1]) : "vcc");
     }
+    static __device__ inline __attribute__((always_inline)) void vvi(uint64_t &acc, const uint32_t *x, const uint32_t *y)
+    {
+        asm("v_mad_i64_i32 %0, vcc, %1, %2, %0\n\tv_mad_i64_i32 %0, vcc, %3, %4, %0" : "+v"(acc) : "v"(x[0]), "v"(y[0]), "v"(x[1]), "v"(y[-1]) : "vcc");
+    }
+    static __device__ inline __attribute__((always_inline)) void vvi0(uint64_t &acc, const uint32_t *x, const uint32_t *y)
+    {
+        asm("v_mad_i64_i32 %0, vcc, %1, %2, 0\n\tv_mad_i64_i32 %0, vcc, %3, %4, %0" : "=&v"(acc) : "v"(x[0]), "v"(y[0]), "v"(x[1]), "v"(y[-1]) : "vcc");
+    }
 };
 template <>
 struct MacChain<3> {
@@ -62,6 +78,14 @@
     {
         asm("v_mad_u64_u32 %0, vcc, %1, %2, 0\n\tv_mad_u64_u32 %0, vcc, %3, %4, %0\n\tv_mad_u64_u32 %0, vcc, %5, %6, %0" : "=&v"(acc) : "v"(x[0]), "s"(y[0]), "v"(x[1]), "s"(y[-1]), "v"(x[2]), "s"(y[-2]) : "vcc");
     }
+    static __device__ inline __attribute__((always_inline)) void vvi(uint64_t &acc, const uint32_t *x, const uint32_t *y)
+    {
+        asm("v_mad_i64_i32 %0, vcc, %1, %2, %0\n\tv_mad_i64_i32 %0, vcc, %3, %4, %0\n\tv_mad_i64_i32 %0, vcc, %5, %6, %0" : "+v"(acc) : "v"(x[0]), "v"(y[0]), "v"(x[1]), "v"(y[-1]), "v"(x[2]), "v"(y[-2]) : "vcc");
+    }
+    static __device__ inline __attribute__((always_inline)) void vvi0(uint64_t &acc, const uint32_t *x, const uint32_t *y)
+    {
+        asm("v_mad_i64_i32 %0, vcc, %1, %2, 0\n\tv_mad_i64_i32 %0, vcc, %3, %4, %0\n\tv_mad_i64_i32 %0, vcc, %5, %6, %0" : "=&v"(acc) : "v"(x[0]), "v"(y[0]), "v"(x[1]), "v"(y[-1]), "v"(x[2]), "v"(y[-2]) : "vcc");
+    }
 };
 template <>
 struct MacChain<4> {
@@ -81,6 +105,14 @@
     {
         asm("v_mad_u64_u32 %0, vcc, %1, %2, 0\n\tv_mad_u64_u32 %0, vcc, %3, %4, %0\n\tv_mad_u64_u32 %0, vcc, %5, %6, %0\n\tv_mad_u64_u32 %0, vcc, %7, %8, %0" : "=&v"(acc) : "v"(x[0]), "s"(y[0]), "v"(x[1]), "s"(y[-1]), "v"(x[2]), "s"(y[-2]), "v"(x[3]), "s"(y[-3]) : "vcc");
     }
+    static __device__ inline __attribute__((always_inline)) void vvi(uint64_t &acc, const uint32_t *x, const uint32_t *y)
+    {
+        asm("v_mad_i64_i32 %0, vcc, %1, %2, %0\n\tv_mad_i64_i32 %0, vcc, %3, %4, %0\n\tv_mad_i64_i32 %0, vcc, %5, %6, %0\n\tv_mad_i64_i32 %0, vcc, %7, %8, %0" : "+v"(acc) : "v"(x[0]), "v"(y[0]), "v"(x[1]), "v"(y[-1]), "v"(x[2]), "v"(y[-2]), "v"(x[3]), "v"(y[-3]) : "vcc");
+    }
+    static __device__ inline __attribute__((always_inline)) void vvi0(uint64_t &acc, const uint32_t *x, const uint32_t *y)
+    {
+        asm("v_mad_i64_i32 %0, vcc, %1, %2, 0\n\tv_mad_i64_i32 %0, vcc, %3, %4, %0\n\tv_mad_i64_i32 %0, vcc, %5, %6, %0\n\tv_mad_i64_i32 %0, vcc, %7, %8, %0" : "=&v"(acc) : "v"(x[0]), "v"(y[0]), "v"(x[1]), "v"(y[-1]), "v"(x[2]), "v"(y[-2]), "v"(x[3]), "v"(y[-3]) : "vcc");
+    }
 };
 template <>
 struct MacChain<5> {
@@ -100,6 +132,14 @@
     {
         asm("v_mad_u64_u32 %0, vcc, %1, %2, 0\n\tv_mad_u64_u32 %0, vcc, %3, %4, %0\n\tv_mad_u64_u32 %0, vcc, %5, %6, %0\n\tv_mad_u64_u32 %0, vcc, %7, %8, %0\n\tv_mad_u64_u32 %0, vcc, %9, %10, %0" : "=&v"(acc) : "v"(x[0]), "s"(y[0]), "v"(x[1]), "s"(y[-1]), "v"(x[2]), "s"(y[-2]), "v"(x[3]), "s"(y[-3]), "v"(x[4]), "s"(y[-4]) : "vcc");
     }
+    static __device__ inline __attribute__((always_inline)) void vvi(uint64_t &acc, const uint32_t *x, const uint32_t *y)
+    {
+        asm("v_mad_i64_i32 %0, vcc, %1, %2, %0\n\tv_mad_i64_i32 %0, vcc, %3, %4, %0\n\tv_mad_i64_i32 %0, vcc, %5, %6, %0\n\tv_mad_i64_i32 %0, vcc, %7, %8, %0\n\tv_mad_i64_i32 %0, vcc, %9, %10, %0" : "+v"(acc) : "v"(x[0]), "v"(y[0]), "v"(x[1]), "v"(y[-1]), "v"(x[2]), "v"(y[-2]), "v"(x[3]), "v"(y[-3]), "v"(x[4]), "v"(y[-4]) : "vcc");
+    }
+    static __device__ inline __attribute__((always_inline)) void vvi0(uint64_t &acc, const uint32_t *x, const uint32_t *y)
+    {
+        asm("v_mad_i64_i32 %0, vcc, %1, %2, 0\n\tv_mad_i64_i32 %0, vcc, %3, %4, %0\n\tv_mad_i64_i32 %0, vcc, %5, %6, %0\n\tv_mad_i64_i32 %0, vcc, %7, %8, %0\n\tv_mad_i64_i32 %0, vcc, %9, %10, %0" : "=&v"(acc) : "v"(x[0]), "v"(y[0]), "v"(x[1]), "v"(y[-1]), "v"(x[2]), "v"(y[-2]), "v"(x[3]), "v"(y[-3]), "v"(x[4]), "v"(y[-4]) : "vcc");
+    }
 };
 template <>
 struct MacChain<6> {
@@ -119,6 +159,14 @@
     {
         asm("v_mad_u64_u32 %0, vcc, %1, %2, 0\n\tv_mad_u64_u32 %0, vcc, %3, %4, %0\n\tv_mad_u64_u32 %0, vcc, %5, %6, %0\n\tv_mad_u64_u32 %0, vcc, %7, %8, %0\n\tv_mad_u64_u32 %0, vcc, %9, %10, %0\n\tv_mad_u64_u32 %0, vcc, %11, %12, %0" : "=&v"(acc) : "v"(x[0]), "s"(y[0]), "v"(x[1]), "s"(y[-1]), "v"(x[2]), "s"(y[-2]), "v"(x[3]), "s"(y[-3]), "v"(x[4]), "s"(y[-4]), "v"(x[5]), "s"(y[-5]) : "vcc");
     }
+    static __device__ inline __attribute__((always_inline)) void vvi(uint64_t &acc, const uint32_t *x, const uint32_t *y)
+    {
+        asm("v_mad_i64_i32 %0, vcc, %1, %2, %0\n\tv_mad_i64_i32 %0, vcc, %3, %4, %0\n\tv_mad_i64_i32 %0, vcc, %5, %6, %0\n\tv_mad_i64_i32 %0, vcc, %7, %8, %0\n\tv_mad_i64_i32 %0, vcc, %9, %10, %0\n\tv_mad_i64_i32 %0, vcc, %11, %12, %0" : "+v"(acc) : "v"(x[0]), "v"(y[0]), "v"(x[1]), "v"(y[-1]), "v"(x[2]), "v"(y[-2]), "v"(x[3]), "v"(y[-3]), "v"(x[4]), "v"(y[-4]), "v"(x[5]), "v"(y[-5]) : "vcc");
+    }
+    static __device__ inline __attribute__((always_inline)) void vvi0(uint64_t &acc, const uint32_t *x, const uint32_t *y)
+    {
+        asm("v_mad_i64_i32 %0, vcc, %1, %2, 0\n\tv_mad_i64_i32 %0, vcc, %3, %4, %0\n\tv_mad_i64_i32 %0, vcc, %5, %6, %0\n\tv_mad_i64_i32 %0, vcc, %7, %8, %0\n\tv_mad_i64_i32 %0, vcc, %9, %10, %0\n\tv_mad_i64_i32 %0, vcc, %11, %12, %0" : "=&v"(acc) : "v"(x[0]), "v"(y[0]), "v"(x[1]), "v"(y[-1]), "v"(x[2]), "v"(y[-2]), "v"(x[3]), "v"(y[-3]), "v"(x[4]), "v"(y[-4]), "v"(x[5]), "v"(y[-5]) : "vcc");
+    }
 };
 template <>
 struct MacChain<7> {
@@ -138,6 +186,14 @@
     {
         asm("v_mad_u64_u32 %0, vcc, %1, %2, 0\n\tv_mad_u64_u32 %0, vcc, %3, %4, %0\n\tv_mad_u64_u32 %0, vcc, %5, %6, %0\n\tv_mad_u64_u32 %0, vcc, %7, %8, %0\n\tv_mad_u64_u32 %0, vcc, %9, %10, %0\n\tv_mad_u64_u32 %0, vcc, %11, %12, %0\n\tv_mad_u64_u32 %0, vcc, %13, %14, %0" : "=&v"(acc) : "v"(x[0]), "s"(y[0]), "v"(x[1]), "s"(y[-1]), "v"(x[2]), "s"(y[-2]), "v"(x[3]), "s"(y[-3]), "v"(x[4]), "s"(y[-4]), "v"(x[5]), "s"(y[-5]), "v"(x[6]), "s"(y[-6]) : "vcc");
     }
+    static __device__ inline __attribute__((always_inline)) void vvi(uint64_t &acc, const uint32_t *x, const uint32_t *y)
+    {
+        asm("v_mad_i64_i32 %0, vcc, %1, %2, %0\n\tv_mad_i64_i32 %0, vcc, %3, %4, %0\n\tv_mad_i64_i32 %0, vcc, %5, %6, %0\n\tv_mad_i64_i32 %0, vcc, %7, %8, %0\n\tv_mad_i64_i32 %0, vcc, %9, %10, %0\n\tv_mad_i64_i32 %0, vcc, %11, %12, %0\n\tv_mad_i64_i32 %0, vcc, %13, %14, %0" : "+v"(acc) : "v"(x[0]), "v"(y[0]), "v"(x[1]), "v"(y[-1]), "v"(x[2]), "v"(y[-2]), "v"(x[3]), "v"(y[-3]), "v"(x[4]), "v"(y[-4]), "v"(x[5]), "v"(y[-5]), "v"(x[6]), "v"(y[-6]) : "vcc");
+    }
+    static __device__ inline __attribute__((always_inline)) void vvi0(uint64_t &acc, const uint32_t *x, const uint32_t *y)
+    {
+        asm("v_mad_i64_i32 %0, vcc, %1, %2, 0\n\tv_mad_i64_i32 %0, vcc, %3, %4, %0\n\tv_mad_i64_i32 %0, vcc, %5, %6, %0\n\tv_mad_i64_i32 %0, vcc, %7, %8, %0\n\tv_mad_i64_i32 %0, vcc, %9, %10, %0\n\tv_mad_i64_i32 %0, vcc, %11, %12, %0\n\tv_mad_i64_i32 %0, vcc, %13, %14, %0" : "=&v"(acc) : "v"(x[0]), "v"(y[0]), "v"(x[1]), "v"(y[-1]), "v"(x[2]), "v"(y[-2]), "v"(x[3]), "v"(y[-3]), "v"(x[4]), "v"(y[-4]), "v"(x[5]), "v"(y[-5]), "v"(x[6]), "v"(y[-6]) : "vcc");
+    }
 };
 template <>
 struct MacChain<8> {
@@ -157,6 +213,14 @@
     {
         asm("v_mad_u64_u32 %0, vcc, %1, %2, 0\n\tv_mad_u64_u32 %0, vcc, %3, %4, %0\n\tv_mad_u64_u32 %0, vcc, %5, %6, %0\n\tv_mad_u64_u32 %0, vcc, %7, %8, %0\n\tv_mad_u64_u32 %0, vcc, %9, %10, %0\n\tv_mad_u64_u32 %0, vcc, %11, %12, %0\n\tv_mad_u64_u32 %0, vcc, %13, %14, %0\n\tv_mad_u64_u32 %0, vcc, %15, %16, %0" : "=&v"(acc) : "v"(x[0]), "s"(y[0]), "v"(x[1]), "s"(y[-1]), "v"(x[2]), "s"(y[-2]), "v"(x[3]), "s"(y[-3]), "v"(x[4]), "s"(y[-4]), "v"(x[5]), "s"(y[-5]), "v"(x[6]), "s"(y[-6]), "v"(x[7]), "s"(y[-7]) : "vcc");
     }
+    static __device__ inline __attribute__((always_inline)) void vvi(uint64_t &acc, const uint32_t *x, const uint32_t *y)
+    {
+        asm("v_mad_i64_i32 %0, vcc, %1, %2, %0\n\tv_mad_i64_i32 %0, vcc, %3, %4, %0\n\tv_mad_i64_i32 %0, vcc, %5, %6, %0\n\tv_mad_i64_i32 %0, vcc, %7, %8, %0\n\tv_mad_i64_i32 %0, vcc, %9, %10, %0\n\tv_mad_i64_i32 %0, vcc, %11, %12, %0\n\tv_mad_i64_i32 %0, vcc, %13, %14, %0\n\tv_mad_i64_i32 %0, vcc, %15, %16, %0" : "+v"(acc) : "v"(x[0]), "v"(y[0]), "v"(x[1]), "v"(y[-1]), "v"(x[2]), "v"(y[-2]), "v"(x[3]), "v"(y[-3]), "v"(x[4]), "v"(y[-4]), "v"(x[5]), "v"(y[-5]), "v"(x[6]), "v"(y[-6]), "v"(x[7]), "v"(y[-7]) : "vcc");
+    }
+    static __device__ inline __attribute__((always_inline)) void vvi0(uint64_t &acc, const uint32_t *x, const uint32_t *y)
+    {
+        asm("v_mad_i64_i32 %0, vcc, %1, %2, 0\n\tv_mad_i64_i32 %0, vcc, %3, %4, %0\n\tv_mad_i64_i32 %0, vcc, %5, %6, %0\n\tv_mad_i64_i32 %0, vcc, %7, %8, %0\n\tv_mad_i64_i32 %0, vcc, %9, %10, %0\n\tv_mad_i64_i32 %0, vcc, %11, %12, %0\n\tv_mad_i64_i32 %0, vcc, %13, %14, %0\n\tv_mad_i64_i32 %0, vcc, %15, %16, %0" : "=&v"(acc) : "v"(x[0]), "v"(y[0]), "v"(x[1]), "v"(y[-1]), "v"(x[2]), "v"(y[-2]), "v"(x[3]), "v"(y[-3]), "v"(x[4]), "v"(y[-4]), "v"(x[5]), "v"(y[-5]), "v"(x[6]), "v"(y[-6]), "v"(x[7]), "v"(y[-7]) : "vcc");
+    }
 };
 template <>
 struct MacChain<9> {
@@ -176,6 +240,14 @@
     {
         asm("v_mad_u64_u32 %0, vcc, %1, %2, 0\n\tv_mad_u64_u32 %0, vcc, %3, %4, %0\n\tv_mad_u64_u32 %0, vcc, %5, %6, %0\n\tv_mad_u64_u32 %0, vcc, %7, %8, %0\n\tv_mad_u64_u32 %0, vcc, %9, %10, %0\n\tv_mad_u64_u32 %0, vcc, %11, %12, %0\n\tv_mad_u64_u32 %0, vcc, %13, %14, %0\n\tv_mad_u64_u32 %0, vcc, %15, %16, %0\n\tv_mad_u64_u32 %0, vcc, %17, %18, %0" : "=&v"(acc) : "v"(x[0]), "s"(y[0]), "v"(x[1]), "s"(y[-1]), "v"(x[2]), "s"(y[-2]), "v"(x[3]), "s"(y[-3]), "v"(x[4]), "s"(y[-4]), "v"(x[5]), "s"(y[-5]), "v"(x[6]), "s"(y[-6]), "v"(x[7]), "s"(y[-7]), "v"(x[8]), "s"(y[-8]) : "vcc");
     }
+    static __device__ inline __attribute__((always_inline)) void vvi(uint64_t &acc, const uint32_t *x, const uint32_t *y)
+    {
+        asm("v_mad_i64_i32 %0, vcc, %1, %2, %0\n\tv_mad_i64_i32 %0, vcc, %3, %4, %0\n\tv_mad_i64_i32 %0, vcc, %5, %6, %0\n\tv_mad_i64_i32 %0, vcc, %7, %8, %0\n\tv_mad_i64_i32 %0, vcc, %9, %10, %0\n\tv_mad_i64_i32 %0, vcc, %11, %12, %0\n\tv_mad_i64_i32 %0, vcc, %13, %14, %0\n\tv_mad_i64_i32 %0, vcc, %15, %16, %0\n\tv_mad_i64_i32 %0, vcc, %17, %18, %0" : "+v"(acc) : "v"(x[0]), "v"(y[0]), "v"(x[1]), "v"(y[-1]), "v"(x[2]), "v"(y[-2]), "v"(x[3]), "v"(y[-3]), "v"(x[4]), "v"(y[-4]), "v"(x[5]), "v"(y[-5]), "v"(x[6]), "v"(y[-6]), "v"(x[7]), "v"(y[-7]), "v"(x[8]), "v"(y[-8]) : "vcc");
+    }
+    static __device__ inline __attribute__((always_inline)) void vvi0(uint64_t &acc, const uint32_t *x, const uint32_t *y)
+    {
+        asm("v_mad_i64_i32 %0, vcc, %1, %2, 0\n\tv_mad_i64_i32 %0, vcc, %3, %4, %0\n\tv_mad_i64_i32 %0, vcc, %5, %6, %0\n\tv_mad_i64_i32 %0, vcc, %7, %8, %0\n\tv_mad_i64_i32 %0, vcc, %9, %10, %0\n\tv_mad_i64_i32 %0, vcc, %11, %12, %0\n\tv_mad_i64_i32 %0, vcc, %13, %14, %0\n\tv_mad_i64_i32 %0, vcc, %15, %16, %0\n\tv_mad_i64_i32 %0, vcc, %17, %18, %0" : "=&v"(acc) : "v"(x[0]), "v"(y[0]), "v"(x[1]), "v"(y[-1]), "v"(x[2]), "v"(y[-2]), "v"(x[3]), "v"(y[-3]), "v"(x[4]), "v"(y[-4]), "v"(x[5]), "v"(y[-5]), "v"(x[6]), "v"(y[-6]), "v"(x[7]), "v"(y[-7]), "v"(x[8]), "v"(y[-8]) : "vcc");
+    }
 };
 template <>
 struct MacChain<10> {
@@ -195,6 +267,14 @@
     {
         asm("v_mad_u64_u32 %0, vcc, %1, %2, 0\n\tv_mad_u64_u32 %0, vcc, %3, %4, %0\n\tv_mad_u64_u32 %0, vcc, %5, %6, %0\n\tv_mad_u64_u32 %0, vcc, %7, %8, %0\n\tv_mad_u64_u32 %0, vcc, %9, %10, %0\n\tv_mad_u64_u32 %0, vcc, %11, %12, %0\n\tv_mad_u64_u32 %0, vcc, %13, %14, %0\n\tv_mad_u64_u32 %0, vcc, %15, %16, %0\n\tv_mad_u64_u32 %0, vcc, %17, %18, %0\n\tv_mad_u64_u32 %0, vcc, %19, %20, %0" : "=&v"(acc) : "v"(x[0]), "s"(y[0]), "v"(x[1]), "s"(y[-1]), "v"(x[2]), "s"(y[-2]), "v"(x[3]), "s"(y[-3]), "v"(x[4]), "s"(y[-4]), "v"(x[5]), "s"(y[-5]), "v"(x[6]), "s"(y[-6]), "v"(x[7]), "s"(y[-7]), "v"(x[8]), "s"(y[-8]), "v"(x[9]), "s"(y[-9]) : "vcc");
     }
+    static __device__ inline __attribute__((always_inline)) void vvi(uint64_t &acc, const uint32_t *x, const uint32_t *y)
+    {
+        asm("v_mad_i64_i32 %0, vcc, %1, %2, %0\n\tv_mad_i64_i32 %0, vcc, %3, %4, %0\n\tv_mad_i64_i32 %0, vcc, %5, %6, %0\n\tv_mad_i64_i32 %0, vcc, %7, %8, %0\n\tv_mad_i64_i32 %0, vcc, %9, %10, %0\n\tv_mad_i64_i32 %0, vcc, %11, %12, %0\n\tv_mad_i64_i32 %0, vcc, %13, %14, %0\n\tv_mad_i64_i32 %0, vcc, %15, %16, %0\n\tv_mad_i64_i32 %0, vcc, %17, %18, %0\n\tv_mad_i64_i32 %0, vcc, %19, %20, %0" : "+v"(acc) : "v"(x[0]), "v"(y[0]), "v"(x[1]), "v"(y[-1]), "v"(x[2]), "v"(y[-2]), "v"(x[3]), "v"(y[-3]), "v"(x[4]), "v"(y[-4]), "v"(x[5]), "v"(y[-5]), "v"(x[6]), "v"(y[-6]), "v"(x[7]), "v"(y[-7]), "v"(x[8]), "v"(y[-8]), "v"(x[9]), "v"(y[-9]) : "vcc");
+    }
+    static __device__ inline __attribute__((always_inline)) void vvi0(uint64_t &acc, const uint32_t *x, const uint32_t *y)
+    {
+        asm("v_mad_i64_i32 %0, vcc, %1, %2, 0\n\tv_mad_i64_i32 %0, vcc, %3, %4, %0\n\tv_mad_i64_i32 %0, vcc, %5, %6, %0\n\tv_mad_i64_i32 %0, vcc, %7, %8, %0\n\tv_mad_i64_i32 %0, vcc, %9, %10, %0\n\tv_mad_i64_i32 %0, vcc, %11, %12, %0\n\tv_mad_i64_i32 %0, vcc, %13, %14, %0\n\tv_mad_i64_i32 %0, vcc, %15, %16, %0\n\tv_mad_i64_i32 %0, vcc, %17, %18, %0\n\tv_mad_i64_i32 %0, vcc, %19, %20, %0" : "=&v"(acc) : "v"(x[0]), "v"(y[0]), "v"(x[1]), "v"(y[-1]), "v"(x[2]), "v"(y[-2]), "v"(x[3]), "v"(y[-3]), "v"(x[4]), "v"(y[-4]), "v"(x[5]), "v"(y[-5]), "v"(x[6]), "v"(y[-6]), "v"(x[7]), "v"(y[-7]), "v"(x[8]), "v"(y[-8]), "v"(x[9]), "v"(y[-9]) : "vcc");
+    }
 };
 template <>
 struct MacChain<11> {
@@ -214,6 +294,14 @@
     {
         asm("v_mad_u64_u32 %0, vcc, %1, %2, 0\n\tv_mad_u64_u32 %0, vcc, %3, %4, %0\n\tv_mad_u64_u32 %0, vcc, %5, %6, %0\n\tv_mad_u64_u32 %0, vcc, %7, %8, %0\n\tv_mad_u64_u32 %0, vcc, %9, %10, %0\n\tv_mad_u64_u32 %0, vcc, %11, %12, %0\n\tv_mad_u64_u32 %0, vcc, %13, %14, %0\n\tv_mad_u64_u32 %0, vcc, %15, %16, %0\n\tv_mad_u64_u32 %0, vcc, %17, %18, %0\n\tv_mad_u64_u32 %0, vcc, %19, %20, %0\n\tv_mad_u64_u32 %0, vcc, %21, %22, %0" : "=&v"(acc) : "v"(x[0]), "s"(y[0]), "v"(x[1]), "s"(y[-1]), "v"(x[2]), "s"(y[-2]), "v"(x[3]), "s"(y[-3]), "v"(x[4]), "s"(y[-4]), "v"(x[5]), "s"(y[-5]), "v"(x[6]), "s"(y[-6]), "v"(x[7]), "s"(y[-7]), "v"(x[8]), "s"(y[-8]), "v"(x[9]), "s"(y[-9]), "v"(x[10]), "s"(y[-10]) : "vcc");
     }
+    static __device__ inline __attribute__((always_inline)) void vvi(uint64_t &acc, const uint32_t *x, const uint32_t *y)
+    {
+        asm("v_mad_i64_i32 %0, vcc, %1, %2, %0\n\tv_mad_i64_i32 %0, vcc, %3, %4, %0\n\tv_mad_i64_i32 %0, vcc, %5, %6, %0\n\tv_mad_i64_i32 %0, vcc, %7, %8, %0\n\tv_mad_i64_i32 %0, vcc, %9, %10, %0\n\tv_mad_i64_i32 %0, vcc, %11, %12, %0\n\tv_mad_i64_i32 %0, vcc, %13, %14, %0\n\tv_mad_i64_i32 %0, vcc, %15, %16, %0\n\tv_mad_i64_i32 %0, vcc, %17, %18, %0\n\tv_mad_i64_i32 %0, vcc, %19, %20, %0\n\tv_mad_i64_i32 %0, vcc, %21, %22, %0" : "+v"(acc) : "v"(x[0]), "v"(y[0]), "v"(x[1]), "v"(y[-1]), "v"(x[2]), "v"(y[-2]), "v"(x[3]), "v"(y[-3]), "v"(x[4]), "v"(y[-4]), "v"(x[5]), "v"(y[-5]), "v"(x[6]), "v"(y[-6]), "v"(x[7]), "v"(y[-7]), "v"(x[8]), "v"(y[-8]), "v"(x[9]), "v"(y[-9]), "v"(x[10]), "v"(y[-10]) : "vcc");
+    }
+    static __device__ inline __attribute__((always_inline)) void vvi0(uint64_t &acc, const uint32_t *x, const uint32_t *y)
+    {
+        asm("v_mad_i64_i32 %0, vcc, %1, %2, 0\n\tv_mad_i64_i32 %0, vcc, %3, %4, %0\n\tv_mad_i64_i32 %0, vcc, %5, %6, %0\n\tv_mad_i64_i32 %0, vcc, %7, %8, %0\n\tv_mad_i64_i32 %0, vcc, %9, %10, %0\n\tv_mad_i64_i32 %0, vcc, %11, %12, %0\n\tv_mad_i64_i32 %0, vcc, %13, %14, %0\n\tv_mad_i64_i32 %0, vcc, %15, %16, %0\n\tv_mad_i64_i32 %0, vcc, %17, %18, %0\n\tv_mad_i64_i32 %0, vcc, %19, %20, %0\n\tv_mad_i64_i32 %0, vcc, %21, %22, %0" : "=&v"(acc) : "v"(x[0]), "v"(y[0]), "v"(x[1]), "v"(y[-1]), "v"(x[2]), "v"(y[-2]), "v"(x[3]), "v"(y[-3]), "v"(x[4]), "v"(y[-4]), "v"(x[5]), "v"(y[-5]), "v"(x[6]), "v"(y[-6]), "v"(x[7]), "v"(y[-7]), "v"(x[8]), "v"(y[-8]), "v"(x[9]), "v"(y[-9]), "v"(x[10]), "v"(y[-10]) : "vcc");
+    }
 };
 template <>
 struct MacChain<12> {
@@ -233,6 +321,14 @@
     {
         asm("v_mad_u64_u32 %0, vcc, %1, %2, 0\n\tv_mad_u64_u32 %0, vcc, %3, %4, %0\n\tv_mad_u64_u32 %0, vcc, %5, %6, %0\n\tv_mad_u64_u32 %0, vcc, %7, %8, %0\n\tv_mad_u64_u32 %0, vcc, %9, %10, %0\n\tv_mad_u64_u32 %0, vcc, %11, %12, %0\n\tv_mad_u64_u32 %0, vcc, %13, %14, %0\n\tv_mad_u64_u32 %0, vcc, %15, %16, %0\n\tv_mad_u64_u32 %0, vcc, %17, %18, %0\n\tv_mad_u64_u32 %0, vcc, %19, %20, %0\n\tv_mad_u64_u32 %0, vcc, %21, %22, %0\n\tv_mad_u64_u32 %0, vcc, %23, %24, %0" : "=&v"(acc) : "v"(x[0]), "s"(y[0]), "v"(x[1]), "s"(y[-1]), "v"(x[2]), "s"(y[-2]), "v"(x[3]), "s"(y[-3]), "v"(x[4]), "s"(y[-4]), "v"(x[5]), "s"(y[-5]), "v"(x[6]), "s"(y[-6]), "v"(x[7]), "s"(y[-7]), "v"(x[8]), "s"(y[-8]), "v"(x[9]), "s"(y[-9]), "v"(x[10]), "s"(y[-10]), "v"(x[11]), "s"(y[-11]) : "vcc");
     }
+    static __device__ inline __attribute__((always_inline)) void vvi(uint64_t &acc, const uint32_t *x, const uint32_t *y)
+    {
+        asm("v_mad_i64_i32 %0, vcc, %1, %2, %0\n\tv_mad_i64_i32 %0, vcc, %3, %4, %0\n\tv_mad_i64_i32 %0, vcc, %5, %6, %0\n\tv_mad_i64_i32 %0, vcc, %7, %8, %0\n\tv_mad_i64_i32 %0, vcc, %9, %10, %0\n\tv_mad_i64_i32 %0, vcc, %11, %12, %0\n\tv_mad_i64_i32 %0, vcc, %13, %14, %0\n\tv_mad_i64_i32 %0, vcc, %15, %16, %0\n\tv_mad_i64_i32 %0, vcc, %17, %18, %0\n\tv_mad_i64_i32 %0, vcc, %19, %20, %0\n\tv_mad_i64_i32 %0, vcc, %21, %22, %0\n\tv_mad_i64_i32 %0, vcc, %23, %24, %0" : "+v"(acc) : "v"(x[0]), "v"(y[0]), "v"(x[1]), "v"(y[-1]), "v"(x[2]), "v"(y[-2]), "v"(x[3]), "v"(y[-3]), "v"(x[4]), "v"(y[-4]), "v"(x[5]), "v"(y[-5]), "v"(x[6]), "v"(y[-6]), "v"(x[7]), "v"(y[-7]), "v"(x[8]), "v"(y[-8]), "v"(x[9]), "v"(y[-9]), "v"(x[10]), "v"(y[-10]), "v"(x[11]), "v"(y[-11]) : "vcc");
+    }
+    static __device__ inline __attribute__((always_inline)) void vvi0(uint64_t &acc, const uint32_t *x, const uint32_t *y)
+    {
+        asm("v_mad_i64_i32 %0, vcc, %1, %2, 0\n\tv_mad_i64_i32 %0, vcc, %3, %4, %0\n\tv_mad_i64_i32 %0, vcc, %5, %6, %0\n\tv_mad_i64_i32 %0, vcc, %7, %8, %0\n\tv_mad_i64_i32 %0, vcc, %9, %10, %0\n\tv_mad_i64_i32 %0, vcc, %11, %12, %0\n\tv_mad_i64_i32 %0, vcc, %13, %14, %0\n\tv_mad_i64_i32 %0, vcc, %15, %16, %0\n\tv_mad_i64_i32 %0, vcc, %17, %18, %0\n\tv_mad_i64_i32 %0, vcc, %19, %20, %0\n\tv_mad_i64_i32 %0, vcc, %21, %22, %0\n\tv_mad_i64_i32 %0, vcc, %23, %24, %0" : "=&v"(acc) : "v"(x[0]), "v"(y[0]), "v"(x[1]), "v"(y[-1]), "v"(x[2]), "v"(y[-2]), "v"(x[3]), "v"(y[-3]), "v"(x[4]), "v"(y[-4]), "v"(x[5]), "v"(y[-5]), "v"(x[6]), "v"(y[-6]), "v"(x[7]), "v"(y[-7]), "v"(x[8]), "v"(y[-8]), "v"(x[9]), "v"(y[-9]), "v"(x[10]), "v"(y[-10]), "v"(x[11]), "v"(y[-11]) : "vcc");
+    }
 };
 template <>
 struct MacChain<13> {
@@ -252,6 +348,14 @@
     {
         asm("v_mad_u64_u32 %0, vcc, %1, %2, 0\n\tv_mad_u64_u32 %0, vcc, %3, %4, %0\n\tv_mad_u64_u32 %0, vcc, %5, %6, %0\n\tv_mad_u64_u32 %0, vcc, %7, %8, %0\n\tv_mad_u64_u32 %0, vcc, %9, %10, %0\n\tv_mad_u64_u32 %0, vcc, %11, %12, %0\n\tv_mad_u64_u32 %0, vcc, %13, %14, %0\n\tv_mad_u64_u32 %0, vcc, %15, %16, %0\n\tv_mad_u64_u32 %0, vcc, %17, %18, %0\n\tv_mad_u64_u32 %0, vcc, %19, %20, %0\n\tv_mad_u64_u32 %0, vcc, %21, %22, %0\n\tv_mad_u64_u32 %0, vcc, %23, %24, %0\n\tv_mad_u64_u32 %0, vcc, %25, %26, %0" : "=&v"(acc) : "v"(x[0]), "s"(y[0]), "v"(x[1]), "s"(y[-1]), "v"(x[2]), "s"(y[-2]), "v"(x[3]), "s"(y[-3]), "v"(x[4]), "s"(y[-4]), "v"(x[5]), "s"(y[-5]), "v"(x[6]), "s"(y[-6]), "v"(x[7]), "s"(y[-7]), "v"(x[8]), "s"(y[-8]), "v"(x[9]), "s"(y[-9]), "v"(x[10]), "s"(y[-10]), "v"(x[11]), "s"(y[-11]), "v"(x[12]), "s"(y[-12]) : "vcc");
     }
+    static __device__ inline __attribute__((always_inline)) void vvi(uint64_t &acc, const uint32_t *x, const uint32_t *y)
+    {
+        asm("v_mad_i64_i32 %0, vcc, %1, %2, %0\n\tv_mad_i64_i32 %0, vcc, %3, %4, %0\n\tv_mad_i64_i32 %0, vcc, %5, %6, %0\n\tv_mad_i64_i32 %0, vcc, %7, %8, %0\n\tv_mad_i64_i32 %0, vcc, %9, %10, %0\n\tv_mad_i64_i32 %0, vcc, %11, %12, %0\n\tv_mad_i64_i32 %0, vcc, %13, %14, %0\n\tv_mad_i64_i32 %0, vcc, %15, %16, %0\n\tv_mad_i64_i32 %0, vcc, %17, %18, %0\n\tv_mad_i64_i32 %0, vcc, %19, %20, %0\n\tv_mad_i64_i32 %0, vcc, %21, %22, %0\n\tv_mad_i64_i32 %0, vcc, %23, %24, %0\n\tv_mad_i64_i32 %0, vcc, %25, %26, %0" : "+v"(acc) : "v"(x[0]), "v"(y[0]), "v"(x[1]), "v"(y[-1]), "v"(x[2]), "v"(y[-2]), "v"(x[3]), "v"(y[-3]), "v"(x[4]), "v"(y[-4]), "v"(x[5]), "v"(y[-5]), "v"(x[6]), "v"(y[-6]), "v"(x[7]), "v"(y[-7]), "v"(x[8]), "v"(y[-8]), "v"(x[9]), "v"(y[-9]), "v"(x[10]), "v"(y[-10]), "v"(x[11]), "v"(y[-11]), "v"(x[12]), "v"(y[-12]) : "vcc");
+    }
+    static __device__ inline __attribute__((always_inline)) void vvi0(uint64_t &acc, const uint32_t *x, const uint32_t *y)
+    {
+        asm("v_mad_i64_i32 %0, vcc, %1, %2, 0\n\tv_mad_i64_i32 %0, vcc, %3, %4, %0\n\tv_mad_i64_i32 %0, vcc, %5, %6, %0\n\tv_mad_i64_i32 %0, vcc, %7, %8, %0\n\tv_mad_i64_i32 %0, vcc, %9, %10, %0\n\tv_mad_i64_i32 %0, vcc, %11, %12, %0\n\tv_mad_i64_i32 %0, vcc, %13, %14, %0\n\tv_mad_i64_i32 %0, vcc, %15, %16, %0\n\tv_mad_i64_i32 %0, vcc, %17, %18, %0\n\tv_mad_i64_i32 %0, vcc, %19, %20, %0\n\tv_mad_i64_i32 %0, vcc, %21, %22, %0\n\tv_mad_i64_i32 %0, vcc, %23, %24, %0\n\tv_mad_i64_i32 %0, vcc, %25, %26, %0" : "=&v"(acc) : "v"(x[0]), "v"(y[0]), "v"(x[1]), "v"(y[-1]), "v"(x[2]), "v"(y[-2]), "v"(x[3]), "v"(y[-3]), "v"(x[4]), "v"(y[-4]), "v"(x[5]), "v"(y[-5]), "v"(x[6]), "v"(y[-6]), "v"(x[7]), "v"(y[-7]), "v"(x[8]), "v"(y[-8]), "v"(x[9]), "v"(y[-9]), "v"(x[10]), "v"(y[-10]), "v"(x[11]), "v"(y[-11]), "v"(x[12]), "v"(y[-12]) : "vcc");
+    }
 };
 template <>
 struct MacChain<14> {
@@ -270,6 +374,14 @@
     static __device__ inline __attribute__((always_inline)) void vs0(uint64_t &acc, const uint32_t *x, const uint32_t *y)
     {
         asm("v_mad_u64_u32 %0, vcc, %1, %2, 0\n\tv_mad_u64_u32 %0, vcc, %3, %4, %0\n\tv_mad_u64_u32 %0, vcc, %5, %6, %0\n\tv_mad_u64_u32 %0, vcc, %7, %8, %0\n\tv_mad_u64_u32 %0, vcc, %9, %10, %0\n\tv_mad_u64_u32 %0, vcc, %11, %12, %0\n\tv_mad_u64_u32 %0, vcc, %13, %14, %0\n\tv_mad_u64_u32 %0, vcc, %15, %16, %0\n\tv_mad_u64_u32 %0, vcc, %17, %18, %0\n\tv_mad_u64_u32 %0, vcc, %19, %20, %0\n\tv_mad_u64_u32 %0, vcc, %21, %22, %0\n\tv_mad_u64_u32 %0, vcc, %23, %24, %0\n\tv_mad_u64_u32 %0, vcc, %25, %26, %0\n\tv_mad_u64_u32 %0, vcc, %27, %28, %0" : "=&v"(acc) : "v"(x[0]), "s"(y[0]), "v"(x[1]), "s"(y[-1]), "v"(x[2]), "s"(y[-2]), "v"(x[3]), "s"(y[-3]), "v"(x[4]), "s"(y[-4]), "v"(x[5]), "s"(y[-5]), "v"(x[6]), "s"(y[-6]), "v"(x[7]), "s"(y[-7]), "v"(x[8]), "s"(y[-8]), "v"(x[9]), "s"(y[-9]), "v"(x[10]), "s"(y[-10]), "v"(x[11]), "s"(y[-11]), "v"(x[12]), "s"(y[-12]), "v"(x[13]), "s"(y[-13]) : "vcc");
+    }
+    static __device__ inline __attribute__((always_inline)) void vvi(uint64_t &acc, const uint32_t *x, const uint32_t *y)
+    {
+        asm("v_mad_i64_i32 %0, vcc, %1, %2, %0\n\tv_mad_i64_i32 %0, vcc, %3, %4, %0\n\tv_mad_i64_i32 %0, vcc, %5, %6, %0\n\tv_mad_i64_i32 %0, vcc, %7, %8, %0\n\tv_mad_i64_i32 %0, vcc, %9, %10, %0\n\tv_mad_i64_i32 %0, vcc, %11, %12, %0\n\tv_mad_i64_i32 %0, vcc, %13, %14, %0\n\tv_mad_i64_i32 %0, vcc, %15, %16, %0\n\tv_mad_i64_i32 %0, vcc, %17, %18, %0\n\tv_mad_i64_i32 %0, vcc, %19, %20, %0\n\tv_mad_i64_i32 %0, vcc, %21, %22, %0\n\tv_mad_i64_i32 %0, vcc, %23, %24, %0\n\tv_mad_i64_i32 %0, vcc, %25, %26, %0\n\tv_mad_i64_i32 %0, vcc, %27, %28, %0" : "+v"(acc) : "v"(x[0]), "v"(y[0]), "v"(x[1]), "v"(y[-1]), "v"(x[2]), "v"(y[-2]), "v"(x[3]), "v"(y[-3]), "v"(x[4]), "v"(y[-4]), "v"(x[5]), "v"(y[-5]), "v"(x[6]), "v"(y[-6]), "v"(x[7]), "v"(y[-7]), "v"(x[8]), "v"(y[-8]), "v"(x[9]), "v"(y[-9]), "v"(x[10]), "v"(y[-10]), "v"(x[11]), "v"(y[-11]), "v"(x[12]), "v"(y[-12]), "v"(x[13]), "v"(y[-13]) : "vcc");
+    }
+    static __device__ inline __attribute__((always_inline)) void vvi0(uint64_t &acc, const uint32_t *x, const uint32_t *y)
+    {
+        asm("v_mad_i64_i32 %0, vcc, %1, %2, 0\n\tv_mad_i64_i32 %0, vcc, %3, %4, %0\n\tv_mad_i64_i32 %0, vcc, %5, %6, %0\n\tv_mad_i64_i32 %0, vcc, %7, %8, %0\n\tv_mad_i64_i32 %0, vcc, %9, %10, %0\n\tv_mad_i64_i32 %0, vcc, %11, %12, %0\n\tv_mad_i64_i32 %0, vcc, %13, %14, %0\n\tv_mad_i64_i32 %0, vcc, %15, %16, %0\n\tv_mad_i64_i32 %0, vcc, %17, %18, %0\n\tv_mad_i64_i32 %0, vcc, %19, %20, %0\n\tv_mad_i64_i32 %0, vcc, %21, %22, %0\n\tv_mad_i64_i32 %0, vcc, %23, %24, %0\n\tv_mad_i64_i32 %0, vcc, %25, %26, %0\n\tv_mad_i64_i32 %0, vcc, %27, %28, %0" : "=&v"(acc) : "v"(x[0]), "v"(y[0]), "v"(x[1]), "v"(y[-1]), "v"(x[2]), "v"(y[-2]), "v"(x[3]), "v"(y[-3]), "v"(x[4]), "v"(y[-4]), "v"(x[5]), "v"(y[-5]), "v"(x[6]), "v"(y[-6]), "v"(x[7]), "v"(y[-7]), "v"(x[8]), "v"(y[-8]), "v"(x[9]), "v"(y[-9]), "v"(x[10]), "v"(y[-10]), "v"(x[11]), "v"(y[-11]), "v"(x[12]), "v"(y[-12]), "v"(x[13]), "v"(y[-13]) : "vcc");
     }
 };
 template <>
@@ -277,6 +389,8 @@
     static __device__ inline __attribute__((always_inline)) void vv(uint64_t &, const uint32_t *, const uint32_t *) {}
     static __device__ inline __attribute__((always_inline)) void vs(uint64_t &, const uint32_t *, const uint32_t *) {}
     static __device__ inline __attribute__((always_inline)) void vv0(uint64_t &acc, const uint32_t *, const uint32_t *) { acc = 0; }
+    static __device__ inline __attribute__((always_inline)) void vvi(uint64_t &, const uint32_t *, const uint32_t *) {}
+    static __device__ inline __attribute__((always_inline)) void vvi0(uint64_t &acc, const uint32_t *, const uint32_t *) { acc = 0; }
     static __device__ inline __attribute__((always_inline)) void vs0(uint64_t &acc, const uint32_t *, const uint32_t *) { acc = 0; }
 };
 
diff --git a/panda_amd/csrc/msm_impl.h b/panda_amd/csrc/msm_impl.h
--- a/panda_amd/csrc/msm_impl.h
+++ b/panda_amd/csrc/msm_impl.h
@@ -329,7 +329,7 @@
 #define PANDA_ROW_MASK 0x7fffffffu
 #endif
 #ifndef PANDA_ACC_ITEMS
-#define PANDA_ACC_ITEMS 0x3fu
+#define PANDA_ACC_ITEMS 0x7fu
 #endif
 constexpr unsigned ACC_ITEM_ROW_TUPLES = 32u;
 constexpr unsigned ACC_ITEM_WORDS_NEG = 1u;
@@ -337,6 +337,7 @@
 constexpr unsigned ACC_ITEM_QUAD_SHIFT = 4u;
 constexpr unsigned ACC_ITEM_ID_FLAG = 8u;
 constexpr unsigned ACC_ITEM_BOUNDARY = 16u;
+constexpr unsigned ACC_ITEM_SIGNED_DIFF = 64u;
 template <class F>
 struct AccSlim {
     static constexpr bool value = !IsExt2<F>::value && F::N <= 9;
@@ -346,6 +347,22 @@
 {
     return AccSlim<F>::value && (PANDA_ACC_ITEMS & item) != 0;
 }
+constexpr u32 STORED_SIGNED_MARK = 0x80000000u;
+template <class F>
+__device__ __forceinline__ void load_xyzz_stored(Xyzz<F> &p, const u32 *src)
+{
+    load_xyzz<F>(p, src);
+    if constexpr (acc_item<F>(ACC_ITEM_SIGNED_DIFF)) {
+        if (p.ZZ.l[F::N - 1] & STORED_SIGNED_MARK) {
+            typedef SignedBounds<F> SB;
+            p.ZZ.l[F::N - 1] &= ~STORED_SIGNED_MARK;
+            fe_from_signed<F, SB::KX>(p.X, p.X);
+            fe_from_signed<F, SB::KY>(p.Y, p.Y);
+            fe_from_signed<F, SB::KZZZ>(p.ZZZ, p.ZZZ);
+        }
+    }
+}
+
 template <class F>
 struct PackedBase {
     u32 w[2 * F::L];
@@ -392,7 +409,7 @@
     }
 }
 
-template <class F, bool RAW = false, bool SLIM = false>
+template <class F, bool RAW = false, bool SLIM = false, bool LOCAL_P = false>
 __device__ __forceinline__ void unpack_base(Fe<F> &x, Fe<F> &y, bool &inf, const PackedBase<F> &b, u32 entry)
 {
     constexpr int L = F::L;
@@ -408,7 +425,7 @@
         u32 yw[L];
 #pragma unroll
         for (int k = 0; k < L; k++) yw[k] = b.w[L + k];
-        if (entry >> 31) fe_words_neg<F>(yw, b.w + L);
+        if (entry >> 31) fe_words_neg<F, LOCAL_P>(yw, b.w + L);
         fe_unpack(y, yw);
     } else {
         fe_unpack(y, b.w + L);
@@ -500,8 +517,13 @@
     constexpr bool ID_FLAG = acc_item<F>(ACC_ITEM_ID_FLAG);
     constexpr bool SLIM_BOUNDARY = ID_FLAG && acc_item<F>(ACC_ITEM_BOUNDARY);
     constexpr bool Y_STORABLE = acc_item<F>(ACC_ITEM_WORDS_NEG) || !(ACC_RAW_Y && RawOperandOk<F>::value);
+    constexpr bool SIGNED = acc_item<F>(ACC_ITEM_SIGNED_DIFF) && acc_item<F>(ACC_ITEM_WORDS_NEG) && !LDSROW;
     bool acc_id = true;
     u32 *brun = bw + (u64)b * PW;
+    auto store_acc = [&](u32 *dst) {
+        if constexpr (SIGNED) acc.ZZ.l[F::N - 1] |= (ID_FLAG ? acc_id : xyzz_is_identity(acc)) ? 0u : STORED_SIGNED_MARK;
+        store_xyzz<F>(dst, acc);
+    };
     if constexpr (QUAD_SHIFT) {
         quad.x = quad.y;
         quad.y = quad.z;
@@ -514,7 +536,7 @@
         const u32 entry = cur_entry;
         if constexpr (LDSROW) read_base_lds<F>(next_base, lds_wave, lane);
         if constexpr (ROW_TUPLES) row_words<F>(next_base, next_row);
-        unpack_base<F, ACC_RAW_Y && RawOperandOk<F>::value, true>(cx, cy, cinf, next_base, entry);
+        unpack_base<F, ACC_RAW_Y && RawOperandOk<F>::value, true, SIGNED>(cx, cy, cinf, next_base, entry);
         if constexpr (ROW_TUPLES) {
 #pragma unroll
             for (int i = 0; i < F::N; i++) asm volatile("" : "+v"(cx.l[i]), "+v"(cy.l[i]));
@@ -522,7 +544,7 @@
         const bool boundary = pos >= next;
         if (boundary) {
             if constexpr (SLIM_BOUNDARY) {
-                store_xyzz<F>(run_starts_inside ? brun : pw, acc);
+                store_acc(run_starts_inside ? brun : pw);
                 run_starts_inside = true;
                 do {
                     b++;
@@ -532,7 +554,7 @@
                 if (cinf) xyzz_set_identity(acc);
                 acc_id = true;
             } else {
-                store_xyzz<F>(run_starts_inside ? bw + (u64)b * PW : pw, acc);
+                store_acc(run_starts_inside ? bw + (u64)b * PW : pw);
                 run_starts_inside = true;
                 do {
                     b++;
@@ -608,7 +630,11 @@
             acc_id = false;
             continue;
         }
-        const int rare = xyzz_madd_core(acc, cx, cy);
+        int rare;
+        if constexpr (SIGNED)
+            rare = xyzz_madd_core_s(acc, cx, cy);
+        else
+            rare = xyzz_madd_core(acc, cx, cy);
         if (rare) {
             if (rare == 1) {
                 PackedBase<F> again;
@@ -616,6 +642,7 @@
                 fetch_base<F>(again, bases, same);
                 unpack_base<F, false, true>(cx, cy, cinf, again, same);
                 xyzz_dbl_affine(acc, cx, cy);
+                if constexpr (SIGNED) signed_after_doubling(acc);
                 acc_id = xyzz_is_identity(acc);
             } else {
                 xyzz_set_identity(acc);
@@ -626,7 +653,7 @@
     const bool starts_inside = run_starts_inside;
     const bool ends_inside = next <= end;
     u32 *dst = (starts_inside && ends_inside) ? (SLIM_BOUNDARY ? brun : bw + (u64)b * PW) : (starts_inside ? pw + PW : pw);
-    store_xyzz<F>(dst, acc);
+    store_acc(dst);
 }
 
 template <class F, bool PERSIST, int WAVES = AccWaves<F>::value, bool LDSROW = false, bool SWLDS = false>
@@ -841,7 +868,7 @@
     const u32 t0 = s / K, t1 = (e - 1) / K;
     if (t0 == t1) {
         if (!MERGE) return;
-        load_xyzz<F>(acc, bucket_acc + ((u64)w * NB + b) * PW);
+        load_xyzz_stored<F>(acc, bucket_acc + ((u64)w * NB + b) * PW);
     } else if (t1 - t0 > LONG_SPAN) {
         u32 slot = atomicAdd(&long_count[w], 1u);
         if (slot < long_cap) {
@@ -853,14 +880,14 @@
         return;
     } else {
         const u32 *pw = parts + (u64)w * chunks * 2 * PW;
-        load_xyzz<F>(acc, pw + ((u64)t0 * 2 + 1) * PW);
+        load_xyzz_stored<F>(acc, pw + ((u64)t0 * 2 + 1) * PW);
         for (u32 t = t0 + 1; t <= t1; t++) {
-            load_xyzz<F>(q, pw + (u64)t * 2 * PW);
+            load_xyzz_stored<F>(q, pw + (u64)t * 2 * PW);
             xyzz_add_k(acc, q);
         }
     }
     if (MERGE) {
-        load_xyzz<F>(q, total + ((u64)w * NB + b) * PW);
+        load_xyzz_stored<F>(q, total + ((u64)w * NB + b) * PW);
         xyzz_add_k(acc, q);
         store_xyzz<F>(total + ((u64)w * NB + b) * PW, acc);
     } else
@@ -882,7 +909,7 @@
         Xyzz<F> acc, q;
         xyzz_set_identity(acc);
         for (u32 c = t0 + t; c <= t1; c += 256) {
-            load_xyzz<F>(q, pw + ((u64)c * 2 + (c == t0 ? 1 : 0)) * PW);
+            load_xyzz_stored<F>(q, pw + ((u64)c * 2 + (c == t0 ? 1 : 0)) * PW);
             xyzz_add_k(acc, q);
         }
         store_xyzz<F>(lds + t * PW, acc);
@@ -897,7 +924,7 @@
         }
         if (t == 0) {
             if (add) {
-                load_xyzz<F>(q, dst + ((u64)w * NB + b) * PW);
+                load_xyzz_stored<F>(q, dst + ((u64)w * NB + b) * PW);
                 xyzz_add_k(acc, q);
             }
             store_xyzz<F>(dst + ((u64)w * NB + b) * PW, acc);
@@ -959,7 +986,7 @@
     xyzz_set_identity(acc);
 #pragma unroll 1
     for (unsigned i = lane; i < count; i += 64) {
-        load_xyzz<F>(q, src + (u64)i * stride * PW);
+        load_xyzz_stored<F>(q, src + (u64)i * stride * PW);
         xyzz_add_k(acc, q);
     }
     wave_reduce<F>(acc, lds, lane);
```
